# AmnonDrory/LidarRegistration

Measured on AMD Instinct MI355X. Metric: registration pairs/sec (30k-pt FCGF pairs, mutual-NN + 50k RANSAC iters + refit), higher is better.
Workload: dtype f32; 1 GPU; configs[1]: 30000-pt x32-d synthetic FCGF pair, --mode MNN --iters 50000, 3-pt sampling + ELC + LS refit; 192 distinct resident pairs per GPU, T copied to the host inside the timed region; pairs_per_batched_call=32, batched_calls_in_flight_per_gpu=2, parallelism=pair-sharded x1

## Files before the change

### include/lidarreg.h

```cpp
#ifndef LIDARREG_H
#define LIDARREG_H

#include <stddef.h>
#include <stdint.h>

#ifdef __cplusplus
extern "C" {
#endif

#define LR_API __attribute__((visibility("default")))

enum { LR_OK = 0, LR_EINVAL = -1, LR_ENOMEM = -2, LR_EHIP = -3, LR_ESIZE = -4 };

enum { LR_MODE_NO_FILTER = 0, LR_MODE_MNN = 1, LR_MODE_GPF = 2 };

typedef struct lr_workspace lr_workspace;

typedef struct lr_ransac_params {
    uint32_t struct_size;
    int32_t  sample_size;
    int32_t  use_elc;
    float    thr2;
    int32_t  iters;
    uint64_t seed;
    float    confidence;
    int32_t  batch;
    int32_t  sampler;
    int32_t  prosac_growth;
    int32_t  scoring;
    int32_t  local_opt;
    int32_t  lo_rounds;
    int32_t  lo_trials;
    int32_t  lo_max_calls;
    int32_t  min_iters;
} lr_ransac_params;

typedef struct lr_ransac_result {
    int64_t  best_h;
    uint32_t best_count;
    uint32_t pad0;
    uint64_t best_ssq;
    int64_t  n_valid;
    int64_t  n_ids;
} lr_ransac_result;

typedef struct lr_icp_result {
    double   fitness;
    double   inlier_rmse;
    int32_t  n_corr;
    int32_t  iterations;
} lr_icp_result;

typedef struct lr_pair_result {
    double   T[16];
    double   T_ransac[16];
    lr_ransac_result ransac;
    int32_t  n_corr;
    int32_t  n_refit;
    int32_t  n_nn_fixed;
    int32_t  status;
    int32_t  reserved[8];
    double   T_icp[16];
    lr_icp_result icp;
} lr_pair_result;

typedef struct lr_pair_params {
    uint32_t struct_size;
    int32_t  mode;
    int32_t  refit;
    lr_ransac_params ransac;
    int32_t  gpf_grid_wid;
    int32_t  icp;
    double   gpf_factor;
    double   refit_thr2;
} lr_pair_params;

LR_API int         lr_version(void);
LR_API const char *lr_last_error(void);

LR_API int    lr_workspace_create(lr_workspace **ws, int max_n0, int max_n1, int dim, int max_iters);
LR_API int    lr_workspace_create_batch(lr_workspace **ws, int max_pairs, int max_n0, int max_n1, int dim, int max_iters);
LR_API int    lr_workspace_destroy(lr_workspace *ws);
LR_API size_t lr_workspace_bytes(const lr_workspace *ws);
LR_API int    lr_workspace_poison(lr_workspace *ws, int byte, void *stream);
LR_API int    lr_debug_fake_current_device(int device);
enum {
    LR_OPT_NN_BLOCKS        = 1,
    LR_OPT_NN_BLOCKS_BATCH  = 2,
    LR_OPT_NN_SAMPLE_STRIDE = 3,
    LR_OPT_REV_STRIPS       = 4,
    LR_OPT_NN_SECOND_AUTO   = 5,
    LR_OPT_CLOCK_PROBE      = 6
};
LR_API int    lr_workspace_option(lr_workspace *ws, int option, int value);
LR_API int    lr_workspace_clock(lr_workspace *ws, double *mhz, unsigned long long *cycles, unsigned long long *ticks, int reset);

LR_API int lr_nn_top2(lr_workspace *ws, const float *F0, int n0, const float *F1, int n1, int dim,
                      int32_t *idx1, int32_t *idx2, float *s1, float *s2, void *stream);

LR_API int lr_nn_to_mutual(lr_workspace *ws, const float *F0, int n0, const float *F1, int n1, int dim,
                           const int32_t *idx1, const int32_t *idx2,
                           uint8_t *is_bb, int32_t *out_idx0, int32_t *out_idx1, int32_t *out_idx2,
                           int32_t *n_out, void *stream);

LR_API int lr_feat_ratio(const float *F0, const float *F1, int dim, int m,
                         const int32_t *i0, const int32_t *i1, const int32_t *i2, float *out, void *stream);

LR_API int lr_gpf(lr_workspace *ws, const float *F0, int n0, const float *F1, int n1, int dim,
                  const int32_t *idx1, const int32_t *idx2, const float *xyz0,
                  int grid_wid, double factor,
                  int32_t *out_idx0, int32_t *out_idx1, int32_t *out_idx2, float *out_score,
                  int32_t *n_out, void *stream);

LR_API int lr_gpf_bb_first(lr_workspace *ws, const float *F0, int n0, const float *F1, int n1, int dim,
                           const int32_t *idx1, const int32_t *idx2, const float *xyz0,
                           int grid_wid, double max_matches,
                           int32_t *out_idx0, int32_t *out_idx1, int32_t *out_idx2, float *out_score,
                           int32_t *n_out, int32_t *has_score, void *stream);

LR_API int lr_ransac(lr_workspace *ws, const float *src, const float *tgt, int m, const int32_t *m_dev,
                     const lr_ransac_params *p, double *T_out, lr_ransac_result *res, void *stream);

LR_API int lr_inlier_mask(lr_workspace *ws, const float *src, const float *tgt, int m, const double *T, float thr2,
                          uint8_t *mask, int32_t *n_inliers, void *stream);
LR_API int lr_workspace_mask_at(lr_workspace *ws, int pair, const float *xyz0, const float *xyz1, int n0, float thr2,
                                uint8_t *mask, int32_t *n_inliers, void *stream);

LR_API int lr_refit(lr_workspace *ws, const float *xyz0, int n0, const float *xyz1, const int32_t *idx1,
                    const double *T_in, double thr2, double *T_out, int32_t *n_inliers, void *stream);

LR_API int lr_icp(lr_workspace *ws, const float *xyz0, int n0, const float *xyz1, int n1, const double *T_init,
                  double max_dist, int max_iter, double rel_fitness, double rel_rmse,
                  double *T_out, lr_icp_result *res, void *stream);

LR_API int lr_icp_batch(lr_workspace *ws, double max_dist, int max_iter, double rel_fitness, double rel_rmse,
                        lr_pair_result *out, void *stream);

LR_API int lr_kabsch(const double *P, const double *Q, const double *w, int n, double *T_out, void *stream);

LR_API int lr_register_pair(lr_workspace *ws, const float *xyz0, const float *xyz1,
                            const float *F0, const float *F1, int n0, int n1, int dim,
                            const lr_pair_params *p, lr_pair_result *out, void *stream);

LR_API int lr_register_batch(lr_workspace *ws, int npairs, const float *const *xyz0, const float *const *xyz1,
                             const float *const *F0, const float *const *F1, const int32_t *n0, const int32_t *n1, int dim,
                             const lr_pair_params *p, lr_pair_result *out, void *stream);

LR_API int lr_workspace_lists(lr_workspace *ws, int n0, int32_t *nn_idx1, int32_t *nn_idx2,
                              int32_t *corr_idx0, int32_t *corr_idx1, void *stream);
LR_API int lr_workspace_lists_at(lr_workspace *ws, int pair, int n0, int32_t *nn_idx1, int32_t *nn_idx2,
                                 int32_t *corr_idx0, int32_t *corr_idx1, void *stream);
LR_API int lr_workspace_lists_batch(lr_workspace *ws, int npairs, int width, int32_t *nn_idx1, int32_t *nn_idx2,
                                    int32_t *corr_idx0, int32_t *corr_idx1, void *stream);

LR_API size_t lr_voxel_dedup_scratch_bytes(int n);
LR_API int    lr_voxel_dedup(const double *coords, int n, int32_t *sel, int32_t *n_sel, int32_t *cells, void *scratch,
                             size_t scratch_bytes, void *stream);

typedef struct lr_teaser_params {
    uint32_t struct_size;
    int32_t  max_iterations;
    double   noise_bound;
    double   cbar2;
    double   kcore_threshold;
    double   gnc_factor;
    double   cost_threshold;
    int64_t  node_budget;
    double   time_budget_ms;
    int32_t  rotation_tim_graph;
    int32_t  estimate_scaling;
} lr_teaser_params;

typedef struct lr_teaser_result {
    double   T[16];
    int32_t  status;
    int32_t  K;
    int32_t  exact;
    int32_t  max_core;
    int32_t  lb;
    int32_t  pad0;
    uint64_t nodes;
    int32_t  gnc_iters;
    int32_t  n_rot_inliers;
    int32_t  n_trans_inliers;
    int32_t  pad1;
} lr_teaser_result;

LR_API size_t lr_teaser_scratch_bytes(int max_m);
LR_API int lr_teaser(const float *src, const float *tgt, int m, const int32_t *m_dev, const lr_teaser_params *p,
                     lr_teaser_result *result, int32_t *clique_out, void *scratch, size_t scratch_bytes, void *stream);
LR_API int lr_teaser_batch(int npairs, const float *const *src, const float *const *tgt, const int32_t *m, const int32_t *const *m_dev,
                           const lr_teaser_params *p, lr_teaser_result *results, int32_t *const *clique_out, void *scratch,
                           size_t scratch_bytes, void *stream);
LR_API int lr_teaser_timing(int enable);
LR_API int lr_teaser_stage_times(float out[4]);

typedef struct lr_sm_params {
    uint32_t struct_size;
    int32_t  iterations;
    double   inlier_threshold;
    double   top_ratio;
} lr_sm_params;

typedef struct lr_sm_result {
    double   T[16];
    int32_t  status;
    int32_t  K;
    int32_t  m;
    int32_t  reserved;
    double   weight_sum;
} lr_sm_result;

LR_API size_t lr_sm_scratch_bytes(int max_m);
LR_API int lr_sm(const float *src, const float *tgt, int m, const int32_t *m_dev, const lr_sm_params *p, lr_sm_result *result,
                 float *eig_out, uint8_t *labels_out, void *scratch, size_t scratch_bytes, void *stream);
LR_API int lr_sm_batch(int npairs, const float *const *src, const float *const *tgt, const int32_t *m, const int32_t *const *m_dev,
                       const lr_sm_params *p, lr_sm_result *results, float *const *eig_out, uint8_t *const *labels_out, void *scratch,
                       size_t scratch_bytes, void *stream);

typedef struct lr_overlap_params {
    uint32_t struct_size;
    uint32_t reserved;
    double   voxel_size;
    double   radius;
} lr_overlap_params;

typedef struct lr_overlap_result {
    int32_t  status;
    int32_t  n0_ds, n1_ds;
    int32_t  n_overlap;
    int32_t  n0_dropped, n1_dropped;
    double   frac, frac_sym;
} lr_overlap_result;

LR_API size_t lr_voxel_mean_scratch_bytes(int n);
LR_API int lr_voxel_mean(const double *xyz, int n, const double *T, double voxel_size, double *cent, float *cent_f32,
                         int32_t *counts, int32_t *first, int32_t *info, void *scratch, size_t scratch_bytes, void *stream);
LR_API size_t lr_overlap_scratch_bytes(int max_n0, int max_n1);
LR_API int lr_overlap(const double *xyz0, int n0, const double *xyz1, int n1, const double *T, const lr_overlap_params *p,
                      lr_overlap_result *result, void *scratch, size_t scratch_bytes, void *stream);
LR_API int lr_overlap_batch(int npairs, const double *const *xyz0, const int32_t *n0, const double *const *xyz1, const int32_t *n1,
                            const double *const *T, const lr_overlap_params *p, lr_overlap_result *results, void *scratch,
                            size_t scratch_bytes, void *stream);

typedef struct lr_nn3_params {
    uint32_t struct_size;
    uint32_t reserved;
    double   cell;
} lr_nn3_params;

typedef struct lr_refine_z_params {
    uint32_t struct_size;
    int32_t  max_repeats;
    double   xy_gate;
    double   min_change;
    double   cell;
} lr_refine_z_params;

typedef struct lr_refine_z_result {
    int32_t  status;
    int32_t  repeats;
    int32_t  n_valid;
    int32_t  n0_dropped, n1_dropped;
    int32_t  reserved;
    double   dz;
    double   last_step;
} lr_refine_z_result;

LR_API size_t lr_nn3_scratch_bytes(int n0, int n1);
LR_API int lr_nn3(const double *xyz0, int n0, const double *xyz1, int n1, const lr_nn3_params *p, int32_t *idx, double *dist,
                  int32_t *info, void *scratch, size_t scratch_bytes, void *stream);
LR_API size_t lr_refine_z_scratch_bytes(int n0, int n1);
LR_API int lr_refine_z(const double *xyz0, int n0, const double *xyz1, int n1, const double *T, const lr_refine_z_params *p,
                       lr_refine_z_result *result, void *scratch, size_t scratch_bytes, void *stream);

typedef struct lr_bbrf_params {
    uint32_t struct_size;
    int32_t  n_iter;
    double   angles_lr, trans_lr;
    double   beta1, beta2, eps;
    double   cell;
} lr_bbrf_params;

typedef struct lr_bbrf_result {
    double   T[16];
    double   B_to_A[16];
    int32_t  status;
    int32_t  best_iter;
    double   best_loss;
    int32_t  n_pairs_best;
    int32_t  iters_run;
} lr_bbrf_result;

LR_API size_t lr_bbrf_scratch_bytes(int n0, int n1, int n_iter);
LR_API int lr_bbrf(const double *xyzA, const double *nrmA, int n0, const double *xyzB, const double *nrmB, int n1,
                   const lr_bbrf_params *params, lr_bbrf_result *result, double *log, void *scratch, size_t scratch_bytes, void *stream);
LR_API size_t lr_normals_scratch_bytes(int n);
LR_API int lr_normals(const double *xyz, int n, double radius, int max_nn, double *normals_out, int32_t *info, void *scratch,
                      size_t scratch_bytes, void *stream);

LR_API int lr_workspace_timing(lr_workspace *ws, int enable);
LR_API int lr_workspace_timing_read(lr_workspace *ws, float *nn_ms, float *ransac_ms, int *n_samples);
LR_API int lr_workspace_stage_times(lr_workspace *ws, float out[8], int *n_samples);

#ifdef __cplusplus
}
#endif
#endif
```

### lidarregistration_amd/_ext.py

```python
import ctypes
import os
import subprocess

_HERE = os.path.dirname(os.path.abspath(__file__))
CSRC = os.path.join(_HERE, "csrc")
LIB_PATH = os.environ.get("LIDARREG_LIB") or os.path.join(CSRC, "liblidarreg.so")

LR_MODE_NO_FILTER, LR_MODE_MNN, LR_MODE_GPF = 0, 1, 2

SYMBOLS = [
    "lr_version", "lr_last_error", "lr_workspace_create", "lr_workspace_destroy", "lr_workspace_bytes", "lr_workspace_poison",
    "lr_nn_top2", "lr_nn_to_mutual", "lr_feat_ratio", "lr_gpf", "lr_gpf_bb_first", "lr_ransac", "lr_refit", "lr_icp", "lr_kabsch",
    "lr_register_pair", "lr_workspace_lists", "lr_workspace_timing", "lr_workspace_timing_read",
    "lr_workspace_create_batch", "lr_register_batch", "lr_workspace_lists_at", "lr_inlier_mask", "lr_workspace_mask_at",
    "lr_voxel_dedup_scratch_bytes", "lr_voxel_dedup", "lr_workspace_option", "lr_workspace_stage_times", "lr_icp_batch", "lr_workspace_lists_batch",
    "lr_workspace_clock", "lr_debug_fake_current_device",
    "lr_teaser_scratch_bytes", "lr_teaser", "lr_teaser_batch", "lr_teaser_timing", "lr_teaser_stage_times",
    "lr_sm_scratch_bytes", "lr_sm", "lr_sm_batch",
    "lr_voxel_mean_scratch_bytes", "lr_voxel_mean", "lr_overlap_scratch_bytes", "lr_overlap", "lr_overlap_batch",
    "lr_nn3_scratch_bytes", "lr_nn3", "lr_refine_z_scratch_bytes", "lr_refine_z",
    "lr_bbrf_scratch_bytes", "lr_bbrf", "lr_normals_scratch_bytes", "lr_normals",
]

OPTIONS = {"nn_blocks": 1, "nn_blocks_batch": 2, "nn_sample_stride": 3, "rev_strips": 4, "nn_second_auto": 5, "clock_probe": 6}
DEFAULT_OPTIONS = {}


class LidarRegError(RuntimeError):
    pass


class RansacParams(ctypes.Structure):
    _fields_ = [("struct_size", ctypes.c_uint32), ("sample_size", ctypes.c_int32), ("use_elc", ctypes.c_int32), ("thr2", ctypes.c_float),
                ("iters", ctypes.c_int32), ("seed", ctypes.c_uint64), ("confidence", ctypes.c_float), ("batch", ctypes.c_int32),
                ("sampler", ctypes.c_int32), ("prosac_growth", ctypes.c_int32), ("scoring", ctypes.c_int32), ("local_opt", ctypes.c_int32),
                ("lo_rounds", ctypes.c_int32), ("lo_trials", ctypes.c_int32), ("lo_max_calls", ctypes.c_int32), ("min_iters", ctypes.c_int32)]

    def __init__(self, *args, **kw):
        kw.pop("struct_size", None)
        super().__init__(ctypes.sizeof(type(self)), *args, **kw)

    def effective_thr2(self):
        return float(self.thr2) * 2.25 if self.scoring == 2 else float(self.thr2)


class RansacResult(ctypes.Structure):
    _fields_ = [("best_h", ctypes.c_int64), ("best_count", ctypes.c_uint32), ("pad0", ctypes.c_uint32),
                ("best_ssq", ctypes.c_uint64), ("n_valid", ctypes.c_int64), ("n_ids", ctypes.c_int64)]


class IcpResult(ctypes.Structure):
    _fields_ = [("fitness", ctypes.c_double), ("inlier_rmse", ctypes.c_double), ("n_corr", ctypes.c_int32),
                ("iterations", ctypes.c_int32)]


class PairResult(ctypes.Structure):
    _fields_ = [("T", ctypes.c_double * 16), ("T_ransac", ctypes.c_double * 16), ("ransac", RansacResult),
                ("n_corr", ctypes.c_int32), ("n_refit", ctypes.c_int32), ("n_nn_fixed", ctypes.c_int32),
                ("status", ctypes.c_int32), ("reserved", ctypes.c_int32 * 8), ("T_icp", ctypes.c_double * 16), ("icp", IcpResult)]


class PairParams(ctypes.Structure):
    _fields_ = [("struct_size", ctypes.c_uint32), ("mode", ctypes.c_int32), ("refit", ctypes.c_int32), ("ransac", RansacParams),
                ("gpf_grid_wid", ctypes.c_int32), ("icp", ctypes.c_int32), ("gpf_factor", ctypes.c_double),
                ("refit_thr2", ctypes.c_double)]

    def __init__(self, *args, **kw):
        kw.pop("struct_size", None)
        super().__init__(ctypes.sizeof(type(self)), *args, **kw)
        if self.ransac.struct_size == 0:
            self.ransac.struct_size = ctypes.sizeof(RansacParams)


class TeaserParams(ctypes.Structure):
    _fields_ = [("struct_size", ctypes.c_uint32), ("max_iterations", ctypes.c_int32), ("noise_bound", ctypes.c_double),
                ("cbar2", ctypes.c_double), ("kcore_threshold", ctypes.c_double), ("gnc_factor", ctypes.c_double),
                ("cost_threshold", ctypes.c_double), ("node_budget", ctypes.c_int64), ("time_budget_ms", ctypes.c_double),
                ("rotation_tim_graph", ctypes.c_int32), ("estimate_scaling", ctypes.c_int32)]
    DEFAULTS = dict(max_iterations=10000, noise_bound=0.3, cbar2=1.0, kcore_threshold=0.5, gnc_factor=1.4, cost_threshold=1e-16,
                    node_budget=10 ** 7, time_budget_ms=10000.0)

    def __init__(self, **kw):
        kw.pop("struct_size", None)
        super().__init__(struct_size=ctypes.sizeof(type(self)), **{**self.DEFAULTS, **kw})


class TeaserResult(ctypes.Structure):
    _fields_ = [("T", ctypes.c_double * 16), ("status", ctypes.c_int32), ("K", ctypes.c_int32), ("exact", ctypes.c_int32),
                ("max_core", ctypes.c_int32), ("lb", ctypes.c_int32), ("pad0", ctypes.c_int32), ("nodes", ctypes.c_uint64),
                ("gnc_iters", ctypes.c_int32), ("n_rot_inliers", ctypes.c_int32), ("n_trans_inliers", ctypes.c_int32),
                ("pad1", ctypes.c_int32)]


class SmParams(ctypes.Structure):
    _fields_ = [("struct_size", ctypes.c_uint32), ("iterations", ctypes.c_int32), ("inlier_threshold", ctypes.c_double),
                ("top_ratio", ctypes.c_double)]
    DEFAULTS = dict(iterations=10, inlier_threshold=0.6, top_ratio=0.05)

    def __init__(self, **kw):
        kw.pop("struct_size", None)
        super().__init__(struct_size=ctypes.sizeof(type(self)), **{**self.DEFAULTS, **kw})


class SmResult(ctypes.Structure):
    _fields_ = [("T", ctypes.c_double * 16), ("status", ctypes.c_int32), ("K", ctypes.c_int32), ("m", ctypes.c_int32),
                ("reserved", ctypes.c_int32), ("weight_sum", ctypes.c_double)]


class OverlapParams(ctypes.Structure):
    _fields_ = [("struct_size", ctypes.c_uint32), ("reserved", ctypes.c_uint32), ("voxel_size", ctypes.c_double), ("radius", ctypes.c_double)]
    DEFAULTS = dict(voxel_size=1.0, radius=0.0)

    def __init__(self, **kw):
        kw.pop("struct_size", None)
        super().__init__(struct_size=ctypes.sizeof(type(self)), **{**self.DEFAULTS, **kw})


class OverlapResult(ctypes.Structure):
    _fields_ = [("status", ctypes.c_int32), ("n0_ds", ctypes.c_int32), ("n1_ds", ctypes.c_int32), ("n_overlap", ctypes.c_int32),
                ("n0_dropped", ctypes.c_int32), ("n1_dropped", ctypes.c_int32), ("frac", ctypes.c_double), ("frac_sym", ctypes.c_double)]


class Nn3Params(ctypes.Structure):
    _fields_ = [("struct_size", ctypes.c_uint32), ("reserved", ctypes.c_uint32), ("cell", ctypes.c_double)]

    def __init__(self, **kw):
        kw.pop("struct_size", None)
        super().__init__(struct_size=ctypes.sizeof(type(self)), **kw)


class RefineZParams(ctypes.Structure):
    _fields_ = [("struct_size", ctypes.c_uint32), ("max_repeats", ctypes.c_int32), ("xy_gate", ctypes.c_double), ("min_change", ctypes.c_double),
                ("cell", ctypes.c_double)]
    DEFAULTS = dict(max_repeats=10, xy_gate=0.3, min_change=1e-6, cell=0.0)

    def __init__(self, **kw):
        kw.pop("struct_size", None)
        super().__init__(struct_size=ctypes.sizeof(type(self)), **{**self.DEFAULTS, **kw})


class RefineZResult(ctypes.Structure):
    _fields_ = [("status", ctypes.c_int32), ("repeats", ctypes.c_int32), ("n_valid", ctypes.c_int32), ("n0_dropped", ctypes.c_int32),
                ("n1_dropped", ctypes.c_int32), ("reserved", ctypes.c_int32), ("dz", ctypes.c_double), ("last_step", ctypes.c_double)]


class BbrfParams(ctypes.Structure):
    _fields_ = [("struct_size", ctypes.c_uint32), ("n_iter", ctypes.c_int32), ("angles_lr", ctypes.c_double), ("trans_lr", ctypes.c_double),
                ("beta1", ctypes.c_double), ("beta2", ctypes.c_double), ("eps", ctypes.c_double), ("cell", ctypes.c_double)]
    DEFAULTS = dict(n_iter=100, angles_lr=2e-4, trans_lr=2e-4, beta1=0.9, beta2=0.999, eps=1e-8, cell=0.0)

    def __init__(self, **kw):
        kw.pop("struct_size", None)
        super().__init__(struct_size=ctypes.sizeof(type(self)), **{**self.DEFAULTS, **kw})


class BbrfResult(ctypes.Structure):
    _fields_ = [("T", ctypes.c_double * 16), ("B_to_A", ctypes.c_double * 16), ("status", ctypes.c_int32), ("best_iter", ctypes.c_int32),
                ("best_loss", ctypes.c_double), ("n_pairs_best", ctypes.c_int32), ("iters_run", ctypes.c_int32)]


assert ctypes.sizeof(BbrfParams) == 56 and ctypes.sizeof(BbrfResult) == 280
assert ctypes.sizeof(Nn3Params) == 16 and ctypes.sizeof(RefineZParams) == 32 and ctypes.sizeof(RefineZResult) == 40
assert ctypes.sizeof(OverlapParams) == 24 and ctypes.sizeof(OverlapResult) == 40
assert ctypes.sizeof(TeaserParams) == 72 and ctypes.sizeof(TeaserResult) == 176
assert ctypes.sizeof(SmParams) == 24 and ctypes.sizeof(SmResult) == 152
assert ctypes.sizeof(PairResult) == 496 and ctypes.sizeof(RansacParams) == 72 and ctypes.sizeof(PairParams) == 112

_lib = None


def build(force=False):
    srcs = [os.path.join(CSRC, f) for f in os.listdir(CSRC) if f.endswith((".hip", ".h"))]
    srcs.append(os.path.join(_HERE, "..", "include", "lidarreg.h"))
    stale = not os.path.exists(LIB_PATH) or any(os.path.getmtime(s) > os.path.getmtime(LIB_PATH) for s in srcs)
    if force or stale:
        subprocess.check_call(["make", "-C", CSRC, "-s", "-j4", "liblidarreg.so"])
    return LIB_PATH


def lib():
    global _lib
    if _lib is None:
        if not os.path.exists(LIB_PATH):
            raise LidarRegError(
                f"{LIB_PATH} is missing: build it with `python -c 'import __graft_entry__ as g; g.build()'` "
                "(hipcc --offload-arch=gfx950).  There is no CPU fallback.")
        import torch
        try:
            L = ctypes.CDLL(LIB_PATH)
        except OSError as e:
            raise LidarRegError(f"cannot load {LIB_PATH}: {e}") from e
        L.lr_last_error.restype = ctypes.c_char_p
        L.lr_workspace_bytes.restype = ctypes.c_size_t
        L.lr_workspace_bytes.argtypes = [ctypes.c_void_p]
        L.lr_workspace_poison.argtypes = [ctypes.c_void_p, ctypes.c_int, ctypes.c_void_p]
        L.lr_workspace_create.argtypes = [ctypes.POINTER(ctypes.c_void_p), ctypes.c_int, ctypes.c_int, ctypes.c_int, ctypes.c_int]
        L.lr_workspace_destroy.argtypes = [ctypes.c_void_p]
        vp, ci = ctypes.c_void_p, ctypes.c_int
        L.lr_nn_top2.argtypes = [vp, vp, ci, vp, ci, ci, vp, vp, vp, vp, vp]
        L.lr_nn_to_mutual.argtypes = [vp, vp, ci, vp, ci, ci, vp, vp, vp, vp, vp, vp, vp, vp]
        L.lr_feat_ratio.argtypes = [vp, vp, ci, ci, vp, vp, vp, vp, vp]
        L.lr_gpf.argtypes = [vp, vp, ci, vp, ci, ci, vp, vp, vp, ci, ctypes.c_double, vp, vp, vp, vp, vp, vp]
        L.lr_gpf_bb_first.argtypes = [vp, vp, ci, vp, ci, ci, vp, vp, vp, ci, ctypes.c_double, vp, vp, vp, vp, vp, vp, vp]
        L.lr_ransac.argtypes = [vp, vp, vp, ci, vp, ctypes.POINTER(RansacParams), vp, vp, vp]
        L.lr_refit.argtypes = [vp, vp, ci, vp, vp, vp, ctypes.c_double, vp, vp, vp]
        L.lr_icp.argtypes = [vp, vp, ci, vp, ci, vp, ctypes.c_double, ci, ctypes.c_double, ctypes.c_double, vp, vp, vp]
        L.lr_kabsch.argtypes = [vp, vp, vp, ci, vp, vp]
        L.lr_icp_batch.argtypes = [vp, ctypes.c_double, ci, ctypes.c_double, ctypes.c_double, vp, vp]
        L.lr_register_pair.argtypes = [vp, vp, vp, vp, vp, ci, ci, ci, ctypes.POINTER(PairParams), vp, vp]
        L.lr_workspace_lists.argtypes = [vp, ci, vp, vp, vp, vp, vp]
        L.lr_workspace_lists_at.argtypes = [vp, ci, ci, vp, vp, vp, vp, vp]
        L.lr_workspace_lists_batch.argtypes = [vp, ci, ci, vp, vp, vp, vp, vp]
        L.lr_inlier_mask.argtypes = [vp, vp, vp, ci, vp, ctypes.c_float, vp, vp, vp]
        L.lr_workspace_mask_at.argtypes = [vp, ci, vp, vp, ci, ctypes.c_float, vp, vp, vp]
        L.lr_voxel_dedup_scratch_bytes.restype = ctypes.c_size_t
        L.lr_voxel_dedup_scratch_bytes.argtypes = [ci]
        L.lr_voxel_dedup.argtypes = [vp, ci, vp, vp, vp, vp, ctypes.c_size_t, vp]
        L.lr_workspace_create_batch.argtypes = [ctypes.POINTER(ctypes.c_void_p), ci, ci, ci, ci, ci]
        pp, ip = ctypes.POINTER(ctypes.c_void_p), ctypes.POINTER(ctypes.c_int32)
        L.lr_register_batch.argtypes = [vp, ci, pp, pp, pp, pp, ip, ip, ci, ctypes.POINTER(PairParams), vp, vp]
        L.lr_workspace_option.argtypes = [vp, ci, ci]
        L.lr_workspace_stage_times.argtypes = [vp, ctypes.POINTER(ctypes.c_float * 8), ctypes.POINTER(ci)]
        L.lr_workspace_timing.argtypes = [vp, ci]
        if hasattr(L, "lr_workspace_clock"):
            L.lr_workspace_clock.argtypes = [vp, ctypes.POINTER(ctypes.c_double), ctypes.POINTER(ctypes.c_ulonglong), ctypes.POINTER(ctypes.c_ulonglong), ci]
        L.lr_teaser_scratch_bytes.restype = ctypes.c_size_t
        L.lr_teaser_scratch_bytes.argtypes = [ci]
        L.lr_teaser.argtypes = [vp, vp, ci, vp, ctypes.POINTER(TeaserParams), vp, vp, vp, ctypes.c_size_t, vp]
        L.lr_teaser_batch.argtypes = [ci, pp, pp, ip, pp, ctypes.POINTER(TeaserParams), vp, pp, vp, ctypes.c_size_t, vp]
        L.lr_teaser_timing.argtypes = [ci]
        L.lr_teaser_stage_times.argtypes = [ctypes.POINTER(ctypes.c_float * 4)]
        L.lr_sm_scratch_bytes.restype = ctypes.c_size_t
        L.lr_sm_scratch_bytes.argtypes = [ci]
        L.lr_sm.argtypes = [vp, vp, ci, vp, ctypes.POINTER(SmParams), vp, vp, vp, vp, ctypes.c_size_t, vp]
        L.lr_sm_batch.argtypes = [ci, pp, pp, ip, pp, ctypes.POINTER(SmParams), vp, pp, pp, vp, ctypes.c_size_t, vp]
        dp = ctypes.c_double
        L.lr_voxel_mean_scratch_bytes.restype = ctypes.c_size_t
        L.lr_voxel_mean_scratch_bytes.argtypes = [ci]
        L.lr_voxel_mean.argtypes = [vp, ci, vp, dp, vp, vp, vp, vp, vp, vp, ctypes.c_size_t, vp]
        L.lr_overlap_scratch_bytes.restype = ctypes.c_size_t
        L.lr_overlap_scratch_bytes.argtypes = [ci, ci]
        L.lr_overlap.argtypes = [vp, ci, vp, ci, vp, ctypes.POINTER(OverlapParams), vp, vp, ctypes.c_size_t, vp]
        L.lr_overlap_batch.argtypes = [ci, pp, ip, pp, ip, pp, ctypes.POINTER(OverlapParams), vp, vp, ctypes.c_size_t, vp]
        L.lr_nn3_scratch_bytes.restype = ctypes.c_size_t
        L.lr_nn3_scratch_bytes.argtypes = [ci, ci]
        L.lr_nn3.argtypes = [vp, ci, vp, ci, ctypes.POINTER(Nn3Params), vp, vp, vp, vp, ctypes.c_size_t, vp]
        L.lr_refine_z_scratch_bytes.restype = ctypes.c_size_t
        L.lr_refine_z_scratch_bytes.argtypes = [ci, ci]
        L.lr_refine_z.argtypes = [vp, ci, vp, ci, vp, ctypes.POINTER(RefineZParams), vp, vp, ctypes.c_size_t, vp]
        L.lr_bbrf_scratch_bytes.restype = ctypes.c_size_t
        L.lr_bbrf_scratch_bytes.argtypes = [ci, ci, ci]
        L.lr_bbrf.argtypes = [vp, vp, ci, vp, vp, ci, ctypes.POINTER(BbrfParams), vp, vp, vp, ctypes.c_size_t, vp]
        L.lr_normals_scratch_bytes.restype = ctypes.c_size_t
        L.lr_normals_scratch_bytes.argtypes = [ci]
        L.lr_normals.argtypes = [vp, ci, dp, ci, vp, vp, vp, ctypes.c_size_t, vp]
        L.lr_workspace_timing_read.argtypes = [vp, ctypes.POINTER(ctypes.c_float), ctypes.POINTER(ctypes.c_float), ctypes.POINTER(ci)]
        _lib = L
    return _lib


def check(rc):
    if rc != 0:
        raise LidarRegError(f"liblidarreg error {rc}: {lib().lr_last_error().decode()}")


class Workspace:

    def __init__(self, max_n0, max_n1, dim=32, max_iters=50000, max_pairs=1):
        self._h = ctypes.c_void_p()
        self.max_n0, self.max_n1, self.dim, self.max_iters = int(max_n0), int(max_n1), int(dim), int(max_iters)
        self.max_pairs = int(max_pairs)
        check(lib().lr_workspace_create_batch(ctypes.byref(self._h), self.max_pairs, self.max_n0, self.max_n1, self.dim, self.max_iters))
        for name, value in DEFAULT_OPTIONS.items():
            self.set_option(name, value)

    def set_option(self, name, value):
        check(lib().lr_workspace_option(self._h, OPTIONS[name], int(value)))

    def stage_times(self):
        out = (ctypes.c_float * 8)(); n = ctypes.c_int()
        check(lib().lr_workspace_stage_times(self._h, out, ctypes.byref(n)))
        return list(out[:6]), n.value

    def timing(self, enable):
        check(lib().lr_workspace_timing(self._h, int(bool(enable))))

    def clock(self, reset=False):
        mhz = ctypes.c_double(); cyc = ctypes.c_ulonglong(); tk = ctypes.c_ulonglong()
        check(lib().lr_workspace_clock(self._h, ctypes.byref(mhz), ctypes.byref(cyc), ctypes.byref(tk), int(bool(reset))))
        return mhz.value, cyc.value, tk.value

    @property
    def handle(self):
        return self._h

    def fits(self, n0, n1, dim, iters):
        return n0 <= self.max_n0 and n1 <= self.max_n1 and dim == self.dim and iters <= self.max_iters

    @property
    def nbytes(self):
        return lib().lr_workspace_bytes(self._h)

    def poison(self, byte, stream=None):
        check(lib().lr_workspace_poison(self._h, int(byte), stream))

    def close(self):
        if self._h:
            lib().lr_workspace_destroy(self._h)
            self._h = ctypes.c_void_p()

    def __del__(self):
        try:
            self.close()
        except Exception:
            pass
```

### lidarregistration_amd/csrc/lr_api.hip

```cpp
#include "lr_internal.h"
#include <stdarg.h>
#include <string.h>
#include <stdlib.h>
#include <new>

static thread_local char g_err[512] = "";

void lr_set_error(const char *fmt, ...)
{
    va_list ap;
    va_start(ap, fmt);
    vsnprintf(g_err, sizeof(g_err), fmt, ap);
    va_end(ap);
}

static_assert(sizeof(lr_ransac_params) == 72 && sizeof(lr_pair_params) == 112 && sizeof(lr_pair_result) == 496,
              "ABI structs changed: update include/lidarreg.h, _ext.py, INTEGRATION.md and tests/test_abi_cpu.py together");

extern "C" int lr_version(void) { return 103; }
extern "C" const char *lr_last_error(void) { return g_err; }

static inline void forget_last_batch(lr_workspace *ws) { if (ws) { ws->last_batch = 0; ws->last_T_final = nullptr; } }

static int g_fake_device = -1;
struct lr_device_info { int known, ok, cus; char arch[64]; };
static lr_device_info g_dev[64];

static int device_info(int dev, const lr_device_info **out)
{
    if (dev < 0 || dev >= 64) { lr_set_error("device index %d out of range", dev); return LR_EINVAL; }
    lr_device_info &d = g_dev[dev];
    if (!d.known) {
        hipDeviceProp_t prop;
        LR_HIP(hipGetDeviceProperties(&prop, dev));
        snprintf(d.arch, sizeof d.arch, "%s", prop.gcnArchName);
        d.ok = strncmp(prop.gcnArchName, "gfx950", 6) == 0;
        d.cus = prop.multiProcessorCount > 0 ? prop.multiProcessorCount : 256;
        d.known = 1;
    }
    *out = &d;
    return LR_OK;
}

static int check_device(const lr_workspace *ws, hipStream_t st, const char *who)
{
    if (!ws) { lr_set_error("%s: null workspace", who); return LR_EINVAL; }
    int cur = -1;
    LR_HIP(hipGetDevice(&cur));
    if (g_fake_device >= 0) cur = g_fake_device;
    if (cur != ws->device) {
        lr_set_error("%s: the workspace was created on device %d but device %d is current (hipSetDevice / torch.cuda.set_device before the call; one workspace per device)",
                     who, ws->device, cur);
        return LR_EINVAL;
    }
    if (st) {
        hipDevice_t sd = -1;
        if (hipStreamGetDevice(st, &sd) == hipSuccess) {
            if ((int)sd != ws->device) { lr_set_error("%s: the stream belongs to device %d, the workspace to device %d", who, (int)sd, ws->device); return LR_EINVAL; }
        } else (void)hipGetLastError();
    }
    return LR_OK;
}
#define LR_CHECK_DEVICE(ws, stream, who) do { int rc_d_ = check_device(ws, (hipStream_t)(stream), who); if (rc_d_ != LR_OK) return rc_d_; } while (0)

int lr_check_memory_device(const void *mem, hipStream_t st, const char *who, int *n_cus)
{
    hipPointerAttribute_t attr;
    if (hipPointerGetAttributes(&attr, mem) != hipSuccess || attr.type != hipMemoryTypeDevice) {
        (void)hipGetLastError();
        lr_set_error("%s: scratch is not device memory", who);
        return LR_EINVAL;
    }
    int cur = -1;
    LR_HIP(hipGetDevice(&cur));
    if (g_fake_device >= 0) cur = g_fake_device;
    if (cur != attr.device) {
        lr_set_error("%s: the scratch lives on device %d but device %d is current (hipSetDevice / torch.cuda.set_device before the call)", who, attr.device, cur);
        return LR_EINVAL;
    }
    if (st) {
        hipDevice_t sd = -1;
        if (hipStreamGetDevice(st, &sd) == hipSuccess) {
            if ((int)sd != attr.device) { lr_set_error("%s: the stream belongs to device %d, the scratch to device %d", who, (int)sd, attr.device); return LR_EINVAL; }
        } else (void)hipGetLastError();
    }
    const lr_device_info *info = nullptr;
    LR_TRY_HIP(device_info(attr.device, &info));
    if (!info->ok) { lr_set_error("%s: device %d is %s; this library holds gfx950 code objects only", who, attr.device, info->arch); return LR_EINVAL; }
    if (n_cus) *n_cus = info->cus;
    return LR_OK;
}

extern "C" int lr_debug_fake_current_device(int device) { g_fake_device = device; return LR_OK; }

namespace {
struct Carver {
    size_t off = 0;
    char *base = nullptr;
    template <class T> T *take(size_t count)
    {
        off = (off + 255) & ~size_t(255);
        T *p = base ? reinterpret_cast<T *>(base + off) : nullptr;
        off += sizeof(T) * count;
        return p;
    }
};

void carve(lr_workspace *ws, Carver &c)
{
    const size_t n0 = ws->max_n0, n1 = ws->max_n1, n = ws->max_n, it = ws->max_iters;
    ws->nrm0 = c.take<float>(n0); ws->nrm1 = c.take<float>(n1);
    ws->H0 = c.take<_Float16>(n0 * 32); ws->H1 = c.take<_Float16>(n1 * 32);
    if (ws->dim != LR_FEAT_DIM) { ws->P0 = c.take<float>(n0 * 32); ws->P1 = c.take<float>(n1 * 32); }
    ws->tau = c.take<float>(n);
    ws->yfin = c.take<float>(n * LR_NN_MAX_STRIPS);
    ws->yshare = c.take<uint32_t>(n);
    ws->cand_cnt = c.take<int32_t>(LR_NN16_CNT_INTS(n)); ws->cand = c.take<int32_t>(LR_NN16_SEG_INTS(n));
    ws->counters = c.take<int32_t>(LR_CNT_TOTAL);
    ws->bmax0 = c.take<float>(n0 / 32 + 2); ws->bmax1 = c.take<float>(n1 / 32 + 2);
    ws->bmin0 = c.take<float>(n0 / 32 + 2); ws->bmin1 = c.take<float>(n1 / 32 + 2);
    ws->nn_range = c.take<float>(8);
    ws->rev_seed = c.take<uint32_t>(n1); ws->rev_rows = c.take<int32_t>(n1);
    ws->rev_seed64 = c.take<unsigned long long>(n1);
    ws->rev_cols = c.take<int32_t>(n0); ws->rev_s1 = c.take<float>(n0); ws->rev_pos = c.take<int32_t>(n0);
    ws->rev_tmin = c.take<float>(n0 / 32 + 2); ws->rev_hist = c.take<int32_t>(2 * 4096);
    ws->Hs = c.take<_Float16>(n0 * 32); ws->nrms = c.take<float>(n0);
    ws->nn_idx1 = c.take<int32_t>(n0); ws->nn_idx2 = c.take<int32_t>(n0);
    ws->nn_s1 = c.take<float>(n0); ws->nn_s2 = c.take<float>(n0);
    ws->rev_idx1 = c.take<int32_t>(n1);
    ws->is_bb = c.take<uint8_t>(n0);
    ws->blk_cnt = c.take<int32_t>(n0 / 256 + 2);
    ws->corr_idx0 = c.take<int32_t>(n0); ws->corr_idx1 = c.take<int32_t>(n0); ws->corr_idx2 = c.take<int32_t>(n0);
    ws->corr_score = c.take<float>(n0);
    ws->ratio = c.take<float>(n0);
    ws->cell = c.take<int32_t>(n0); ws->cell_sorted = c.take<int32_t>(n0);
    ws->gpf_quota = c.take<double>(LR_GPF_MAX_CELLS);
    ws->gpf_cells = c.take<int32_t>(3 * (LR_GPF_MAX_CELLS + 8) > 2 * (LR_PR_BUCKETS + 8) + 8 ? 3 * (LR_GPF_MAX_CELLS + 8) : 2 * (LR_PR_BUCKETS + 8) + 8);
    ws->gpf_keep = c.take<uint8_t>(n0);
    ws->gpf_f = c.take<float>(8);
    ws->corr8 = c.take<float>((n0 + 2) * 8);
    ws->prosac_G = c.take<int32_t>(n0 + 2); ws->prosac_rank = c.take<int32_t>(n0);
    ws->models = c.take<float>(it * 12);
    ws->models64 = c.take<double>(it * 12);
    ws->model_h = c.take<int32_t>(it);
    ws->models2 = c.take<float>(it * 12); ws->models64_2 = c.take<double>(it * 12); ws->model_h2 = c.take<int32_t>(it);
    ws->score_cnt = c.take<uint32_t>(it);
    ws->score_ssq = c.take<unsigned long long>(it);
    ws->refit_part = c.take<double>((n0 / 256 + 2) * 16);
    ws->icp_ints = c.take<int32_t>(3 * (32768 + 8));
    ws->icp_bucket = c.take<int32_t>(n1); ws->icp_pts = c.take<float>(4 * n1);
    ws->icp_state = c.take<double>(32); ws->icp_part = c.take<double>((n0 / 256 + 2) * 18);
    ws->lo_list = c.take<int32_t>(n0);
    ws->lo_ctl = c.take<char>(LR_LO_CTL_BYTES);
    ws->sc_info = c.take<char>(LR_SC_INFO_BYTES);
    ws->corr8s = c.take<float>((n0 + 4) * 8);
    ws->sc_perm = c.take<int32_t>(it); ws->sc_glen = c.take<int32_t>(it / 64 + 2);
    ws->sc_mb = c.take<uint8_t>(it); ws->sc_cb = c.take<uint8_t>(n0);
    ws->models_s = c.take<float>(it * 12);
    ws->res_tmp = c.take<lr_ransac_result>(1);
    ws->T_tmp = c.take<double>(48);
}
}

extern "C" int lr_workspace_create(lr_workspace **out, int max_n0, int max_n1, int dim, int max_iters)
{
    return lr_workspace_create_batch(out, 1, max_n0, max_n1, dim, max_iters);
}

extern "C" int lr_workspace_create_batch(lr_workspace **out, int max_pairs, int max_n0, int max_n1, int dim, int max_iters)
{
    LR_REQUIRE(out, LR_EINVAL, "lr_workspace_create: null output");
    LR_REQUIRE(max_pairs >= 1 && max_pairs <= LR_MAX_BATCH, LR_EINVAL, "lr_workspace_create_batch: max_pairs must be in [1, 64]");
    LR_REQUIRE(max_n0 > 0 && max_n1 > 0 && max_iters >= 0, LR_EINVAL, "lr_workspace_create: sizes must be positive");
    LR_REQUIRE(dim >= 1 && dim <= LR_FEAT_DIM, LR_EINVAL, "lr_workspace_create: descriptors of 1 to 32 dimensions are supported");
    LR_REQUIRE(max_n0 < (1 << 22) && max_n1 < (1 << 22), LR_ESIZE, "lr_workspace_create: clouds are limited to 2^22 points");
    int dev = -1;
    LR_HIP(hipGetDevice(&dev));
    const lr_device_info *di = nullptr;
    LR_TRY_HIP(device_info(dev, &di));
    if (!di->ok) {
        lr_set_error("lr_workspace_create: device %d is %s; this library holds gfx950 (MI355X) code objects only", dev, di->arch);
        return LR_EINVAL;
    }
    lr_workspace *ws = new (std::nothrow) lr_workspace();
    LR_REQUIRE(ws, LR_ENOMEM, "lr_workspace_create: host allocation failed");
    memset(ws, 0, sizeof(*ws));
    ws->device = dev; ws->n_cus = di->cus;
    ws->max_n0 = max_n0; ws->max_n1 = max_n1; ws->max_n = max_n0 > max_n1 ? max_n0 : max_n1;
    ws->dim = dim; ws->max_iters = max_iters > 0 ? max_iters : 1;
    ws->max_pairs = max_pairs;
    ws->nn_blocks_target = 3 * ws->n_cus;
    ws->nn_blocks_batch = 12 * ws->n_cus;
    ws->nn_sample_stride = 0; ws->rev_strips = 0; ws->nn_second_auto = 0; ws->clock_probe = 0;
    Carver sizing;
    carve(ws, sizing);
    ws->stride = (sizing.off + 511) & ~size_t(255);
    const size_t desc_off = ws->stride * (size_t)max_pairs;
    const size_t clk_off = (desc_off + sizeof(lr_pair_desc) * LR_MAX_BATCH + 255) & ~size_t(255);
    ws->bytes = clk_off + 256;
    hipError_t e = hipMalloc(&ws->base, ws->bytes);
    if (e != hipSuccess) {
        lr_set_error("lr_workspace_create: hipMalloc(%zu) -> %s", ws->bytes, hipGetErrorString(e));
        delete ws;
        return e == hipErrorOutOfMemory ? LR_ENOMEM : LR_EHIP;
    }
    Carver real;
    real.base = ws->base;
    carve(ws, real);
    ws->descs = reinterpret_cast<lr_pair_desc *>(ws->base + desc_off);
    ws->clk_dev = reinterpret_cast<unsigned long long *>(ws->base + clk_off);
    if (hipHostMalloc(reinterpret_cast<void **>(&ws->form_host), 2 * sizeof(int32_t), hipHostMallocMapped) == hipSuccess) {
        ws->form_host[0] = ws->form_host[1] = 0;
        if (hipHostGetDevicePointer(reinterpret_cast<void **>(&ws->form_dev), ws->form_host, 0) != hipSuccess) { (void)hipHostFree(ws->form_host); ws->form_host = ws->form_dev = nullptr; }
    } else { (void)hipGetLastError(); ws->form_host = ws->form_dev = nullptr; }
    if (hipMemset(ws->base, 0, ws->bytes) != hipSuccess || hipStreamSynchronize(nullptr) != hipSuccess) {
        if (ws->form_host) (void)hipHostFree(ws->form_host);
        (void)hipFree(ws->base); delete ws; lr_set_error("lr_workspace_create: hipMemset failed"); return LR_EHIP;
    }
    for (int k = 0; k < LR_NEV; ++k)
        if (hipEventCreate(&ws->timer.ev[k]) != hipSuccess) {
            for (int q = 0; q < k; ++q) (void)hipEventDestroy(ws->timer.ev[q]);
            if (ws->form_host) (void)hipHostFree(ws->form_host);
            (void)hipFree(ws->base); delete ws; lr_set_error("lr_workspace_create: hipEventCreate failed"); return LR_EHIP;
        }
    *out = ws;
    return LR_OK;
}

extern "C" int lr_workspace_destroy(lr_workspace *ws)
{
    if (!ws) return LR_OK;
    if (ws->form_host) (void)hipHostFree(ws->form_host);
    for (int k = 0; k < LR_NEV; ++k) (void)hipEventDestroy(ws->timer.ev[k]);
    (void)hipFree(ws->base);
    delete ws;
    return LR_OK;
}

extern "C" size_t lr_workspace_bytes(const lr_workspace *ws) { return ws ? ws->bytes : 0; }

extern "C" int lr_workspace_option(lr_workspace *ws, int option, int value)
{
    LR_REQUIRE(ws, LR_EINVAL, "lr_workspace_option: null workspace");
    LR_REQUIRE(value >= 0, LR_EINVAL, "lr_workspace_option: value must be >= 0");
    switch (option) {
    case LR_OPT_NN_BLOCKS: ws->nn_blocks_target = value > 0 ? value : 3 * ws->n_cus; break;
    case LR_OPT_NN_BLOCKS_BATCH: ws->nn_blocks_batch = value > 0 ? value : 12 * ws->n_cus; break;
    case LR_OPT_NN_SAMPLE_STRIDE: ws->nn_sample_stride = value > 4096 ? 4096 : value; break;
    case LR_OPT_REV_STRIPS: ws->rev_strips = value > 64 ? 64 : value; break;
    case LR_OPT_NN_SECOND_AUTO: ws->nn_second_auto = value ? 1 : 0; break;
    case LR_OPT_CLOCK_PROBE: ws->clock_probe = value ? 1 : 0; break;
    default: lr_set_error("lr_workspace_option: unknown option %d", option); return LR_EINVAL;
    }
    return LR_OK;
}

extern "C" int lr_workspace_poison(lr_workspace *ws, int byte, void *stream)
{
    LR_CHECK_DEVICE(ws, stream, "lr_workspace_poison");
    forget_last_batch(ws);
    LR_HIP(hipMemsetAsync(ws->base, byte & 0xff, ws->bytes, (hipStream_t)stream));
    return LR_OK;
}

extern "C" int lr_workspace_lists(lr_workspace *ws, int n0, int32_t *nn_idx1, int32_t *nn_idx2,
                                  int32_t *corr_idx0, int32_t *corr_idx1, void *stream)
{
    return lr_workspace_lists_at(ws, 0, n0, nn_idx1, nn_idx2, corr_idx0, corr_idx1, stream);
}

extern "C" int lr_workspace_lists_at(lr_workspace *ws, int pair, int n0, int32_t *nn_idx1, int32_t *nn_idx2,
                                     int32_t *corr_idx0, int32_t *corr_idx1, void *stream)
{
    LR_CHECK_DEVICE(ws, stream, "lr_workspace_lists");
    LR_REQUIRE(pair >= 0 && pair < ws->max_pairs, LR_EINVAL, "lr_workspace_lists: pair outside the workspace");
    LR_REQUIRE(pair < ws->last_npairs, LR_EINVAL, "lr_workspace_lists: the last registration call on this workspace had fewer pairs");
    LR_REQUIRE(n0 > 0 && n0 <= ws->max_n0, LR_ESIZE, "lr_workspace_lists: n0 exceeds the workspace");
    hipStream_t st = (hipStream_t)stream;
    const size_t nb = sizeof(int32_t) * (size_t)n0, off = (size_t)pair * ws->stride;
    auto at = [&](const int32_t *p) { return reinterpret_cast<const char *>(p) + off; };
    if (nn_idx1) LR_HIP(hipMemcpyAsync(nn_idx1, at(ws->nn_idx1), nb, hipMemcpyDeviceToDevice, st));
    if (nn_idx2) LR_HIP(hipMemcpyAsync(nn_idx2, at(ws->nn_idx2), nb, hipMemcpyDeviceToDevice, st));
    if (corr_idx0) LR_HIP(hipMemcpyAsync(corr_idx0, at(ws->corr_idx0), nb, hipMemcpyDeviceToDevice, st));
    if (corr_idx1) LR_HIP(hipMemcpyAsync(corr_idx1, at(ws->corr_idx1), nb, hipMemcpyDeviceToDevice, st));
    return LR_OK;
}

extern "C" int lr_workspace_lists_batch(lr_workspace *ws, int npairs, int width, int32_t *nn_idx1, int32_t *nn_idx2,
                                        int32_t *corr_idx0, int32_t *corr_idx1, void *stream)
{
    LR_CHECK_DEVICE(ws, stream, "lr_workspace_lists_batch");
    LR_REQUIRE(npairs >= 1 && npairs <= ws->last_npairs, LR_EINVAL, "lr_workspace_lists_batch: the last registration call on this workspace had fewer pairs");
    LR_REQUIRE(width > 0 && width <= ws->max_n0, LR_ESIZE, "lr_workspace_lists_batch: width exceeds the workspace");
    hipStream_t st = (hipStream_t)stream;
    const size_t wb = sizeof(int32_t) * (size_t)width;
    auto copy = [&](int32_t *dst, const int32_t *src) -> int {
        if (!dst) return LR_OK;
        LR_HIP(hipMemcpy2DAsync(dst, wb, src, ws->stride, wb, (size_t)npairs, hipMemcpyDeviceToDevice, st));
        return LR_OK;
    };
    LR_TRY_HIP(copy(nn_idx1, ws->nn_idx1)); LR_TRY_HIP(copy(nn_idx2, ws->nn_idx2));
    LR_TRY_HIP(copy(corr_idx0, ws->corr_idx0)); LR_TRY_HIP(copy(corr_idx1, ws->corr_idx1));
    return LR_OK;
}

__global__ void __launch_bounds__(256) zero_scratch_kernel(uint32_t *__restrict__ p, size_t words, lr_zargs z)
{
    lr_z(p, z, blockIdx.z);
    for (size_t k = (size_t)blockIdx.x * 256 + threadIdx.x; k < words; k += (size_t)gridDim.x * 256) p[k] = 0u;
}
int lr_zero_scratch(const lr_call &c, void *p, size_t bytes)
{
    const size_t words = (bytes + 3) / 4;
    int blocks = (int)((words + 255) / 256);
    if (blocks > 1024) blocks = 1024;
    hipLaunchKernelGGL(zero_scratch_kernel, dim3(blocks < 1 ? 1 : blocks, 1, c.pairs), dim3(256), 0, c.st, reinterpret_cast<uint32_t *>(p), words, c.z);
    LR_LAUNCH_CHECK();
    return LR_OK;
}

extern "C" int lr_workspace_clock(lr_workspace *ws, double *mhz, unsigned long long *cycles, unsigned long long *ticks, int reset)
{
    LR_CHECK_DEVICE(ws, nullptr, "lr_workspace_clock");
    unsigned long long h[2] = { 0ull, 0ull };
    LR_HIP(hipMemcpy(h, ws->clk_dev, sizeof h, hipMemcpyDeviceToHost));
    if (cycles) *cycles = h[0];
    if (ticks) *ticks = h[1];
    if (mhz) *mhz = h[1] ? 100.0 * (double)h[0] / (double)h[1] : 0.0;
    if (reset) LR_HIP(hipMemset(ws->clk_dev, 0, sizeof h));
    return LR_OK;
}

int lr_timer_mark(const lr_call &c, lr_event e)
{
    lr_stage_timer &t = c.ws->timer;
    bool due = false;
    switch (e) {
    case LR_EV_FWD_FILTER_BEGIN: case LR_EV_FWD_FILTER_END: due = c.armed && !t.begun(); break;
    case LR_EV_REV_FILTER_BEGIN: case LR_EV_REV_FILTER_END: due = t.begun() && !t.has(LR_EV_REV_FILTER_END) && !t.has(LR_EV_RANSAC_END); break;
    case LR_EV_RANSAC_BEGIN: case LR_EV_RANSAC_END: due = t.begun() && !t.has(LR_EV_RANSAC_END); break;
    case LR_EV_CALL_BEGIN: case LR_EV_FWD_NN_DONE: case LR_EV_REV_NN_DONE: due = c.armed; break;
    case LR_EV_CALL_END: due = c.armed && t.has(LR_EV_RANSAC_END); break;
    case LR_NEV: break;
    }
    if (!t.on || !due) return LR_OK;
    LR_HIP(hipEventRecord(t.ev[e], c.st));
    t.recorded |= 1u << e;
    return LR_OK;
}

static int lr_timer_collect(lr_stage_timer &t)
{
    if (!t.begun()) return LR_OK;
    float ms = 0;
    auto span = [&](lr_event a, lr_event b) -> int { LR_HIP(hipEventElapsedTime(&ms, t.ev[a], t.ev[b])); return LR_OK; };
    LR_TRY_HIP(span(LR_EV_FWD_FILTER_BEGIN, LR_EV_FWD_FILTER_END)); t.ms.nn += ms; t.ms.fwd_filter += ms;
    if (t.has(LR_EV_REV_FILTER_END)) { LR_TRY_HIP(span(LR_EV_REV_FILTER_BEGIN, LR_EV_REV_FILTER_END)); t.ms.nn += ms; t.ms.rev_filter += ms; }
    if (t.has(LR_EV_RANSAC_END)) { LR_TRY_HIP(span(LR_EV_RANSAC_BEGIN, LR_EV_RANSAC_END)); t.ms.ransac += ms; }
    if (t.has(LR_EV_CALL_END)) {
        LR_TRY_HIP(span(LR_EV_CALL_BEGIN, LR_EV_CALL_END)); t.ms.call += ms;
        LR_TRY_HIP(span(LR_EV_CALL_BEGIN, LR_EV_FWD_NN_DONE)); t.ms.fwd += ms;
        if (t.has(LR_EV_REV_NN_DONE)) { LR_TRY_HIP(span(LR_EV_FWD_NN_DONE, LR_EV_REV_NN_DONE)); t.ms.rev += ms; }
    }
    t.n_samples += 1;
    t.recorded = 0;
    return LR_OK;
}

extern "C" int lr_workspace_timing(lr_workspace *ws, int enable)
{
    LR_CHECK_DEVICE(ws, nullptr, "lr_workspace_timing");
    ws->timer.on = enable; ws->timer.recorded = 0; ws->timer.n_samples = 0; ws->timer.ms = {};
    return LR_OK;
}

extern "C" int lr_workspace_timing_read(lr_workspace *ws, float *nn_ms, float *ransac_ms, int *n_samples)
{
    LR_CHECK_DEVICE(ws, nullptr, "lr_workspace_timing_read");
    LR_TRY_HIP(lr_timer_collect(ws->timer));
    if (nn_ms) *nn_ms = ws->timer.ms.nn;
    if (ransac_ms) *ransac_ms = ws->timer.ms.ransac;
    if (n_samples) *n_samples = ws->timer.n_samples;
    return LR_OK;
}

extern "C" int lr_workspace_stage_times(lr_workspace *ws, float out[8], int *n_samples)
{
    LR_REQUIRE(ws && out, LR_EINVAL, "lr_workspace_stage_times: null pointer");
    LR_CHECK_DEVICE(ws, nullptr, "lr_workspace_stage_times");
    const lr_stage_timer &t = ws->timer;
    LR_TRY_HIP(lr_timer_collect(ws->timer));
    out[0] = t.ms.call; out[1] = t.ms.fwd; out[2] = t.ms.fwd_filter; out[3] = t.ms.rev_filter; out[4] = t.ms.ransac; out[5] = t.ms.rev;
    out[6] = out[7] = 0.0f;
    if (n_samples) *n_samples = t.n_samples;
    return LR_OK;
}

static int check_nn_args(const lr_workspace *ws, const void *F0, int n0, const void *F1, int n1, int dim, const char *who)
{
    if (!ws || !F0 || !F1) { lr_set_error("%s: null pointer", who); return LR_EINVAL; }
    if (dim != ws->dim) { lr_set_error("%s: dim %d != workspace dim %d", who, dim, ws->dim); return LR_EINVAL; }
    if (n0 <= 0 || n1 <= 0) { lr_set_error("%s: empty cloud (n0=%d, n1=%d)", who, n0, n1); return LR_EINVAL; }
    if (n0 > ws->max_n0 || n1 > ws->max_n1) { lr_set_error("%s: (%d,%d) exceeds workspace (%d,%d)", who, n0, n1, ws->max_n0, ws->max_n1); return LR_ESIZE; }
    return LR_OK;
}

#define LR_TRY(x) do { int rc_ = (x); if (rc_ != LR_OK) return rc_; } while (0)


static int check_ransac_params(const lr_ransac_params *p, const char *who) { LR_CHECK_STRUCT_SIZE(lr_ransac_params, p, who); return LR_OK; }
static int check_pair_params(const lr_pair_params *p, const char *who) { LR_CHECK_STRUCT_SIZE(lr_pair_params, p, who); return check_ransac_params(&p->ransac, who); }

__global__ void __launch_bounds__(256)
pad_feats_kernel(const float *__restrict__ Fa, int na, float *__restrict__ Pa, const float *__restrict__ Fb, int nb, float *__restrict__ Pb,
                 int dim, int nblk_a, lr_zargs z)
{
    if (z.descs) { const lr_pair_desc d = z.descs[blockIdx.z]; Fa = d.F0; na = d.n0; Fb = d.F1; nb = d.n1; }
    lr_z(Pa, z, blockIdx.z); lr_z(Pb, z, blockIdx.z);
    const bool second = (int)blockIdx.x >= nblk_a;
    const float *__restrict__ F = second ? Fb : Fa;
    float *__restrict__ P = second ? Pb : Pa;
    const int n = second ? nb : na;
    const int row = (second ? blockIdx.x - nblk_a : blockIdx.x) * 8 + (threadIdx.x >> 5), k = threadIdx.x & 31;
    if (row < n) P[(size_t)row * 32 + k] = k < dim ? F[(size_t)row * dim + k] : 0.0f;
}
__global__ void pad_patch_descs_kernel(lr_pair_desc *__restrict__ descs, int npairs, float *P0, float *P1, size_t stride)
{
    const int k = threadIdx.x;
    if (k < npairs) {
        descs[k].F0 = reinterpret_cast<const float *>(reinterpret_cast<const char *>(P0) + (size_t)k * stride);
        descs[k].F1 = reinterpret_cast<const float *>(reinterpret_cast<const char *>(P1) + (size_t)k * stride);
    }
}
static void pad_if_narrow(const lr_call &c, const float *&F0, int n0, const float *&F1, int n1, int &dim)
{
    if (dim == LR_FEAT_DIM) return;
    lr_workspace *ws = c.ws;
    const int nblk_a = lr_cdiv(n0, 8);
    hipLaunchKernelGGL(pad_feats_kernel, dim3(nblk_a + lr_cdiv(n1, 8), 1, c.pairs), dim3(256), 0, c.st, F0, n0, ws->P0, F1, n1, ws->P1, dim, nblk_a, c.z);
    if (c.z.descs) hipLaunchKernelGGL(pad_patch_descs_kernel, dim3(1), dim3(64), 0, c.st, ws->descs, c.pairs, ws->P0, ws->P1, ws->stride);
    F0 = ws->P0; F1 = ws->P1; dim = LR_FEAT_DIM;
}

static int operator_prep(lr_workspace *ws, const float *&F0, int n0, const float *&F1, int n1, int &dim, void *stream, const char *who,
                         bool required, const char *required_msg, lr_call *call)
{
    LR_TRY(check_nn_args(ws, F0, n0, F1, n1, dim, who));
    LR_CHECK_DEVICE(ws, stream, who);
    forget_last_batch(ws);
    LR_REQUIRE(required, LR_EINVAL, required_msg);
    *call = lr_call_single(ws, stream);
    pad_if_narrow(*call, F0, n0, F1, n1, dim);
    return lr_nn16_prep(*call, F0, n0, F1, n1);
}

extern "C" int lr_nn_top2(lr_workspace *ws, const float *F0, int n0, const float *F1, int n1, int dim,
                          int32_t *idx1, int32_t *idx2, float *s1, float *s2, void *stream)
{
    lr_call c;
    LR_TRY(operator_prep(ws, F0, n0, F1, n1, dim, stream, "lr_nn_top2", idx1, "lr_nn_top2: idx1 is required", &c));
    return lr_nn16_run(c, F0, n0, F1, n1, idx1, idx2, s1, s2);
}

extern "C" int lr_nn_to_mutual(lr_workspace *ws, const float *F0, int n0, const float *F1, int n1, int dim,
                               const int32_t *idx1, const int32_t *idx2, uint8_t *is_bb,
                               int32_t *o0, int32_t *o1, int32_t *o2, int32_t *n_out, void *stream)
{
    lr_call c;
    LR_TRY(operator_prep(ws, F0, n0, F1, n1, dim, stream, "lr_nn_to_mutual", idx1, "lr_nn_to_mutual: idx1 is required", &c));
    LR_TRY(lr_nn16_reverse(c, F0, n0, F1, n1, idx1, ws->rev_idx1));
    return lr_mutual_run(c, n0, idx1, idx2, ws->rev_idx1, is_bb, o0, o1, o2, n_out);
}

extern "C" int lr_gpf(lr_workspace *ws, const float *F0, int n0, const float *F1, int n1, int dim,
                      const int32_t *idx1, const int32_t *idx2, const float *xyz0, int grid_wid, double factor,
                      int32_t *o0, int32_t *o1, int32_t *o2, float *oscore, int32_t *n_out, void *stream)
{
    lr_call c;
    LR_TRY(operator_prep(ws, F0, n0, F1, n1, dim, stream, "lr_gpf", idx1 && idx2 && xyz0 && o0 && o1, "lr_gpf: null pointer", &c));
    LR_TRY(lr_nn16_reverse(c, F0, n0, F1, n1, idx1, ws->rev_idx1));
    LR_TRY(lr_mutual_run(c, n0, idx1, nullptr, ws->rev_idx1, ws->is_bb, nullptr, nullptr, nullptr, nullptr));
    return lr_gpf_run(c, F0, n0, F1, dim, idx1, idx2, ws->is_bb, xyz0, grid_wid, factor, o0, o1, o2, oscore, n_out);
}

extern "C" int lr_gpf_bb_first(lr_workspace *ws, const float *F0, int n0, const float *F1, int n1, int dim,
                               const int32_t *idx1, const int32_t *idx2, const float *xyz0, int grid_wid, double max_matches,
                               int32_t *o0, int32_t *o1, int32_t *o2, float *oscore, int32_t *n_out, int32_t *has_score,
                               void *stream)
{
    lr_call c;
    LR_TRY(operator_prep(ws, F0, n0, F1, n1, dim, stream, "lr_gpf_bb_first", idx1 && idx2 && xyz0 && o0 && o1 && o2 && n_out && has_score,
                         "lr_gpf_bb_first: null pointer", &c));
    int32_t *mb_dev = ws->counters + LR_CNT_NCORR;
    LR_TRY(lr_nn16_reverse(c, F0, n0, F1, n1, idx1, ws->rev_idx1));
    LR_TRY(lr_mutual_run(c, n0, idx1, idx2, ws->rev_idx1, ws->is_bb, ws->corr_idx0, ws->corr_idx1, ws->corr_idx2, mb_dev));
    const lr_gpf_subset sub = { mb_dev, ws->corr_idx0, has_score, max_matches };
    return lr_gpf_run(c, F0, n0, F1, dim, ws->corr_idx1, ws->corr_idx2, nullptr, xyz0, grid_wid, 0.0, o0, o1, o2, oscore, n_out, nullptr, nullptr, &sub);
}

extern "C" int lr_ransac(lr_workspace *ws, const float *src, const float *tgt, int m, const int32_t *m_dev,
                         const lr_ransac_params *p, double *T_out, lr_ransac_result *res, void *stream)
{
    LR_REQUIRE(ws && src && tgt && p && T_out && res, LR_EINVAL, "lr_ransac: null pointer");
    LR_TRY(check_ransac_params(p, "lr_ransac"));
    LR_CHECK_DEVICE(ws, stream, "lr_ransac");
    forget_last_batch(ws);
    LR_REQUIRE(m >= 0 && m <= ws->max_n0, LR_ESIZE, "lr_ransac: m exceeds the workspace");
    const lr_call c = lr_call_single(ws, stream);
    LR_TRY(lr_pack_corr(c, src, tgt, nullptr, nullptr, m, m_dev, ws->corr8));
    return lr_ransac_run(c, ws->corr8, m, m_dev, p, T_out, res);
}

extern "C" int lr_inlier_mask(lr_workspace *ws, const float *src, const float *tgt, int m, const double *T, float thr2,
                              uint8_t *mask, int32_t *n_inliers, void *stream)
{
    LR_REQUIRE(src && tgt && mask && m >= 0, LR_EINVAL, "lr_inlier_mask: bad argument");
    LR_REQUIRE(T || ws, LR_EINVAL, "lr_inlier_mask: neither a model nor a workspace");
    LR_REQUIRE(thr2 > 0.0f, LR_EINVAL, "lr_inlier_mask: thr2 must be positive");
    if (!T) LR_CHECK_DEVICE(ws, stream, "lr_inlier_mask");
    return lr_inlier_mask_run(src, tgt, nullptr, nullptr, m, nullptr, T ? T : ws->T_tmp, thr2, mask, n_inliers, (hipStream_t)stream);
}

extern "C" int lr_workspace_mask_at(lr_workspace *ws, int pair, const float *xyz0, const float *xyz1, int n0, float thr2,
                                    uint8_t *mask, int32_t *n_inliers, void *stream)
{
    LR_REQUIRE(ws && xyz0 && xyz1 && mask, LR_EINVAL, "lr_workspace_mask_at: null pointer");
    LR_REQUIRE(pair >= 0 && pair < ws->max_pairs, LR_EINVAL, "lr_workspace_mask_at: pair outside the workspace");
    LR_REQUIRE(pair < ws->last_npairs, LR_EINVAL, "lr_workspace_mask_at: the last registration call on this workspace had fewer pairs");
    LR_REQUIRE(n0 > 0 && n0 <= ws->max_n0, LR_ESIZE, "lr_workspace_mask_at: n0 exceeds the workspace");
    LR_REQUIRE(thr2 > 0.0f, LR_EINVAL, "lr_workspace_mask_at: thr2 must be positive");
    LR_CHECK_DEVICE(ws, stream, "lr_workspace_mask_at");
    const size_t off = (size_t)pair * ws->stride;
    auto at = [&](auto *p) { return reinterpret_cast<decltype(p)>(reinterpret_cast<char *>(p) + off); };
    return lr_inlier_mask_run(xyz0, xyz1, at(ws->corr_idx0), at(ws->corr_idx1), n0, at(ws->counters) + LR_CNT_NCORR, at(ws->T_tmp), thr2,
                              mask, n_inliers, (hipStream_t)stream);
}

extern "C" int lr_refit(lr_workspace *ws, const float *xyz0, int n0, const float *xyz1, const int32_t *idx1,
                        const double *T_in, double thr2, double *T_out, int32_t *n_inl, void *stream)
{
    LR_REQUIRE(ws && xyz0 && xyz1 && idx1 && T_in && T_out, LR_EINVAL, "lr_refit: null pointer");
    LR_REQUIRE(n0 > 0 && n0 <= ws->max_n0, LR_ESIZE, "lr_refit: n0 exceeds the workspace");
    LR_CHECK_DEVICE(ws, stream, "lr_refit");
    forget_last_batch(ws);
    return lr_refit_run(lr_call_single(ws, stream), xyz0, n0, xyz1, idx1, T_in, thr2, T_out, n_inl, nullptr);
}

extern "C" int lr_icp(lr_workspace *ws, const float *xyz0, int n0, const float *xyz1, int n1, const double *T_init,
                      double max_dist, int max_iter, double rel_fitness, double rel_rmse, double *T_out, lr_icp_result *res, void *stream)
{
    LR_REQUIRE(ws && xyz0 && xyz1 && T_init && T_out, LR_EINVAL, "lr_icp: null pointer");
    LR_REQUIRE(n0 > 0 && n0 <= ws->max_n0 && n1 > 0 && n1 <= ws->max_n1, LR_ESIZE, "lr_icp: cloud exceeds the workspace");
    LR_CHECK_DEVICE(ws, stream, "lr_icp");
    forget_last_batch(ws);
    return lr_icp_run(lr_call_single(ws, stream), xyz0, n0, xyz1, n1, T_init, nullptr, max_dist, max_iter, rel_fitness, rel_rmse, T_out, res);
}

__global__ void pair_icp_kernel(const double *__restrict__ T_icp, const lr_icp_result *__restrict__ r, lr_pair_result *__restrict__ out, int have, lr_zargs z);

extern "C" int lr_icp_batch(lr_workspace *ws, double max_dist, int max_iter, double rel_fitness, double rel_rmse, lr_pair_result *out, void *stream)
{
    LR_REQUIRE(ws && out, LR_EINVAL, "lr_icp_batch: null pointer");
    LR_CHECK_DEVICE(ws, stream, "lr_icp_batch");
    LR_REQUIRE(ws->last_batch && ws->last_npairs >= 1 && ws->last_T_final, LR_EINVAL,
               "lr_icp_batch: no successful lr_register_batch on this workspace since the last call that touched its scratch");
    hipStream_t st = (hipStream_t)stream;
    LR_REQUIRE(st == ws->last_stream, LR_EINVAL, "lr_icp_batch: must be enqueued on the stream of the lr_register_batch call it continues");
    const lr_call c = lr_call_batch(ws, stream, ws->last_npairs);
    lr_icp_result *icp_res = reinterpret_cast<lr_icp_result *>(ws->icp_state + 24);
    LR_TRY(lr_icp_run(c, nullptr, ws->last_mx0, nullptr, ws->last_mx1, ws->last_T_final, ws->res_tmp, max_dist, max_iter, rel_fitness, rel_rmse,
                      ws->T_tmp + 32, icp_res));
    hipLaunchKernelGGL(pair_icp_kernel, dim3(1, 1, c.pairs), dim3(64), 0, st, ws->T_tmp + 32, icp_res, out, 1, c.z);
    if (hipGetLastError() != hipSuccess) { lr_set_error("lr_icp_batch: launch failed"); return LR_EHIP; }
    return LR_OK;
}

__global__ void pair_icp_kernel(const double *__restrict__ T_icp, const lr_icp_result *__restrict__ r, lr_pair_result *__restrict__ out, int have,
                                lr_zargs z)
{
    lr_z(T_icp, z, blockIdx.z); lr_z(r, z, blockIdx.z);
    out += blockIdx.z;
    const int k = threadIdx.x;
    if (k < 16) out->T_icp[k] = have ? T_icp[k] : out->T[k];
    if (k == 0) {
        if (have) out->icp = *r;
        else { out->icp.fitness = 0.0; out->icp.inlier_rmse = 0.0; out->icp.n_corr = 0; out->icp.iterations = 0; }
    }
}

__global__ void pair_result_kernel(const double *__restrict__ T_ransac, const double *__restrict__ T_final,
                                   const lr_ransac_result *__restrict__ rr, const int32_t *__restrict__ counters,
                                   const int32_t *__restrict__ n_refit, lr_pair_result *__restrict__ out, lr_zargs z)
{
    lr_z(T_ransac, z, blockIdx.z); lr_z(T_final, z, blockIdx.z); lr_z(rr, z, blockIdx.z); lr_z(counters, z, blockIdx.z); lr_z(n_refit, z, blockIdx.z);
    out += blockIdx.z;
    const int k = threadIdx.x;
    if (k < 16) { out->T[k] = T_final[k]; out->T_ransac[k] = T_ransac[k]; }
    if (k == 0) {
        out->ransac = *rr;
        out->n_corr = counters[LR_CNT_NCORR];
        out->n_refit = n_refit ? *n_refit : 0;
        out->n_nn_fixed = counters[LR_CNT_FIX_TOTAL];
        out->status = rr->best_h < 0 ? 1 : 0;
        for (int q = 0; q < 8; ++q) out->reserved[q] = 0;
        out->reserved[1] = reinterpret_cast<const lr_ransac_state *>(counters + LR_CNT_COUNT)->lo_timeouts;
        out->reserved[2] = (counters[LR_CNT_FORM_MISS_F] ? 1 : 0) | (counters[LR_CNT_FORM_MISS_R] ? 2 : 0);
        out->icp.fitness = 0.0; out->icp.inlier_rmse = 0.0; out->icp.n_corr = 0; out->icp.iterations = 0;
    }
    if (k < 16) out->T_icp[k] = T_final[k];
}

static int register_stages(const lr_call &c, const float *xyz0, const float *xyz1, const float *F0, const float *F1,
                           int n0, int n1, int dim, const lr_pair_params *p, lr_pair_result *out)
{
    lr_workspace *ws = c.ws;
    int32_t *m_dev = ws->counters + LR_CNT_NCORR;
    int32_t *n_refit = ws->counters + LR_CNT_COUNT - 2;
    pad_if_narrow(c, F0, n0, F1, n1, dim);
    LR_TRY(lr_nn16_prep(c, F0, n0, F1, n1, true));
    const bool fuse_seed = p->mode != LR_MODE_NO_FILTER;
    LR_TRY_HIP(lr_timer_mark(c, LR_EV_CALL_BEGIN));
    const bool want2 = !(ws->nn_second_auto && p->mode != LR_MODE_GPF && p->ransac.sampler == 0);
    int32_t *idx2 = want2 ? ws->nn_idx2 : nullptr;
    LR_TRY(lr_nn16_run(c, F0, n0, F1, n1, ws->nn_idx1, idx2, ws->nn_s1, ws->nn_s2, fuse_seed));
    LR_TRY_HIP(lr_timer_mark(c, LR_EV_FWD_NN_DONE));
    if (p->mode == LR_MODE_NO_FILTER) {
        LR_TRY(lr_identity_corr(c, n0, ws->nn_idx1, idx2, ws->corr_idx0, ws->corr_idx1, idx2 ? ws->corr_idx2 : nullptr, m_dev));
    } else {
        LR_TRY(lr_nn16_reverse(c, F0, n0, F1, n1, ws->nn_idx1, ws->rev_idx1, fuse_seed));
        LR_TRY_HIP(lr_timer_mark(c, LR_EV_REV_NN_DONE));
        if (p->mode == LR_MODE_MNN) {
            LR_TRY(lr_mutual_run(c, n0, ws->nn_idx1, idx2, ws->rev_idx1, ws->is_bb, ws->corr_idx0, ws->corr_idx1,
                                 idx2 ? ws->corr_idx2 : nullptr, m_dev, xyz0, xyz1, ws->corr8));
        } else {
            LR_TRY(lr_mutual_run(c, n0, ws->nn_idx1, nullptr, ws->rev_idx1, ws->is_bb, nullptr, nullptr, nullptr, nullptr));
            LR_TRY(lr_gpf_run(c, F0, n0, F1, dim, ws->nn_idx1, ws->nn_idx2, ws->is_bb, xyz0, p->gpf_grid_wid, p->gpf_factor,
                              ws->corr_idx0, ws->corr_idx1, ws->corr_idx2, ws->corr_score, m_dev, xyz1, ws->corr8));
        }
    }
    if (p->ransac.sampler == 1) {
        LR_TRY(lr_prosac_order(c, F0, F1, dim, p->mode == LR_MODE_GPF ? ws->corr_score : nullptr, n0, m_dev));
        LR_TRY(lr_pack_corr(c, xyz0, xyz1, ws->corr_idx0, ws->corr_idx1, n0, m_dev, ws->corr8, ws->prosac_rank));
    } else if (p->mode == LR_MODE_NO_FILTER) LR_TRY(lr_pack_corr(c, xyz0, xyz1, ws->corr_idx0, ws->corr_idx1, n0, m_dev, ws->corr8));
    LR_TRY(lr_ransac_run(c, ws->corr8, n0, m_dev, &p->ransac, ws->T_tmp, ws->res_tmp));
    const double *T_final = ws->T_tmp;
    if (p->refit) {
        const bool filtered = p->refit == 2, weighted = p->refit == 3;
        LR_TRY(lr_refit_run(c, xyz0, n0, xyz1, filtered ? ws->corr_idx1 : ws->nn_idx1, ws->T_tmp, p->refit_thr2, ws->T_tmp + 16, n_refit, ws->res_tmp, out,
                            filtered ? ws->corr_idx0 : nullptr, filtered ? m_dev : nullptr, weighted ? F0 : nullptr, weighted ? F1 : nullptr));
        T_final = ws->T_tmp + 16;
    }
    if (!p->refit)
        hipLaunchKernelGGL(pair_result_kernel, dim3(1, 1, c.pairs), dim3(64), 0, c.st, ws->T_tmp, T_final, ws->res_tmp, ws->counters,
                           (const int32_t *)nullptr, out, c.z);
    ws->last_T_final = T_final; ws->last_mx0 = n0; ws->last_mx1 = n1;
    if (p->icp) {
        lr_icp_result *icp_res = reinterpret_cast<lr_icp_result *>(ws->icp_state + 24);
        LR_TRY(lr_icp_run(c, xyz0, n0, xyz1, n1, T_final, ws->res_tmp, 0.6, 30, 1e-6, 1e-6, ws->T_tmp + 32, icp_res));
        hipLaunchKernelGGL(pair_icp_kernel, dim3(1, 1, c.pairs), dim3(64), 0, c.st, ws->T_tmp + 32, icp_res, out, 1, c.z);
    }
    LR_TRY_HIP(lr_timer_mark(c, LR_EV_CALL_END));
    LR_LAUNCH_CHECK();
    return LR_OK;
}

extern "C" int lr_register_pair(lr_workspace *ws, const float *xyz0, const float *xyz1, const float *F0, const float *F1,
                                int n0, int n1, int dim, const lr_pair_params *p, lr_pair_result *out, void *stream)
{
    LR_REQUIRE(ws && xyz0 && xyz1 && p && out, LR_EINVAL, "lr_register_pair: null pointer");
    LR_TRY(check_pair_params(p, "lr_register_pair"));
    LR_TRY(check_nn_args(ws, F0, n0, F1, n1, dim, "lr_register_pair"));
    LR_CHECK_DEVICE(ws, stream, "lr_register_pair");
    LR_REQUIRE(p->mode == LR_MODE_NO_FILTER || p->mode == LR_MODE_MNN || p->mode == LR_MODE_GPF, LR_EINVAL,
               "lr_register_pair: unknown mode");
    ws->last_npairs = 1; ws->last_batch = 0;
    return register_stages(lr_call_single(ws, stream), xyz0, xyz1, F0, F1, n0, n1, dim, p, out);
}

__global__ void batch_setup_kernel(lr_desc_table t, lr_pair_desc *__restrict__ descs, int npairs)
{
    const int k = threadIdx.x;
    if (k < npairs) descs[k] = t.d[k];
}

extern "C" int lr_register_batch(lr_workspace *ws, int npairs, const float *const *xyz0, const float *const *xyz1,
                                 const float *const *F0, const float *const *F1, const int32_t *n0, const int32_t *n1, int dim,
                                 const lr_pair_params *p, lr_pair_result *out, void *stream)
{
    LR_REQUIRE(ws && xyz0 && xyz1 && F0 && F1 && n0 && n1 && p && out, LR_EINVAL, "lr_register_batch: null pointer");
    LR_TRY(check_pair_params(p, "lr_register_batch"));
    LR_REQUIRE(npairs >= 1 && npairs <= ws->max_pairs, LR_ESIZE, "lr_register_batch: npairs exceeds the workspace (lr_workspace_create_batch)");
    LR_CHECK_DEVICE(ws, stream, "lr_register_batch");
    LR_REQUIRE(p->mode == LR_MODE_NO_FILTER || p->mode == LR_MODE_MNN || p->mode == LR_MODE_GPF, LR_EINVAL,
               "lr_register_batch: unknown mode");
    lr_desc_table t;
    int mx0 = 0, mx1 = 0;
    for (int k = 0; k < npairs; ++k) {
        LR_REQUIRE(xyz0[k] && xyz1[k], LR_EINVAL, "lr_register_batch: null pointer");
        LR_TRY(check_nn_args(ws, F0[k], n0[k], F1[k], n1[k], dim, "lr_register_batch"));
        t.d[k] = lr_pair_desc{ xyz0[k], xyz1[k], F0[k], F1[k], n0[k], n1[k] };
        mx0 = n0[k] > mx0 ? n0[k] : mx0; mx1 = n1[k] > mx1 ? n1[k] : mx1;
    }
    for (int k = npairs; k < LR_MAX_BATCH; ++k) t.d[k] = lr_pair_desc{ nullptr, nullptr, nullptr, nullptr, 0, 0 };
    hipStream_t st = (hipStream_t)stream;
    hipLaunchKernelGGL(batch_setup_kernel, dim3(1), dim3(64), 0, st, t, ws->descs, npairs);
    ws->last_npairs = npairs; forget_last_batch(ws);
    const int rc = register_stages(lr_call_batch(ws, stream, npairs), xyz0[0], xyz1[0], F0[0], F1[0], mx0, mx1, dim, p, out);
    if (rc == LR_OK) { ws->last_batch = 1; ws->last_stream = st; } else ws->last_T_final = nullptr;
    return rc;
}
```

### lidarregistration_amd/csrc/lr_internal.h

```cpp
#pragma once
#include <hip/hip_runtime.h>
#include <stdint.h>
#include <stdio.h>
#include "../../include/lidarreg.h"

void lr_set_error(const char *fmt, ...);

#define LR_HIP(call)                                                                      \
    do {                                                                                  \
        hipError_t e_ = (call);                                                           \
        if (e_ != hipSuccess) {                                                           \
            lr_set_error("%s:%d: %s -> %s", __FILE__, __LINE__, #call, hipGetErrorString(e_)); \
            return LR_EHIP;                                                               \
        }                                                                                 \
    } while (0)

#define LR_LAUNCH_CHECK() LR_HIP(hipGetLastError())

#define LR_REQUIRE(cond, code, msg)                 \
    do {                                            \
        if (!(cond)) { lr_set_error("%s", msg); return code; } \
    } while (0)

#define LR_NN16_SEG 4096
#define LR_NN16_SEG_INTS(n) ((size_t)((n) / 256 + 1) * 4 * LR_NN16_SEG * 2)
#define LR_NN16_CNT_INTS(n) ((size_t)((n) / 256 + 1) * 4 * 65)
static inline int lr_cdiv(int a, int b) { return (a + b - 1) / b; }
__host__ __device__ static inline int lr_seg_cap(int strips) { const int c = (LR_NN16_SEG / strips) & ~63; return c < 64 ? 64 : c; }

#define LR_TRY_HIP(x) do { int rc__ = (x); if (rc__ != LR_OK) return rc__; } while (0)

#define LR_CHECK_STRUCT_SIZE(T, p, who) do {                                                                                            \
        if (!(p)) { lr_set_error("%s: null params", who); return LR_EINVAL; }                                                            \
        if ((p)->struct_size != sizeof(T)) {                                                                                             \
            lr_set_error("%s: " #T ".struct_size is %u, this library (lr_version %d) expects %zu -- set it to sizeof(" #T ") / rebuild against include/lidarreg.h", \
                         who, (p)->struct_size, lr_version(), sizeof(T));                                                                \
            return LR_EINVAL;                                                                                                            \
        } } while (0)

#define LR_NN_MAX_STRIPS 8
#define LR_FEAT_DIM 32

#ifndef LR_SCORE_BLOCKS
#define LR_SCORE_BLOCKS 2048
#endif
#define LR_GPF_MAX_CELLS 4096
#define LR_PR_BUCKETS 8192
#define LR_SC_INFO_BYTES 2048
#define LR_LO_CTL_BYTES 20480

struct lr_pair_desc {
    const float *xyz0, *xyz1, *F0, *F1;
    int32_t n0, n1;
};
struct lr_zargs {
    size_t stride;
    const lr_pair_desc *descs;
};
#define LR_MAX_BATCH 64
struct lr_desc_table { lr_pair_desc d[LR_MAX_BATCH]; };

#ifdef __HIPCC__
#define lr_z(p, z, pair) \
    do { const size_t lr_zo_ = (size_t)(pair) * (z).stride; p = (decltype(p))((const char *)(p) + (lr_zo_ & ((size_t)0 - (size_t)((p) != nullptr)))); } while (0)
__device__ __forceinline__ bool lr_xcd_block(int total, int &logical)
{
    const int chunk = (int)gridDim.x >> 3;
    logical = ((int)blockIdx.x & 7) * chunk + ((int)blockIdx.x >> 3);
    return logical < total;
}
#endif

enum lr_event {
    LR_EV_FWD_FILTER_BEGIN, LR_EV_FWD_FILTER_END,
    LR_EV_RANSAC_BEGIN, LR_EV_RANSAC_END,
    LR_EV_REV_FILTER_BEGIN, LR_EV_REV_FILTER_END,
    LR_EV_CALL_BEGIN,
    LR_EV_FWD_NN_DONE, LR_EV_CALL_END, LR_EV_REV_NN_DONE,
    LR_NEV
};
struct lr_stage_timer {
    int on;
    unsigned recorded;
    int n_samples;
    hipEvent_t ev[LR_NEV];
    struct { float call, fwd, fwd_filter, rev_filter, ransac, rev, nn; } ms;
    bool has(lr_event e) const { return (recorded >> e & 1u) != 0; }
    bool begun() const { return has(LR_EV_FWD_FILTER_END); }
    bool armed() const { return on && !begun(); }
};

struct lr_workspace {
    int max_n0, max_n1, max_n, dim, max_iters;
    int max_pairs;
    int device, n_cus;
    int last_npairs;
    int last_batch;
    int last_mx0, last_mx1;
    const double *last_T_final;
    hipStream_t last_stream;
    size_t stride;
    size_t bytes;
    char *base;
    lr_pair_desc *descs;
    float *nrm0, *nrm1;
    _Float16 *H0, *H1;
    float *P0, *P1;
    float *tau;
    uint32_t *yshare;
    float *yfin;
    int32_t *cand_cnt, *cand;
    float *bmax0, *bmax1;
    float *bmin0, *bmin1;
    float *nn_range;
    int form_prev[2];
    int32_t *form_host, *form_dev;
    uint32_t *rev_seed;
    unsigned long long *rev_seed64;
    int32_t *rev_rows;
    int32_t *rev_cols;
    int32_t *rev_pos;
    float *rev_s1;
    float *rev_tmin;
    int32_t *rev_hist;
    _Float16 *Hs; float *nrms;
    int nn_blocks_target;
    int nn_blocks_batch;
    int nn_sample_stride;
    int rev_strips;
    int nn_second_auto;
    int clock_probe;
    unsigned long long *clk_dev;
    int32_t *counters;
    int32_t *nn_idx1, *nn_idx2;
    float *nn_s1, *nn_s2;
    int32_t *rev_idx1;
    uint8_t *is_bb;
    int32_t *blk_cnt;
    int32_t *corr_idx0, *corr_idx1, *corr_idx2;
    float *corr_score;
    float *ratio;
    int32_t *cell;
    int32_t *cell_sorted;
    double *gpf_quota;
    int32_t *gpf_cells;
    uint8_t *gpf_keep;
    float *gpf_f;
    int32_t *prosac_G;
    int32_t *prosac_rank;
    float *corr8;
    float *models;
    double *models64;
    int32_t *model_h;
    float *models2; double *models64_2; int32_t *model_h2;
    uint32_t *score_cnt;
    unsigned long long *score_ssq;
    double *refit_part;
    int32_t *lo_list;
    void *lo_ctl;
    void *sc_info;
    float *corr8s;
    int32_t *sc_perm;
    float *models_s;
    int32_t *sc_glen;
    uint8_t *sc_mb, *sc_cb;
    lr_ransac_result *res_tmp;
    double *T_tmp;
    int32_t *icp_ints;
    int32_t *icp_bucket;
    float *icp_pts;
    double *icp_state, *icp_part;
    lr_stage_timer timer;
};

struct lr_call {
    lr_workspace *ws;
    hipStream_t st;
    int pairs;
    lr_zargs z;
    bool armed;
};
static inline lr_call lr_call_single(lr_workspace *ws, void *stream) { return lr_call{ ws, (hipStream_t)stream, 1, lr_zargs{ 0, nullptr }, ws->timer.armed() }; }
static inline lr_call lr_call_batch(lr_workspace *ws, void *stream, int pairs) { return lr_call{ ws, (hipStream_t)stream, pairs, lr_zargs{ ws->stride, ws->descs }, ws->timer.armed() }; }

enum {
    LR_CNT_FIX = 0,
    LR_CNT_FIX_TOTAL,
    LR_CNT_NCORR,
    LR_CNT_NVALID,
    LR_CNT_NBB,
    LR_CNT_NREV,
    LR_CNT_RLO,
    LR_CNT_RHI,
    LR_CNT_REFIT_TICKET,
    LR_CNT_NVALID2,
    LR_CNT_FORM_MISS_F,
    LR_CNT_FORM_MISS_R,
    LR_CNT_COUNT = 16,
    LR_CNT_TOTAL = 64
};

__host__ __device__ inline size_t lr_corr_at(int c, int k) { return (size_t)(c >> 1) * 16 + 2 * k + (c & 1); }

struct lr_ransac_state {
    double T[12];
    unsigned long long ssq;
    long long n_valid, n_ids;
    uint32_t cnt;
    int32_t h;
    int32_t done;
    int32_t lo_pending;
    int32_t lo_calls;
    int32_t lo_timeouts;
    double sprt_eps, sprt_delta;
    unsigned long long rej_inl, rej_pts;
    unsigned long long evals, evals_full;
};
static_assert(sizeof(lr_ransac_state) <= (LR_CNT_TOTAL - LR_CNT_COUNT) * sizeof(int32_t), "lr_ransac_state does not fit");

int lr_zero_scratch(const lr_call &c, void *p, size_t bytes);
int lr_check_memory_device(const void *mem, hipStream_t st, const char *who, int *n_cus);
int lr_timer_mark(const lr_call &c, lr_event e);

int lr_nn16_prep(const lr_call &c, const float *F0, int n0, const float *F1, int n1, bool zero_counters = false);
int lr_nn16_run(const lr_call &c, const float *F0, int n0, const float *F1, int n1,
                int32_t *idx1, int32_t *idx2, float *s1, float *s2, bool seed_reverse = false);
int lr_nn16_reverse(const lr_call &c, const float *F0, int n0, const float *F1, int n1, const int32_t *fwd_idx1, int32_t *rev, bool seeded = false);

int lr_mutual_run(const lr_call &c, int n0, const int32_t *idx1, const int32_t *idx2, const int32_t *rev,
                  uint8_t *is_bb, int32_t *o0, int32_t *o1, int32_t *o2, int32_t *n_out,
                  const float *xyz0 = nullptr, const float *xyz1 = nullptr, float *corr8 = nullptr);
int lr_identity_corr(const lr_call &c, int n0, const int32_t *idx1, const int32_t *idx2,
                     int32_t *o0, int32_t *o1, int32_t *o2, int32_t *n_out);
int lr_pack_corr(const lr_call &c, const float *xyz0, const float *xyz1, const int32_t *i0, const int32_t *i1, int m_max,
                 const int32_t *m_dev, float *corr8, const int32_t *rank = nullptr);
int lr_prosac_order(const lr_call &c, const float *F0, const float *F1, int dim, const float *quality, int m_max, const int32_t *m_dev);
struct lr_gpf_subset { const int32_t *mb_dev, *b0; int32_t *has_score; double max_matches; };
int lr_gpf_run(const lr_call &c, const float *F0, int n0, const float *F1, int dim,
               const int32_t *idx1, const int32_t *idx2, const uint8_t *is_bb, const float *xyz0,
               int grid_wid, double factor, int32_t *o0, int32_t *o1, int32_t *o2, float *oscore,
               int32_t *n_out, const float *xyz1 = nullptr, float *corr8 = nullptr, const lr_gpf_subset *sub = nullptr);

int lr_icp_run(const lr_call &c, const float *xyz0, int n0, const float *xyz1, int n1, const double *T_init,
               const lr_ransac_result *gate, double max_dist, int max_iter, double rel_fit, double rel_rmse,
               double *T_out, lr_icp_result *res);

int lr_ransac_run(const lr_call &c, const float *corr8, int m_max, const int32_t *m_dev, const lr_ransac_params *p,
                  double *T_out, lr_ransac_result *res);
int lr_inlier_mask_run(const float *src, const float *tgt, const int32_t *i0, const int32_t *i1, int m_max, const int32_t *m_dev,
                       const double *T, float thr2, uint8_t *mask, int32_t *n_inliers, hipStream_t st);
int lr_refit_run(const lr_call &c, const float *xyz0, int n0, const float *xyz1, const int32_t *idx1,
                 const double *T_in, double thr2, double *T_out, int32_t *n_inl, const lr_ransac_result *gate,
                 lr_pair_result *pair_out = nullptr, const int32_t *idx0 = nullptr, const int32_t *m_dev = nullptr,
                 const float *F0 = nullptr, const float *F1 = nullptr);
```

### lidarregistration_amd/csrc/lr_nn16.hip

```cpp
#include "lr_internal.h"
#include <math.h>
#include <stdlib.h>
#include <type_traits>

typedef float f32x4 __attribute__((ext_vector_type(4)));
typedef float f32x2 __attribute__((ext_vector_type(2)));
typedef _Float16 f16x8 __attribute__((ext_vector_type(8)));

#define LR_INF __builtin_huge_valf()
#define LR_IMAX 0x7fffffff

__device__ __forceinline__ uint32_t lr_ord_enc(float v) { const uint32_t b = __float_as_uint(v); return (b & 0x80000000u) ? ~b : (b | 0x80000000u); }
__device__ __forceinline__ float lr_ord_dec(uint32_t u) { return __uint_as_float((u & 0x80000000u) ? (u & 0x7fffffffu) : ~u); }
#define LR_ORD_INF 0xff800000u

__global__ void __launch_bounds__(256)
nn16_prep_kernel(const float *__restrict__ Fa, int na, _Float16 *__restrict__ Ha, float *__restrict__ nrma, float *__restrict__ bmaxa, float *__restrict__ bmina,
                 const float *__restrict__ Fb, int nb, _Float16 *__restrict__ Hb, float *__restrict__ nrmb, float *__restrict__ bmaxb, float *__restrict__ bminb,
                 uint32_t *__restrict__ seed_b, unsigned long long *__restrict__ seed64_b, int32_t *__restrict__ counters, int zero_counters, int nblk_a,
                 uint32_t *__restrict__ yshare_a, lr_zargs z)
{
    __shared__ float s_m[4], s_n[4];
    if (z.descs) { const lr_pair_desc d = z.descs[blockIdx.z]; Fa = d.F0; na = d.n0; Fb = d.F1; nb = d.n1; }
    lr_z(bmina, z, blockIdx.z); lr_z(bminb, z, blockIdx.z);
    lr_z(Ha, z, blockIdx.z); lr_z(nrma, z, blockIdx.z); lr_z(bmaxa, z, blockIdx.z); lr_z(Hb, z, blockIdx.z); lr_z(nrmb, z, blockIdx.z);
    lr_z(bmaxb, z, blockIdx.z); lr_z(seed_b, z, blockIdx.z); lr_z(seed64_b, z, blockIdx.z); lr_z(counters, z, blockIdx.z); lr_z(yshare_a, z, blockIdx.z);
    if (counters && blockIdx.x == 0 && (int)threadIdx.x < LR_CNT_TOTAL) {
        const int k = threadIdx.x;
        if (k == LR_CNT_RLO) counters[k] = 0x7f7f7f7f;
        else if (k == LR_CNT_RHI || k == LR_CNT_FORM_MISS_F || k == LR_CNT_FORM_MISS_R || zero_counters) counters[k] = 0;
    }
    const bool second = (int)blockIdx.x >= nblk_a;
    const float *__restrict__ F = second ? Fb : Fa;
    _Float16 *__restrict__ H = second ? Hb : Ha;
    float *__restrict__ nrm = second ? nrmb : nrma;
    float *__restrict__ block_max = second ? bmaxb : bmaxa;
    float *__restrict__ block_min = second ? bminb : bmina;
    const int n = second ? nb : na;
    const int blk = second ? blockIdx.x - nblk_a : blockIdx.x;
    const int gid = blk * 256 + threadIdx.x;
    const int row = gid >> 3, t = gid & 7, lane = threadIdx.x & 63;
    const bool live = row < n;
    f32x4 v = { 0.0f, 0.0f, 0.0f, 0.0f };
    if (live) v = reinterpret_cast<const f32x4 *>(F + (size_t)row * 32)[t];
    float run = 0.0f;
#pragma unroll
    for (int s = 0; s < 8; ++s) {
        float in = __shfl(run, (lane & ~7) | (s > 0 ? s - 1 : 0));
        if (s == 0) in = 0.0f;
        float out = __builtin_fmaf(v.x, v.x, in);
        out = __builtin_fmaf(v.y, v.y, out);
        out = __builtin_fmaf(v.z, v.z, out);
        out = __builtin_fmaf(v.w, v.w, out);
        if (t == s) run = out;
    }
    const float norm = __shfl(run, (lane & ~7) | 7);
    if (live) {
        if (t == 0) {
            nrm[row] = norm;
            if (!second && yshare_a) yshare_a[row] = LR_ORD_INF;
            if (second && seed_b) { seed_b[row] = 0x7f7f7f7fu; seed64_b[row] = ~0ull; }
        }
        const int pos = 4 * t;
        typedef _Float16 f16x4 __attribute__((ext_vector_type(4)));
        f16x4 hv = { (_Float16)v.x, (_Float16)v.y, (_Float16)v.z, (_Float16)v.w };
        *reinterpret_cast<f16x4 *>(H + (size_t)row * 32 + pos) = hv;
    }
    float m = live ? norm : 0.0f, mn = live ? ((norm - norm == 0.0f) ? norm : -1.0f) : LR_INF;
#pragma unroll
    for (int k = 32; k >= 1; k >>= 1) { m = fmaxf(m, __shfl_xor(m, k)); mn = fminf(mn, __shfl_xor(mn, k)); }
    if (lane == 0) { s_m[threadIdx.x >> 6] = m; s_n[threadIdx.x >> 6] = mn; }
    __syncthreads();
    if (threadIdx.x == 0) {
        block_max[blk] = fmaxf(fmaxf(s_m[0], s_m[1]), fmaxf(s_m[2], s_m[3]));
        if (block_min) block_min[blk] = fminf(fminf(s_n[0], s_n[1]), fminf(s_n[2], s_n[3]));
    }
}

__global__ void __launch_bounds__(256)
nn16_range_kernel(int na, const float *__restrict__ bmaxa, const float *__restrict__ bmina, int nb, const float *__restrict__ bmaxb,
                  const float *__restrict__ bminb, float *__restrict__ range, int32_t *__restrict__ form_out, lr_zargs z)
{
    __shared__ float s_m[4], s_n[4];
    if (z.descs) { na = z.descs[blockIdx.z].n0; nb = z.descs[blockIdx.z].n1; }
    lr_z(bmaxa, z, blockIdx.z); lr_z(bmina, z, blockIdx.z); lr_z(bmaxb, z, blockIdx.z); lr_z(bminb, z, blockIdx.z); lr_z(range, z, blockIdx.z);
    const bool second = blockIdx.x == 1;
    const float *__restrict__ bmax = second ? bmaxb : bmaxa, *__restrict__ bmin = second ? bminb : bmina;
    const int nblk = ((second ? nb : na) + 31) >> 5;
    float mx = 0.0f, mn = LR_INF;
    for (int b = threadIdx.x; b < nblk; b += 256) { mx = fmaxf(mx, bmax[b]); mn = fminf(mn, bmin[b]); }
#pragma unroll
    for (int k = 32; k >= 1; k >>= 1) { mx = fmaxf(mx, __shfl_xor(mx, k)); mn = fminf(mn, __shfl_xor(mn, k)); }
    if ((threadIdx.x & 63) == 0) { s_m[threadIdx.x >> 6] = mx; s_n[threadIdx.x >> 6] = mn; }
    __syncthreads();
    if (threadIdx.x == 0) {
        const float hi = fmaxf(fmaxf(s_m[0], s_m[1]), fmaxf(s_m[2], s_m[3])), lo = fminf(fminf(s_n[0], s_n[1]), fminf(s_n[2], s_n[3]));
        range[2 * second] = hi;
        range[2 * second + 1] = lo;
        if (form_out) form_out[second] = (lo > 0.0f && hi < LR_INF && hi - lo <= 1e-4f * hi) ? 1 : 2;
    }
}

#define LR_LDS_ROW 64
__device__ __forceinline__ int lr_lds_off(int j, int p) { return j * LR_LDS_ROW + ((p ^ ((j >> 1) & 3)) << 4); }
#define LR_BLOCK_ROWS 256
#define LR_PB_CH 4
#define LR_PB_WLIST 512
#define LR_PB_COLMASK 0x3fffffu
#define LR_PB_HASG 0x1000000u
#define LR_PB_DGROUPS 3
#define LR_PB_TIGHTEN 48

__device__ __forceinline__ int lr_pb_row(int kb, int b) { return 16 * (b >> 2) + 4 * kb + (b & 3); }
__device__ __forceinline__ int lr_pb_kb(unsigned x) { return (int)(x >> 22) & 3; }

#define LR_RS_BUCKETS 4096

__device__ __forceinline__ int rs_bucket(float v, float lo, float scale)
{
    const int b = (int)((v - lo) * scale);
    return min(max(b, 0), LR_RS_BUCKETS - 1);
}
__device__ __forceinline__ float rs_scale(float lo, float hi) { return hi > lo ? (float)LR_RS_BUCKETS / (hi - lo) : 0.0f; }

struct lr_thr_in {
    const float *nQ;
    const float *range_c;
    int need, sstride;
};
struct lr_pb_grid { int gx, gy, total, dir, only; };
struct lr_ex_out {
    int32_t *idx1, *idx2;
    float *s1o, *s2o;
    uint32_t *seed_out;
    float *seed_s1;
    uint32_t *seed_range;
    unsigned long long *seed64;
};
struct lr_pb_tail {
    unsigned long long *clk;
};
__device__ __forceinline__ lr_pb_tail lr_pb_tail_args()
{
    auto ka = __builtin_amdgcn_kernarg_segment_ptr();
    asm volatile("" : "+s"(ka) :: "memory");
    typedef const unsigned long long __attribute__((opencl_constant)) *cw_t;
    static_assert(sizeof(lr_pb_tail) == 8, "read as one 64-bit word");
    lr_pb_tail t;
    const unsigned long long w = *(cw_t)ka;
    __builtin_memcpy(&t, &w, sizeof t);
    return t;
}

#define LR_EX_EMPTY 0xffffffffffffffffull
__device__ __forceinline__ void ex_offer(unsigned long long *best, unsigned long long *second, float sv, int j)
{
    const unsigned long long key = ((unsigned long long)__float_as_uint(sv) << 32) | (unsigned)j;
    const unsigned long long old = atomicMin(best, key);
    atomicMin(second, old > key ? old : key);
}
__device__ __forceinline__ void ex_write_row(const lr_ex_out &o, int rowd, unsigned long long kb, unsigned long long ks, int nb, int need, float &sv, float &key)
{
    const int i1 = kb == LR_EX_EMPTY ? -1 : (int)(unsigned)kb;
    const float b1 = kb == LR_EX_EMPTY ? LR_INF : __uint_as_float((unsigned)(kb >> 32));
    o.idx1[rowd] = i1;
    if (o.idx2) o.idx2[rowd] = ks == LR_EX_EMPTY ? (nb > 1 ? LR_IMAX : -1) : (int)(unsigned)ks;
    if (o.s1o) o.s1o[rowd] = b1;
    if (o.s2o) o.s2o[rowd] = ks == LR_EX_EMPTY ? LR_INF : __uint_as_float((unsigned)(ks >> 32));
    if (o.seed_out) {
        sv = b1;
        if (!(sv < 3.0e38f)) sv = 3.0e38f;
        if (i1 >= 0 && i1 < nb) {
            atomicMin(&o.seed_out[i1], __float_as_uint(sv));
            atomicMin(&o.seed64[i1], ((unsigned long long)__float_as_uint(sv) << 32) | (unsigned)rowd);
        }
        key = sv;
        if (need >= 2) { key = ks == LR_EX_EMPTY ? 3.0e38f : __uint_as_float((unsigned)(ks >> 32)); if (!(key < 3.0e38f)) key = 3.0e38f; }
        o.seed_s1[rowd] = key;
    }
}
__device__ __forceinline__ void ex_range(const lr_ex_out &o, bool writer, float sv, float key, int lane)
{
    float lo = writer ? sv : 3.0e38f, hi = writer ? fmaxf(sv, key) : 0.0f;
#pragma unroll
    for (int k = 32; k >= 1; k >>= 1) { lo = fminf(lo, __shfl_xor(lo, k)); hi = fmaxf(hi, __shfl_xor(hi, k)); }
    if (lane == 0) {
        atomicMin(&o.seed_range[0], __float_as_uint(lo));
        atomicMax(&o.seed_range[1], __float_as_uint(hi));
    }
}
__device__ __forceinline__ bool ex_bad8(const f32x4 &u, const f32x4 &v)
{
    const float big = fmaxf(fmaxf(fmaxf(fabsf(u.x), fabsf(u.y)), fmaxf(fabsf(u.z), fabsf(u.w))), fmaxf(fmaxf(fabsf(v.x), fabsf(v.y)), fmaxf(fabsf(v.z), fabsf(v.w))));
    return !(big <= 65504.0f) || u.x != u.x || u.y != u.y || u.z != u.z || u.w != u.w || v.x != v.x || v.y != v.y || v.z != v.z || v.w != v.w;
}

#ifdef LR_PB_PROBE
__device__ unsigned long long lr_pb_stat[16];
#define LR_PROBE(...) __VA_ARGS__
#else
#define LR_PROBE(...)
#endif
#define LR_PB_WAVES 3
template <bool SIGN>
__global__ void __launch_bounds__(256) __attribute__((amdgpu_waves_per_eu(LR_PB_WAVES, LR_PB_WAVES)))
nn16_passb_kernel(lr_pb_tail tail_first , unsigned long long *clk_on,
                  const _Float16 *__restrict__ Hq, int na_host, const int32_t *__restrict__ rowmap, const int32_t *__restrict__ na_dev,
                  const _Float16 *__restrict__ Hc, const float *__restrict__ nC, int nb,
                  int tiles_per_strip, const float *__restrict__ tau, int32_t *__restrict__ cand_cnt, int32_t *__restrict__ cand,
                  const int32_t *__restrict__ colmap, const float *__restrict__ tile_min, const uint32_t *__restrict__ row_bound,
                  const int32_t *__restrict__ rev_offs, const uint32_t *__restrict__ rev_range, float *__restrict__ yfin, int yfin_stride,
                  uint32_t *__restrict__ yshare, int32_t *__restrict__ form_miss, lr_thr_in thr, lr_pb_grid pg, lr_zargs z)
{
    int logical;
    if (!lr_xcd_block(pg.total, logical)) return;
    const int bx = logical % pg.gx, by = (logical / pg.gx) % pg.gy, pair = logical / (pg.gx * pg.gy);
    if (z.descs) {
        const lr_pair_desc d = z.descs[pair];
        na_host = pg.dir ? d.n1 : d.n0; nb = pg.dir ? d.n0 : d.n1;
    }
    lr_z(Hq, z, pair); lr_z(rowmap, z, pair); lr_z(na_dev, z, pair); lr_z(Hc, z, pair); lr_z(nC, z, pair); lr_z(tau, z, pair);
    lr_z(cand_cnt, z, pair); lr_z(cand, z, pair); lr_z(colmap, z, pair); lr_z(tile_min, z, pair); lr_z(row_bound, z, pair); lr_z(rev_offs, z, pair); lr_z(rev_range, z, pair);
    lr_z(thr.nQ, z, pair); lr_z(thr.range_c, z, pair); lr_z(yfin, z, pair); lr_z(yshare, z, pair);
    const int na = na_dev ? *na_dev : na_host;
    if (bx * LR_BLOCK_ROWS >= na) return;
    float max_nc = 0.0f, min_nc = 0.0f;
    if (thr.range_c) { max_nc = thr.range_c[0]; min_nc = thr.range_c[1]; }
    const bool sign_ok = thr.range_c != nullptr && min_nc > 0.0f && max_nc < LR_INF && max_nc - min_nc <= 1e-4f * max_nc && true;
    if (sign_ok != SIGN) {
        if (pg.only && form_miss && bx == 0 && by == 0 && threadIdx.x == 0) { lr_z(form_miss, z, pair); *form_miss = 1; }
        return;
    }
    const float xhat = SIGN ? 0.5f * min_nc : 0.0f;
    __shared__ int s_limit[4];
    __shared__ unsigned long long s_clk[2];
    if (clk_on && threadIdx.x == 0) { s_clk[0] = __builtin_amdgcn_s_memtime(); s_clk[1] = __builtin_amdgcn_s_memrealtime(); }
    constexpr int CH = LR_PB_CH;
    constexpr int XOFF = CH * 32 * LR_LDS_ROW;
    constexpr int BUF = XOFF + (SIGN ? 0 : CH * 32 * 4);
    __shared__ __attribute__((aligned(16))) unsigned char lds_a[BUF];
    __shared__ __attribute__((aligned(16))) unsigned char lds_b[BUF];
    constexpr int WL = (LR_PB_CH >= 8 && !SIGN) ? (LR_PB_WLIST * 7) / 8 : LR_PB_WLIST;
    __shared__ uint2 wlist[4][WL];
    __shared__ __attribute__((aligned(16))) float s_Y[LR_BLOCK_ROWS];
    __shared__ float s_D[LR_BLOCK_ROWS], s_N1[LR_BLOCK_ROWS], s_N2[LR_BLOCK_ROWS];
    __shared__ unsigned s_att[2];
    const int tid = threadIdx.x, wave = __builtin_amdgcn_readfirstlane(tid >> 6), lane = tid & 63;
    const int c16 = lane & 15, kb = lane >> 4;
    const int row0 = bx * LR_BLOCK_ROWS + wave * 64;
    LR_PROBE(int n_visits = 0, n_hits = 0, n_rounds = 0, n_groups = 0, n_tk_derive = 0, n_tk_flush = 0, n_tk_a = 0, n_tk_b = 0;
             const unsigned long long tk_start = __builtin_amdgcn_s_memrealtime(); unsigned long long tk_walk = 0;)
    int ntiles = (nb + 31) >> 5;
    int my_strips = pg.gy;
    if (tile_min) {
        if (tid == 0) {
            const float lo = __uint_as_float(rev_range[0]), scale = rs_scale(lo, __uint_as_float(rev_range[1]));
            const float sv = __uint_as_float(row_bound[rowmap[bx * LR_BLOCK_ROWS]]);
            const int b = rs_bucket(sv, lo, scale);
            s_limit[0] = ((b + 1 < LR_RS_BUCKETS ? rev_offs[b + 1] : nb) + 31) >> 5;
        }
        __syncthreads();
        ntiles = min(ntiles, s_limit[0]);
        my_strips = min(pg.gy, (ntiles + tiles_per_strip - 1) / tiles_per_strip);
        if (by >= my_strips) return;
        tiles_per_strip = (ntiles + my_strips - 1) / my_strips;
    }
    const int t_begin = by * tiles_per_strip;
    const int t_end = min(ntiles, t_begin + tiles_per_strip);
    const int nchunks = t_end > t_begin ? (t_end - t_begin + CH - 1) / CH : 0;

    f16x8 a16[4];
#pragma unroll
    for (int rbk = 0; rbk < 4; ++rbk) {
        int row = min(row0 + 16 * rbk + c16, na - 1);
        if (rowmap) row = rowmap[row];
        a16[rbk] = *reinterpret_cast<const f16x8 *>(Hq + (size_t)row * 32 + 8 * kb);
    }

    f32x4 stage[CH / 2];
    float stage_n = 0.0f;

    {
        const int rw = bx * LR_BLOCK_ROWS + tid;
        float Dv = LR_INF;
        if (thr.nQ && rw < na) {
            const float scale = thr.nQ[rowmap ? rowmap[rw] : rw] + max_nc;
            Dv = (1.05e-3f * scale + 4e-7f) + 8e-6f * scale;
        }
        s_D[tid] = Dv; s_N1[tid] = -LR_INF; s_N2[tid] = -LR_INF;
        if (tau) s_Y[tid] = rw < na ? 0.5f * tau[rw] : -LR_INF;
        else {
            const int sstride = thr.sstride;
            const int nsamp = t_end > t_begin ? (t_end - t_begin + sstride - 1) / sstride : 0;
            const int nsch = (nsamp + CH - 1) / CH;
            constexpr bool P1E = SIGN;
            auto tile_s = [&](int c, int k) { return t_begin + (c * CH + k) * sstride; };
            auto load_s = [&](int c) {
#pragma unroll
                for (int q = 0; q < CH / 2; ++q) {
                    const int p = tid + 256 * q;
                    const int col = tile_s(c, p >> 7) * 32 + ((p >> 2) & 31);
                    stage[q] = *reinterpret_cast<const f32x4 *>(reinterpret_cast<const unsigned char *>(Hc) + (size_t)min(col, nb - 1) * 64 + (p & 3) * 16);
                }
                const int lc = tid & (CH * 32 - 1);
                const int col = tile_s(c, lc >> 5) * 32 + (lc & 31);
                if constexpr (!P1E) stage_n = nC[min(col, nb - 1)];
            };
            auto store_s = [&](int buf) {
#pragma unroll
                for (int q = 0; q < CH / 2; ++q) {
                    const int p = tid + 256 * q;
                    *reinterpret_cast<f32x4 *>(&(buf ? lds_b : lds_a)[lr_lds_off(p >> 2, p & 3)]) = stage[q];
                }
                if constexpr (P1E) return;
                float xm = 0.5f * stage_n;
#pragma unroll
                for (int k = 16; k >= 1; k >>= 1) xm = fmaxf(xm, __shfl_xor(xm, k));
                if (tid < CH * 32 && (tid & 31) == 0) *reinterpret_cast<float *>(&(buf ? lds_b : lds_a)[XOFF + (tid >> 5) * 4]) = xm;
            };
            float m1[4], m2[4];
#pragma unroll
            for (int rbk = 0; rbk < 4; ++rbk) { m1[rbk] = -LR_INF; m2[rbk] = -LR_INF; }
            f32x4 runm[4];
#pragma unroll
            for (int rbk = 0; rbk < 4; ++rbk) runm[rbk] = f32x4{ -LR_INF, -LR_INF, -LR_INF, -LR_INF };
            auto fold = [&](const f32x4 &lo4, const f32x4 &hi4, int rbk, float xmax) {
                if constexpr (P1E) {
                    asm("v_max3_f32 %0, %0, %4, %8\n\tv_max3_f32 %1, %1, %5, %9\n\tv_max3_f32 %2, %2, %6, %10\n\tv_max3_f32 %3, %3, %7, %11"
                        : "+v"(runm[rbk][0]), "+v"(runm[rbk][1]), "+v"(runm[rbk][2]), "+v"(runm[rbk][3])
                        : "v"(lo4[0]), "v"(lo4[1]), "v"(lo4[2]), "v"(lo4[3]), "v"(hi4[0]), "v"(hi4[1]), "v"(hi4[2]), "v"(hi4[3]));
                    return;
                }
                float t, lo;
                asm("v_max3_f32 %0, %2, %3, %4\n\tv_max3_f32 %0, %0, %5, %6\n\tv_max3_f32 %0, %0, %7, %8\n\tv_max_f32 %0, %0, %9\n\t"
                    "v_sub_f32 %0, %0, %10\n\tv_min_f32 %1, %11, %0"
                    : "=&v"(t), "=&v"(lo)
                    : "v"(lo4[0]), "v"(lo4[1]), "v"(lo4[2]), "v"(lo4[3]), "v"(hi4[0]), "v"(hi4[1]), "v"(hi4[2]), "v"(hi4[3]), "v"(xmax), "v"(m1[rbk]));
                asm("v_max_f32 %0, %0, %1" : "+v"(m1[rbk]) : "v"(t));
                asm("v_max_f32 %0, %0, %1" : "+v"(m2[rbk]) : "v"(lo));
            };
            const f32x4 zero4 = { 0, 0, 0, 0 };
            const int frag16s = lr_lds_off(c16, kb);
            f32x4 sA[8], sB[8];
            bool pend = false;
            float pend_x = 0.0f;
            if (nsch > 0) {
                load_s(0); store_s(0);
                __syncthreads();
                for (int c = 0; c < nsch; ++c) {
                    const int buf = c & 1;
                    if (c + 1 < nsch) load_s(c + 1);
                    const unsigned char *lbuf = buf ? lds_b : lds_a;
                    const unsigned char *bp = &lbuf[frag16s];
                    f16x8 b0 = *reinterpret_cast<const f16x8 *>(bp), b1 = *reinterpret_cast<const f16x8 *>(bp + 16 * LR_LDS_ROW);
                    float xmax = *reinterpret_cast<const float *>(&lbuf[XOFF]);
#pragma unroll
                    for (int k = 0; k < CH; ++k) {
                        f16x8 n0 = b0, n1 = b1; float nx = xmax;
                        if (k + 1 < CH) {
                            n0 = *reinterpret_cast<const f16x8 *>(bp + (k + 1) * 32 * LR_LDS_ROW);
                            n1 = *reinterpret_cast<const f16x8 *>(bp + (k + 1) * 32 * LR_LDS_ROW + 16 * LR_LDS_ROW);
                            nx = *reinterpret_cast<const float *>(&lbuf[XOFF + (k + 1) * 4]);
                        }
                        f32x4 (&cur)[8] = (k & 1) ? sB : sA;
                        const f32x4 (&prev)[8] = (k & 1) ? sA : sB;
                        __builtin_amdgcn_sched_barrier(0);
#pragma unroll
                        for (int rbk = 0; rbk < 4; ++rbk) {
                            cur[rbk] = __builtin_amdgcn_mfma_f32_16x16x32_f16(b0, a16[rbk], zero4, 0, 0, 0);
                            cur[4 + rbk] = __builtin_amdgcn_mfma_f32_16x16x32_f16(b1, a16[rbk], zero4, 0, 0, 0);
                        }
                        __builtin_amdgcn_sched_barrier(0);
                        if (pend) {
#pragma unroll
                            for (int rbk = 0; rbk < 4; ++rbk) fold(prev[rbk], prev[4 + rbk], rbk, pend_x);
                        }
                        __builtin_amdgcn_sched_barrier(0);
                        pend = tile_s(c, k) < t_end && (tile_s(c, k) + 1) * 32 <= nb;
                        pend_x = xmax;
                        b0 = n0; b1 = n1; xmax = nx;
                    }
                    if (c + 1 < nsch) store_s(buf ^ 1);
                    __syncthreads();
                }
                if (pend) {
                    asm volatile("s_nop 15\n\ts_nop 15" ::: "memory");
#pragma unroll
                    for (int rbk = 0; rbk < 4; ++rbk) fold(sB[rbk], sB[4 + rbk], rbk, pend_x);
                }
            }
            if constexpr (P1E) {
                const float xg = 0.5f * max_nc;
#pragma unroll
                for (int rbk = 0; rbk < 4; ++rbk) {
                    const float a = fmaxf(runm[rbk][0], runm[rbk][1]), b = fminf(runm[rbk][0], runm[rbk][1]);
                    const float c = fmaxf(runm[rbk][2], runm[rbk][3]), d = fminf(runm[rbk][2], runm[rbk][3]);
                    m1[rbk] = fmaxf(a, c) - xg;
                    m2[rbk] = fmaxf(fminf(a, c), fmaxf(b, d)) - xg;
                }
            }
#pragma unroll
            for (int rbk = 0; rbk < 4; ++rbk) {
#pragma unroll
                for (int o = 16; o <= 32; o <<= 1) {
                    const float c1 = __shfl_xor(m1[rbk], o), c2 = __shfl_xor(m2[rbk], o);
                    const float hi = fmaxf(m1[rbk], c1), lo = fminf(m1[rbk], c1);
                    m2[rbk] = fmaxf(lo, fmaxf(m2[rbk], c2));
                    m1[rbk] = hi;
                }
                const int rl = wave * 64 + 16 * rbk + c16, row = bx * LR_BLOCK_ROWS + rl;
                if (kb == 0) {
                    float yv = -LR_INF;
                    if (row < na) {
                        const float U = -2.0f * (thr.need >= 2 ? m2[rbk] : m1[rbk]);
                        const float scale = thr.nQ[rowmap ? rowmap[row] : row] + max_nc;
                        const float E = 1.05e-3f * scale + 4e-7f;
                        yv = 0.5f * (U + 2.0f * E + 6e-6f * scale + 2e-6f * fabsf(U));
                    }
                    s_Y[rl] = yv;
                }
            }
        }
        __syncthreads();
    }
    const bool pooled = yshare != nullptr && thr.nQ != nullptr && my_strips > 1;
    if (pooled) {
        const int rw = bx * LR_BLOCK_ROWS + tid;
        if (rw < na) {
            const float yv = s_Y[tid];
            if (yv == yv) { const float other = lr_ord_dec(atomicMin(&yshare[rw], lr_ord_enc(yv))); if (other < yv) s_Y[tid] = other; }
        }
        __syncthreads();
    }

    f32x4 y4[4];
    auto load_y = [&]() {
#pragma unroll
        for (int rbk = 0; rbk < 4; ++rbk) y4[rbk] = *reinterpret_cast<const f32x4 *>(&s_Y[wave * 64 + 16 * rbk + 4 * kb]);
#pragma unroll
        for (int rbk = 0; rbk < 4; ++rbk) y4[rbk] -= xhat;
    };
    load_y();
    LR_PROBE(tk_walk = __builtin_amdgcn_s_memrealtime();)
    static_assert(CH % 4 == 0, "the staging maps 4 waves onto groups of 16 columns");
    constexpr int NQ = CH * 2 / 4;
    const __amdgpu_buffer_rsrc_t rsrcH = __builtin_amdgcn_make_buffer_rsrc(const_cast<_Float16 *>(Hc), 0, nb * 64, 0x27000);
    const __amdgpu_buffer_rsrc_t rsrcN = __builtin_amdgcn_make_buffer_rsrc(const_cast<float *>(nC), 0, nb * 4, 0x27000);
    const int ld_voff = wave * NQ * 1024 + (lane >> 2) * 64 + (((lane & 3) ^ ((lane >> 3) & 3)) << 4);
    const int st_noff = (tid & (CH * 32 - 1)) * 4;
    auto load_chunk = [&](auto bufc, int c) {
        constexpr int buf = decltype(bufc)::value;
        const int col0 = (t_begin + c * CH) * 32;
        __attribute__((address_space(3))) void *dst = (__attribute__((address_space(3))) void *)((buf ? lds_b : lds_a) + wave * NQ * 1024);
        static_assert(NQ == 2 || NQ == 4, "chunks of 4 or 8 tiles");
        __builtin_amdgcn_raw_ptr_buffer_load_lds(rsrcH, dst, 16, ld_voff, col0 * 64, 0, 0);
        __builtin_amdgcn_raw_ptr_buffer_load_lds(rsrcH, dst, 16, ld_voff, col0 * 64, 1024, 0);
        if constexpr (NQ == 4) {
            __builtin_amdgcn_raw_ptr_buffer_load_lds(rsrcH, dst, 16, ld_voff, col0 * 64, 2048, 0);
            __builtin_amdgcn_raw_ptr_buffer_load_lds(rsrcH, dst, 16, ld_voff, col0 * 64, 3072, 0);
        }
        if constexpr (!SIGN) stage_n = __builtin_bit_cast(float, __builtin_amdgcn_raw_buffer_load_b32(rsrcN, st_noff, col0 * 4, 0));
    };
    auto finish_chunk = [&](auto bufc, int c) {
        constexpr int buf = decltype(bufc)::value;
        if constexpr (!SIGN) {
            const int col = (t_begin + c * CH) * 32 + (tid & (CH * 32 - 1));
            const bool ok = col < nb && (col >> 5) < t_end;
            if (tid < CH * 32) *reinterpret_cast<float *>(&(buf ? lds_b : lds_a)[XOFF + tid * 4]) = ok ? 0.5f * stage_n : LR_INF;
        }
    };
    typedef std::integral_constant<int, 0> c0_t;
    typedef std::integral_constant<int, 1> c1_t;
    const int frag16 = lr_lds_off(c16, kb), x_lane = XOFF + c16 * 4;
    auto read_b = [&](auto bufc, int k, f16x8 &b0, f16x8 &b1, f32x2 &xj) {
        constexpr int buf = decltype(bufc)::value;
        const unsigned char *lbuf = buf ? lds_b : lds_a;
        b0 = *reinterpret_cast<const f16x8 *>(&lbuf[frag16 + k * 32 * LR_LDS_ROW]);
        b1 = *reinterpret_cast<const f16x8 *>(&lbuf[frag16 + k * 32 * LR_LDS_ROW + 16 * LR_LDS_ROW]);
        if constexpr (!SIGN) {
            xj.x = *reinterpret_cast<const float *>(&lbuf[x_lane + k * 32 * 4]);
            xj.y = *reinterpret_cast<const float *>(&lbuf[x_lane + k * 32 * 4 + 64]);
        }
    };
    int wcnt = 0;
    const unsigned lanecode = (unsigned)c16 | ((unsigned)kb << 22);
    auto cold_lane = [&]() { int l; asm volatile("v_mbcnt_lo_u32_b32 %0, -1, 0\n\tv_mbcnt_hi_u32_b32 %0, -1, %0" : "=v"(l)); return l; };
    int wdone = 0;
    int trig = LR_PB_TIGHTEN;
    int wposted = 0, wnext = 0;
    const int seg_cap = lr_seg_cap(my_strips);
    uint2 *__restrict__ seg = reinterpret_cast<uint2 *>(cand) + (size_t)(bx * 4 + wave) * LR_NN16_SEG + (size_t)by * seg_cap;
    int seg_fill = 0;
    const bool tightening = thr.nQ != nullptr;
    auto my_wish = [&]() { return (wcnt >= WL / 2 ? 2 : 0) | ((tightening && wcnt - wdone >= trig) ? 1 : 0); };
    auto set_next = [&]() { wnext = tightening ? min(wdone + trig, WL / 2) : WL / 2; };
    set_next();
    auto derive = [&](bool update) {
        const int lane = cold_lane(), c16 = lane & 15, kb = lane >> 4;
        const int nlist = min(wcnt, WL);
        __builtin_amdgcn_s_setprio(3);
        LR_PROBE(++n_rounds; n_groups += (nlist - wdone + 15) >> 4; const unsigned long long tk0 = __builtin_amdgcn_s_memrealtime();)
        constexpr int DG = SIGN ? LR_PB_DGROUPS : (LR_PB_DGROUPS > 2 ? 2 : LR_PB_DGROUPS);
        for (int e0 = wdone; e0 < nlist; e0 += 16 * DG) {
            uint2 v[DG]; f16x8 bf[DG]; float xn[DG];
#pragma unroll
            for (int g = 0; g < DG; ++g) {
                v[g] = wlist[wave][min(e0 + 16 * g + c16, WL - 1)];
                const int col = (int)(v[g].x & LR_PB_COLMASK);
                bf[g] = __builtin_bit_cast(f16x8, __builtin_amdgcn_raw_buffer_load_b128(rsrcH, col * 64 + kb * 16, 0, 0));
                xn[g] = __builtin_bit_cast(float, __builtin_amdgcn_raw_buffer_load_b32(rsrcN, col * 4, 0, 0));
            }
            LR_PROBE({ const unsigned long long ta = __builtin_amdgcn_s_memrealtime(); asm volatile("s_waitcnt vmcnt(0)" ::: "memory"); n_tk_a += (int)(__builtin_amdgcn_s_memrealtime() - ta); })
#pragma unroll
            for (int g = 0; g < DG; ++g) {
                if (e0 + 16 * g >= nlist) break;
                const int e = e0 + 16 * g + c16;
                const bool valid = e < nlist;
                const int col = (int)(v[g].x & LR_PB_COLMASK);
                const float x = (valid && col < nb && (col >> 5) < t_end) ? 0.5f * xn[g] - xhat : LR_INF;
                f32x4 d[4];
#pragma unroll
                for (int rbk = 0; rbk < 4; ++rbk) d[rbk] = __builtin_amdgcn_mfma_f32_16x16x32_f16(a16[rbk], bf[g], y4[rbk], 0, 0, 0);
                if (valid && lr_pb_kb(v[g].x) == kb) {
                    unsigned mask = 0u;
#pragma unroll
                    for (int rbk = 0; rbk < 4; ++rbk)
#pragma unroll
                        for (int k = 0; k < 4; ++k) mask |= (d[rbk][k] < x) ? 0u : (1u << (4 * rbk + k));
                    uint2 w = make_uint2(v[g].x, mask);
                    if (update && mask != 0u && (mask & (mask - 1u)) == 0u) {
                        const int b = __builtin_ctz(mask);
                        const int rl = wave * 64 + lr_pb_row(kb, b);
                        float m = fmaxf(fmaxf(fmaxf(d[0][0], d[0][1]), fmaxf(d[0][2], d[0][3])), fmaxf(fmaxf(d[1][0], d[1][1]), fmaxf(d[1][2], d[1][3])));
                        m = fmaxf(m, fmaxf(fmaxf(fmaxf(d[2][0], d[2][1]), fmaxf(d[2][2], d[2][3])), fmaxf(fmaxf(d[3][0], d[3][1]), fmaxf(d[3][2], d[3][3]))));
                        const float gv = (m - x) - s_Y[rl];
                        const float old = atomicMax(&s_N1[rl], gv);
                        atomicMax(&s_N2[rl], fminf(old, gv));
                        const unsigned gb = __float_as_uint(gv);
                        const unsigned up16 = (gb & 0x80000000u) ? (gb >> 16) : ((gb + 0xffffu) >> 16);
                        w.y |= up16 << 16;
                        w.x |= LR_PB_HASG;
                    }
                    wlist[wave][e] = w;
                }
            }
        }
        LR_PROBE(const unsigned long long tb = __builtin_amdgcn_s_memrealtime();)
        wdone = nlist;
        if (false && update) trig = min(2 * trig, 192);
        set_next();
        if (update) {
            const int rl = wave * 64 + lane;
            const float gn = thr.need >= 2 ? s_N2[rl] : s_N1[rl];
            const float yn = (s_D[rl] - gn) + 2e-6f * fabsf(gn);
            float yv = s_Y[rl];
            if (yn < yv) yv = yn;
            if (pooled && row0 + lane < na && yv == yv) {
                const float other = lr_ord_dec(atomicMin(&yshare[row0 + lane], lr_ord_enc(yv)));
                if (other < yv) yv = other;
            }
            s_Y[rl] = yv;
            load_y();
        }
        LR_PROBE(asm volatile("s_waitcnt vmcnt(0) lgkmcnt(0)" ::: "memory"); n_tk_b += (int)(__builtin_amdgcn_s_memrealtime() - tb); n_tk_derive += (int)(__builtin_amdgcn_s_memrealtime() - tk0);)
        __builtin_amdgcn_s_setprio(0);
    };
    auto flush = [&]() {
        if (wdone < wcnt) derive(tightening);
        const int lane = cold_lane();
        LR_PROBE(const unsigned long long tkf = __builtin_amdgcn_s_memrealtime();)
        if (wcnt > WL) seg_fill = -1;
        else if (seg_fill >= 0) {
            for (int e0 = 0; e0 < wcnt; e0 += 64) {
                const int e = e0 + lane;
                uint2 v = make_uint2(0u, 0u);
                if (e < wcnt) v = wlist[wave][e];
                const int col = (int)(v.x & LR_PB_COLMASK);
                bool keep = e < wcnt && (v.y & 0xffffu) != 0u && col < nb && (col >> 5) < t_end;
                if (v.x & LR_PB_HASG) {
                    const float gv = __uint_as_float(v.y & 0xffff0000u);
                    const int rl = wave * 64 + lr_pb_row(lr_pb_kb(v.x), __builtin_ctz((v.y & 0xffffu) | 0x8000u));
                    const float yr = s_Y[rl];
                    if (gv + 1e-5f * (fabsf(gv) + fabsf(yr)) < -yr) keep = false;
                }
                const unsigned long long kb = __builtin_amdgcn_ballot_w64(keep);
                const int pos = seg_fill + (int)__builtin_amdgcn_mbcnt_hi((unsigned)(kb >> 32), __builtin_amdgcn_mbcnt_lo((unsigned)kb, 0u));
                const int nk = __builtin_popcountll(kb);
                if (seg_fill + nk > seg_cap) { seg_fill = -1; break; }
                if (keep) { if (colmap) v.x = (unsigned)colmap[col] | (v.x & ~LR_PB_COLMASK); seg[pos] = v; }
                seg_fill += nk;
            }
        }
        wcnt = 0; wdone = 0; set_next();
        LR_PROBE(n_tk_flush += (int)(__builtin_amdgcn_s_memrealtime() - tkf);)
    };
    auto check = [&](const f32x4 &r0, const f32x4 &r1, const f32x4 &r2, const f32x4 &r3, float x, int tile, int cb) {
        bool mine_hit;
        if constexpr (SIGN) {
            int sa, sb;
            asm("v_bitop3_b32 %0, %2, %3, %4 bitop3:0x80\n\tv_bitop3_b32 %1, %10, %11, %12 bitop3:0x80\n\t"
                "v_bitop3_b32 %0, %0, %5, %6 bitop3:0x80\n\tv_bitop3_b32 %1, %1, %13, %14 bitop3:0x80\n\t"
                "v_bitop3_b32 %0, %0, %7, %8 bitop3:0x80\n\tv_bitop3_b32 %1, %1, %15, %16 bitop3:0x80\n\t"
                "v_bitop3_b32 %0, %0, %1, %9 bitop3:0x80\n\tv_and_b32 %0, %0, %17"
                : "=&v"(sa), "=&v"(sb)
                : "v"(r0[0]), "v"(r0[1]), "v"(r0[2]), "v"(r0[3]), "v"(r1[0]), "v"(r1[1]), "v"(r1[2]), "v"(r1[3]),
                  "v"(r2[0]), "v"(r2[1]), "v"(r2[2]), "v"(r2[3]), "v"(r3[0]), "v"(r3[1]), "v"(r3[2]), "v"(r3[3]));
            mine_hit = sa >= 0;
        } else {
            float ma, mb;
            asm("v_max3_f32 %0, %2, %3, %4\n\tv_max3_f32 %1, %10, %11, %12\n\t"
                "v_max3_f32 %0, %0, %5, %6\n\tv_max3_f32 %1, %1, %13, %14\n\t"
                "v_max3_f32 %0, %0, %7, %8\n\tv_max3_f32 %1, %1, %15, %16\n\t"
                "v_max3_f32 %0, %0, %1, %9\n\tv_max_f32 %0, %0, %17"
                : "=&v"(ma), "=&v"(mb)
                : "v"(r0[0]), "v"(r0[1]), "v"(r0[2]), "v"(r0[3]), "v"(r1[0]), "v"(r1[1]), "v"(r1[2]), "v"(r1[3]),
                  "v"(r2[0]), "v"(r2[1]), "v"(r2[2]), "v"(r2[3]), "v"(r3[0]), "v"(r3[1]), "v"(r3[2]), "v"(r3[3]));
            mine_hit = ma >= x;
        }
        const unsigned long long hit = __builtin_amdgcn_ballot_w64(mine_hit);
        if (__builtin_expect(hit != 0ull, 0)) {
            if (mine_hit) {
                const int pos = wcnt + (int)__builtin_amdgcn_mbcnt_hi((unsigned)(hit >> 32), __builtin_amdgcn_mbcnt_lo((unsigned)hit, 0u));
                unsigned lc = lanecode;
                if constexpr (!SIGN) { const int ln = cold_lane(); lc = (unsigned)(ln & 15) | ((unsigned)(ln >> 4) << 22); }
                if (pos < WL) wlist[wave][pos] = make_uint2((unsigned)(tile * 32 + cb * 16) | lc, 0u);
            }
            wcnt += __builtin_popcountll(hit);
            LR_PROBE(++n_visits; n_hits += __builtin_popcountll(hit);)
        }
    };

    f16x8 b0, b1;
    f32x2 xN = { LR_INF, LR_INF }, xC = { LR_INF, LR_INF };
    f32x4 acc[4][2];
#pragma unroll
    for (int q = 0; q < 4; ++q)
#pragma unroll
        for (int cb = 0; cb < 2; ++cb)
#pragma unroll
            for (int g = 0; g < 4; ++g) acc[q][cb][g] = -LR_INF;

    auto step = [&](int c, int k, auto parc) {
        constexpr int par = decltype(parc)::value;
        f16x8 n0, n1; f32x2 nx;
        if (k + 1 < CH) read_b(std::integral_constant<int, par>{}, k + 1, n0, n1, nx);
        else read_b(std::integral_constant<int, par ^ 1>{}, 0, n0, n1, nx);
        const int tileC = t_begin + c * CH + k - 1;
#define MF(rbk, cb, b) acc[rbk][cb] = __builtin_amdgcn_mfma_f32_16x16x32_f16(a16[rbk], b, y4[rbk], 0, 0, 0)
        check(acc[0][0], acc[1][0], acc[2][0], acc[3][0], xC.x, tileC, 0);
        __builtin_amdgcn_sched_barrier(0);
        MF(0, 0, b0); MF(1, 0, b0); MF(2, 0, b0); MF(3, 0, b0);
        __builtin_amdgcn_sched_barrier(0);
        check(acc[0][1], acc[1][1], acc[2][1], acc[3][1], xC.y, tileC, 1);
        __builtin_amdgcn_sched_barrier(0);
        MF(0, 1, b1); MF(1, 1, b1); MF(2, 1, b1); MF(3, 1, b1);
        __builtin_amdgcn_sched_barrier(0);
#undef MF
        b0 = n0; b1 = n1; xC = xN; xN = nx;
    };
    auto drain = [&]() {
        const int tileC = t_begin + nchunks * CH - 1;
        check(acc[0][0], acc[1][0], acc[2][0], acc[3][0], xC.x, tileC, 0);
        check(acc[0][1], acc[1][1], acc[2][1], acc[3][1], xC.y, tileC, 1);
    };
    if (nchunks > 0) {
        load_chunk(c0_t{}, 0);
        __builtin_amdgcn_s_waitcnt(0x0F70);
        finish_chunk(c0_t{}, 0);
        if (nchunks > 1) load_chunk(c1_t{}, 1);
        if (tid == 0) s_att[0] = 0u;
        __syncthreads();
        read_b(c0_t{}, 0, b0, b1, xN);
        int c = 0;
        int wish = 0;
        auto chunk = [&](auto parc, auto tailc) {
            constexpr int par = decltype(parc)::value;
            constexpr bool tail = decltype(tailc)::value != 0;
            unsigned wishes = 0u;
#pragma unroll
            for (int k = 0; k < CH; ++k) {
                if (k == CH - 1) {
                    if (!tail || c + 1 < nchunks) { __builtin_amdgcn_s_waitcnt(0x0F70); finish_chunk(std::integral_constant<int, par ^ 1>{}, c + 1); }
                    if (__builtin_expect(wcnt >= wnext, 0)) {
                        const int wm = my_wish();
                        if (lane == 0) reinterpret_cast<unsigned char *>(&s_att[0])[wave] = (unsigned char)wm;
                        wposted = wm; wnext = 0x7fffffff;
                    }
                    __syncthreads();
                    wishes = s_att[0];
                    if (!tail || c + 2 < nchunks) load_chunk(std::integral_constant<int, par>{}, c + 2);
                }
                step(c, k, parc);
            }
            wish = (int)__builtin_amdgcn_readfirstlane(wishes);
            ++c;
        };
        typedef std::integral_constant<int, 0> body_t;
        typedef std::integral_constant<int, 1> tail_t;
        while (c < nchunks) {
            wish = 0;
            if (c & 1) chunk(c1_t{}, tail_t{});
            else if (c + 3 < nchunks) {
                do { chunk(c0_t{}, body_t{}); if (wish) break; chunk(c1_t{}, body_t{}); } while (!wish && c + 3 < nchunks);
            } else chunk(c0_t{}, tail_t{});
            wish = (wish & 0x02020202) ? 2 : (wish ? 1 : 0);
            if (wish && wposted) { if (lane == 0) reinterpret_cast<unsigned char *>(&s_att[0])[wave] = 0; wposted = 0; }
            if (wish & 2) flush();
            else if (wish) { if (wdone < wcnt) derive(true); }
        }
        asm volatile("s_nop 15\n\ts_nop 15" ::: "memory");
        drain();
        flush();
    }
    if (lane == 0) {
        int32_t *cw = cand_cnt + (bx * 4 + wave) * (pg.gy + 1);
        cw[by] = seg_fill;
        if (by == 0) cw[pg.gy] = my_strips;
    }
    LR_PROBE(if (lane == 0) {
        atomicAdd(&lr_pb_stat[0], 1ull); atomicAdd(&lr_pb_stat[1], (unsigned long long)nchunks * CH * 4); atomicAdd(&lr_pb_stat[2], (unsigned long long)n_visits);
        atomicAdd(&lr_pb_stat[3], (unsigned long long)n_hits); atomicAdd(&lr_pb_stat[4], (unsigned long long)n_rounds); atomicAdd(&lr_pb_stat[5], (unsigned long long)n_groups);
        const unsigned long long tk_end = __builtin_amdgcn_s_memrealtime();
        atomicAdd(&lr_pb_stat[6], (unsigned long long)n_tk_derive); atomicAdd(&lr_pb_stat[7], (unsigned long long)n_tk_flush);
        atomicAdd(&lr_pb_stat[8], tk_walk - tk_start); atomicAdd(&lr_pb_stat[9], tk_end - tk_start);
        atomicAdd(&lr_pb_stat[10], (unsigned long long)n_tk_a); atomicAdd(&lr_pb_stat[11], (unsigned long long)n_tk_b);
    })
    if (yfin) {
        const int rw = row0 + lane;
        if (rw < na) yfin[(size_t)by * yfin_stride + rw] = tightening ? s_Y[wave * 64 + lane] : LR_INF;
    }
    if (threadIdx.x == 0) {
        const lr_pb_tail tl = lr_pb_tail_args();
        if (tl.clk) {
            atomicAdd(&tl.clk[0], __builtin_amdgcn_s_memtime() - s_clk[0]);
            atomicAdd(&tl.clk[1], __builtin_amdgcn_s_memrealtime() - s_clk[1]);
        }
    }
}

#define LR_EX_ROWS 64
#define LR_EX_STRIDE 33

__global__ void __launch_bounds__(256)
nn16_exact_kernel(const float *__restrict__ Fq, const float *__restrict__ nQ, int na,
                  const float *__restrict__ Fc, const float *__restrict__ nC, int nb,
                  const int32_t *__restrict__ cand_cnt, const int32_t *__restrict__ cand, int nstrips, int need,
                  const float *__restrict__ yfin, int yfin_stride,
                  const int32_t *__restrict__ rowmap, const int32_t *__restrict__ na_dev, lr_ex_out out,
                  int32_t *__restrict__ counters, const float *__restrict__ range_c, int dir, int gx, int total, lr_zargs z)
{
    int logical;
    if (!lr_xcd_block(total, logical)) return;
    const int bxi = logical % gx, pair = logical / gx;
    __shared__ float s_a[LR_EX_ROWS * LR_EX_STRIDE];
    __shared__ float s_nq[LR_EX_ROWS];
    __shared__ unsigned long long s_best[LR_EX_ROWS], s_second[LR_EX_ROWS];
    __shared__ int s_cnt[LR_EX_ROWS], s_rowd[LR_EX_ROWS], s_badrow[LR_EX_ROWS];
    __shared__ int s_bad, s_skip, s_nredo, s_redo[LR_EX_ROWS];
    if (z.descs) {
        const lr_pair_desc d = z.descs[pair];
        Fq = dir ? d.F1 : d.F0; na = dir ? d.n1 : d.n0; Fc = dir ? d.F0 : d.F1; nb = dir ? d.n0 : d.n1;
    }
    lr_z(nQ, z, pair); lr_z(nC, z, pair); lr_z(cand_cnt, z, pair); lr_z(cand, z, pair); lr_z(rowmap, z, pair); lr_z(yfin, z, pair);
    lr_z(na_dev, z, pair); lr_z(out.idx1, z, pair); lr_z(out.idx2, z, pair); lr_z(out.s1o, z, pair); lr_z(out.s2o, z, pair);
    lr_z(counters, z, pair); lr_z(out.seed_out, z, pair); lr_z(out.seed_s1, z, pair); lr_z(out.seed_range, z, pair); lr_z(out.seed64, z, pair); lr_z(range_c, z, pair);
    unsigned long long *__restrict__ const seed64 = out.seed64;
    if (na_dev) na = *na_dev;
    const int row0 = bxi * LR_EX_ROWS;
    if (row0 >= na) return;
    const int tid = threadIdx.x;
    const int miss = counters[LR_CNT_FORM_MISS_F + (dir ? 1 : 0)] != 0 ? 1 : 0;
    {
        const int rl = tid >> 2, part = tid & 3;
        const int rowc = min(row0 + rl, na - 1);
        const int rowd = rowmap ? rowmap[rowc] : rowc;
        const f32x4 *pa = reinterpret_cast<const f32x4 *>(Fq + (size_t)rowd * 32 + 8 * part);
        const f32x4 u = pa[0], v = pa[1];
        float *dst = &s_a[rl * LR_EX_STRIDE + 8 * part];
        dst[0] = u.x; dst[1] = u.y; dst[2] = u.z; dst[3] = u.w; dst[4] = v.x; dst[5] = v.y; dst[6] = v.z; dst[7] = v.w;
        const bool bad = ex_bad8(u, v);
        if (tid < LR_EX_ROWS) { s_best[tid] = LR_EX_EMPTY; s_second[tid] = LR_EX_EMPTY; s_cnt[tid] = 0; s_badrow[tid] = 0; }
        if (tid == 0) {
            s_bad = ((range_c != nullptr && range_c[1] < 0.0f) || miss) ? 1 : 0; s_skip = miss; s_nredo = 0;
        }
        if (part == 0) { s_nq[rl] = nQ[rowd]; s_rowd[rl] = rowd; }
        __syncthreads();
        if (bad) s_badrow[rl] = 1;
        if (dir == 1 && seed64 && tid < LR_EX_ROWS && row0 + tid < na) { s_best[tid] = seed64[s_rowd[tid]]; s_cnt[tid] = 1; }
    }
    __syncthreads();
    auto dist = [&](int rl, const f32x4 (&t)[8], float ncj) {
        const float *a = &s_a[rl * LR_EX_STRIDE];
        float acc = 0.0f;
#pragma unroll
        for (int k = 0; k < 8; ++k) {
            acc = __builtin_fmaf(a[4 * k], t[k].x, acc);
            acc = __builtin_fmaf(a[4 * k + 1], t[k].y, acc);
            acc = __builtin_fmaf(a[4 * k + 2], t[k].z, acc);
            acc = __builtin_fmaf(a[4 * k + 3], t[k].w, acc);
        }
        const float d2 = __builtin_fmaf(-2.0f, acc, s_nq[rl] + ncj);
        return __builtin_sqrtf(fmaxf(d2, 1e-30f));
    };
    if (!s_skip) {
        const int32_t *cw = cand_cnt + bxi * (nstrips + 1);
        const int used = min(max(cw[nstrips], 1), nstrips);
        const int seg_cap = lr_seg_cap(used);
        __shared__ float s_yf[LR_EX_ROWS];
        if (tid < LR_EX_ROWS) {
            float yv = LR_INF;
            if (yfin && row0 + tid < na) for (int sidx = 0; sidx < used; ++sidx) yv = fminf(yv, yfin[(size_t)sidx * yfin_stride + row0 + tid]);
            s_yf[tid] = yv;
        }
        __syncthreads();
        const uint2 *__restrict__ segs = reinterpret_cast<const uint2 *>(cand) + (size_t)bxi * LR_NN16_SEG;
        for (int sidx = 0; sidx < used; ++sidx) {
            const int c = cw[sidx];
            if (c < 0) { if (tid == 0) s_bad = 1; continue; }
            for (int e = tid; e < c; e += 256) {
                const uint2 v = segs[(size_t)sidx * seg_cap + e];
                const int j = (int)(v.x & LR_PB_COLMASK), ekb = lr_pb_kb(v.x);
                if (v.x & LR_PB_HASG) {
                    const int rl = lr_pb_row(ekb, __builtin_ctz((v.y & 0xffffu) | 0x8000u));
                    const float gv = __uint_as_float(v.y & 0xffff0000u), yr = s_yf[rl];
                    if (gv + 1e-5f * (fabsf(gv) + fabsf(yr)) < -yr) continue;
                }
                f32x4 t[8];
                const f32x4 *pb = reinterpret_cast<const f32x4 *>(Fc + (size_t)j * 32);
#pragma unroll
                for (int k = 0; k < 8; ++k) t[k] = pb[k];
                const float ncj = nC[j];
                unsigned m = v.y & 0xffffu;
                while (m) {
                    const int bit = __builtin_ctz(m);
                    m &= m - 1;
                    const int rl = lr_pb_row(ekb, bit);
                    ex_offer(&s_best[rl], &s_second[rl], dist(rl, t, ncj), j);
                    atomicAdd(&s_cnt[rl], 1);
                }
            }
        }
    }
    __syncthreads();
    if (tid < LR_EX_ROWS && row0 + tid < na && (s_bad || s_badrow[tid] || s_cnt[tid] < min(need, nb))) s_redo[atomicAdd(&s_nredo, 1)] = tid;
    __syncthreads();
    const int nredo = s_nredo;
    for (int r = 0; r < nredo; ++r) {
        const int rl = s_redo[r];
        if (tid == 0) { s_best[rl] = LR_EX_EMPTY; s_second[rl] = LR_EX_EMPTY; atomicAdd(&counters[LR_CNT_FIX_TOTAL], 1); }
        __syncthreads();
        for (int j = tid; j < nb; j += 256) {
            f32x4 t[8];
            const f32x4 *pb = reinterpret_cast<const f32x4 *>(Fc + (size_t)j * 32);
#pragma unroll
            for (int k = 0; k < 8; ++k) t[k] = pb[k];
            ex_offer(&s_best[rl], &s_second[rl], dist(rl, t, nC[j]), j);
        }
    }
    __syncthreads();
    float sv = 3.0e38f, key = 0.0f;
    const bool writer = tid < LR_EX_ROWS && row0 + tid < na;
    if (writer) ex_write_row(out, s_rowd[tid], s_best[tid], s_second[tid], nb, need, sv, key);
    if (out.seed_out && tid < 64) ex_range(out, writer, sv, key, tid);
}

int lr_nn16_prep(const lr_call &c, const float *F0, int n0, const float *F1, int n1, bool zero_counters)
{
    lr_workspace *ws = c.ws;
    hipLaunchKernelGGL(nn16_prep_kernel, dim3(lr_cdiv(n0, 32) + lr_cdiv(n1, 32), 1, c.pairs), dim3(256), 0, c.st, F0, n0, ws->H0, ws->nrm0, ws->bmax0, ws->bmin0,
                       F1, n1, ws->H1, ws->nrm1, ws->bmax1, ws->bmin1, ws->rev_seed, ws->rev_seed64, ws->counters, zero_counters ? 1 : 0, lr_cdiv(n0, 32), ws->yshare, c.z);
    hipLaunchKernelGGL(nn16_range_kernel, dim3(2, 1, c.pairs), dim3(256), 0, c.st, n0, (const float *)ws->bmax0, (const float *)ws->bmin0, n1, (const float *)ws->bmax1,
                       (const float *)ws->bmin1, ws->nn_range, c.pairs == 1 ? ws->form_dev : (int32_t *)nullptr, c.z);
    LR_LAUNCH_CHECK();
    return LR_OK;
}

static int lr_nn16_form_hint(const lr_call &c, int col_cloud)
{
    lr_workspace *ws = c.ws;
    if (c.pairs != 1 || !ws->form_host) return 0;
    const int h = *reinterpret_cast<const volatile int32_t *>(&ws->form_host[col_cloud]);
    const int prev = ws->form_prev[col_cloud];
    ws->form_prev[col_cloud] = h;
    return ((h == 1 || h == 2) && h == prev) ? h : 0;
}

struct lr_pb_args {
    const _Float16 *Hq; int na; const int32_t *rowmap, *na_dev;
    const _Float16 *Hc; const float *nC; int nb, tps;
    const float *tau;
    const int32_t *colmap; const float *tile_min; const uint32_t *row_bound; const int32_t *rev_offs; const uint32_t *rev_range;
    float *yfin; int yfin_stride; uint32_t *yshare;
    lr_thr_in thr;
    int row_blocks, strips, dir;
};
static int lr_nn16_passb(const lr_call &c, const lr_pb_args &a)
{
    lr_workspace *ws = c.ws;
    const int total = a.row_blocks * a.strips * c.pairs;
    const dim3 grid(8 * lr_cdiv(total, 8));
    LR_TRY_HIP(lr_timer_mark(c, a.dir ? LR_EV_REV_FILTER_BEGIN : LR_EV_FWD_FILTER_BEGIN));
    const int only = lr_nn16_form_hint(c, a.dir ? 0 : 1);
    int32_t *miss = ws->counters + (a.dir ? LR_CNT_FORM_MISS_R : LR_CNT_FORM_MISS_F);
    unsigned long long *clk = ws->clock_probe ? ws->clk_dev : (unsigned long long *)nullptr;
    const lr_pb_tail tl = { clk };
    const lr_pb_grid pg = { a.row_blocks, a.strips, total, a.dir, only };
    auto launch = [&](auto kernel) {
        hipLaunchKernelGGL(kernel, grid, dim3(256), 0, c.st, tl, clk, a.Hq, a.na, a.rowmap, a.na_dev, a.Hc, a.nC, a.nb, a.tps, a.tau, ws->cand_cnt, ws->cand,
                           a.colmap, a.tile_min, a.row_bound, a.rev_offs, a.rev_range, a.yfin, a.yfin_stride, a.yshare, miss, a.thr, pg, c.z);
    };
    if (only != 2) launch(nn16_passb_kernel<true>);
    if (only != 1) launch(nn16_passb_kernel<false>);
    return lr_timer_mark(c, a.dir ? LR_EV_REV_FILTER_END : LR_EV_FWD_FILTER_END);
}

int lr_nn16_run(const lr_call &c, const float *Fq, int na, const float *Fc, int nb,
                int32_t *idx1, int32_t *idx2, float *s1, float *s2, bool seed_reverse)
{
    lr_workspace *ws = c.ws;
    const float *nQ = ws->nrm0, *nC = ws->nrm1, *range_c = ws->nn_range + 2;
    const int need = idx2 ? 2 : 1;
    const int ntiles = lr_cdiv(nb, 32);
    const int row_blocks = lr_cdiv(na, LR_BLOCK_ROWS);
    int strips = c.pairs > 1 ? lr_cdiv(ws->nn_blocks_batch, row_blocks * c.pairs) : ws->nn_blocks_target / row_blocks;
    int smax = ntiles / 64;
    if (strips > smax) strips = smax;
    if (strips > LR_NN_MAX_STRIPS) strips = LR_NN_MAX_STRIPS;
    if (strips < 1) strips = 1;
    const int tps = lr_cdiv(ntiles, strips);
    int sstride = ws->nn_sample_stride > 0 ? ws->nn_sample_stride : (strips > 1 ? ntiles / 64 : tps / 32);
    if (ws->nn_sample_stride <= 0) { const int cap = strips > 1 ? 16 : 32; if (sstride > cap) sstride = cap; }
    if (sstride < 1) sstride = 1;
    if (sstride > tps) sstride = tps;
    lr_pb_args a = {};
    a.Hq = ws->H0; a.na = na; a.Hc = ws->H1; a.nC = nC; a.nb = nb; a.tps = tps;
    a.yfin = ws->yfin; a.yfin_stride = ws->max_n; a.yshare = ws->yshare;
    a.thr = lr_thr_in{ nQ, range_c, need, sstride };
    a.row_blocks = row_blocks; a.strips = strips; a.dir = 0;
    LR_TRY_HIP(lr_nn16_passb(c, a));
    const lr_ex_out eo = { idx1, idx2, s1, idx2 ? s2 : (float *)nullptr, seed_reverse ? ws->rev_seed : (uint32_t *)nullptr, ws->rev_s1,
                           reinterpret_cast<uint32_t *>(ws->counters + LR_CNT_RLO), ws->rev_seed64 };
    const int ex_gx = lr_cdiv(na, LR_EX_ROWS), ex_total = ex_gx * c.pairs;
    hipLaunchKernelGGL(nn16_exact_kernel, dim3(8 * lr_cdiv(ex_total, 8)), dim3(256), 0, c.st, Fq, nQ, na, Fc, nC, nb, ws->cand_cnt, ws->cand,
                       strips, need, (const float *)ws->yfin, ws->max_n, (const int32_t *)nullptr, (const int32_t *)nullptr, eo, ws->counters,
                       range_c, 0, ex_gx, ex_total, c.z);
    LR_LAUNCH_CHECK();
    return LR_OK;
}

__global__ void __launch_bounds__(256)
nn16_rev_seed_kernel(const float *__restrict__ F0, const float *__restrict__ n0v, int n0, const float *__restrict__ F1,
                     const float *__restrict__ n1v, const int32_t *__restrict__ idx1, uint32_t *__restrict__ seed_bits,
                     float *__restrict__ s1, uint32_t *__restrict__ range)
{
    __shared__ float s_lo[4], s_hi[4];
    const int i = blockIdx.x * 256 + threadIdx.x;
    float sv = 0.0f;
    if (i < n0) {
    const int j = idx1[i];
    const f32x4 *pa = reinterpret_cast<const f32x4 *>(F0 + (size_t)i * 32);
    const f32x4 *pb = reinterpret_cast<const f32x4 *>(F1 + (size_t)j * 32);
    float acc = 0.0f;
#pragma unroll
    for (int k = 0; k < 8; ++k) {
        const f32x4 a = pa[k], b = pb[k];
        acc = __builtin_fmaf(a.x, b.x, acc);
        acc = __builtin_fmaf(a.y, b.y, acc);
        acc = __builtin_fmaf(a.z, b.z, acc);
        acc = __builtin_fmaf(a.w, b.w, acc);
    }
    const float d2 = __builtin_fmaf(-2.0f, acc, n0v[i] + n1v[j]);
    sv = __builtin_sqrtf(fmaxf(d2, 1e-30f));
    if (!(sv < 3.0e38f)) sv = 3.0e38f;
    atomicMin(&seed_bits[j], __float_as_uint(sv));
    s1[i] = sv;
    }
    float lo = i < n0 ? sv : 3.0e38f, hi = i < n0 ? sv : 0.0f;
#pragma unroll
    for (int k = 32; k >= 1; k >>= 1) { lo = fminf(lo, __shfl_xor(lo, k)); hi = fmaxf(hi, __shfl_xor(hi, k)); }
    if ((threadIdx.x & 63) == 0) { s_lo[threadIdx.x >> 6] = lo; s_hi[threadIdx.x >> 6] = hi; }
    __syncthreads();
    if (threadIdx.x == 0) {
        atomicMin(&range[0], __float_as_uint(fminf(fminf(s_lo[0], s_lo[1]), fminf(s_lo[2], s_lo[3]))));
        atomicMax(&range[1], __float_as_uint(fmaxf(fmaxf(s_hi[0], s_hi[1]), fmaxf(s_hi[2], s_hi[3]))));
    }
}

#define LR_RO_ROUND 8192
#define LR_RO_QUEUE 3072
__global__ void __launch_bounds__(1024)
nn16_rev_order_kernel(int n0, int n1, const float *__restrict__ s1, const uint32_t *__restrict__ seed_bits, const uint32_t *__restrict__ range,
                      int32_t *__restrict__ offs, int32_t *__restrict__ n_rows, const float *__restrict__ block_max_c, int nblk_c,
                      const float *__restrict__ nrm1, const _Float16 *__restrict__ H0, const float *__restrict__ nrm0, int32_t *__restrict__ colmap,
                      _Float16 *__restrict__ H0s, float *__restrict__ nrm0s, int32_t *__restrict__ rowmap, float *__restrict__ tau,
                      int32_t *__restrict__ cand_cnt, int32_t *__restrict__ rev_out, int seg_counters, lr_zargs z)
{
    __shared__ int s_pos[2 * LR_RS_BUCKETS];
    __shared__ int2 s_q[LR_RO_QUEUE];
    __shared__ float s_m[16];
    __shared__ int s_w[16], s_own[4], s_nq, s_nrows;
    if (z.descs) { n0 = z.descs[blockIdx.z].n0; n1 = z.descs[blockIdx.z].n1; nblk_c = (n0 + 31) >> 5; }
    lr_z(s1, z, blockIdx.z); lr_z(seed_bits, z, blockIdx.z); lr_z(range, z, blockIdx.z); lr_z(offs, z, blockIdx.z); lr_z(n_rows, z, blockIdx.z);
    lr_z(block_max_c, z, blockIdx.z); lr_z(nrm1, z, blockIdx.z); lr_z(H0, z, blockIdx.z); lr_z(nrm0, z, blockIdx.z); lr_z(colmap, z, blockIdx.z);
    lr_z(H0s, z, blockIdx.z); lr_z(nrm0s, z, blockIdx.z); lr_z(rowmap, z, blockIdx.z); lr_z(tau, z, blockIdx.z); lr_z(cand_cnt, z, blockIdx.z); lr_z(rev_out, z, blockIdx.z);
    const int tid = threadIdx.x, lane = tid & 63, part = blockIdx.x, parts = gridDim.x;
    for (int k = part * 1024 + tid; k < seg_counters; k += parts * 1024) cand_cnt[k] = 0;
    const float lo = __uint_as_float(range[0]), scale = rs_scale(lo, __uint_as_float(range[1]));
    for (int k = tid; k < 2 * LR_RS_BUCKETS; k += 1024) s_pos[k] = 0;
    if (tid < 4) s_own[tid] = (tid & 1) ? 0 : 0x7fffffff;
    if (tid == 0) s_nq = 0;
    float mx = 0.0f;
    for (int b = tid; b < nblk_c; b += 1024) mx = fmaxf(mx, block_max_c[b]);
#pragma unroll
    for (int k = 32; k >= 1; k >>= 1) mx = fmaxf(mx, __shfl_xor(mx, k));
    if (lane == 0) s_m[tid >> 6] = mx;
    __syncthreads();
    float max_nc = 0.0f;
#pragma unroll
    for (int w = 0; w < 16; ++w) max_nc = fmaxf(max_nc, s_m[w]);
    for (int i0 = tid; i0 < max(n0, n1); i0 += 8 * 1024) {
        float v[8]; uint32_t u[8];
#pragma unroll
        for (int k = 0; k < 8; ++k) { v[k] = s1[min(i0 + 1024 * k, n0 - 1)]; u[k] = seed_bits[min(i0 + 1024 * k, n1 - 1)]; }
#pragma unroll
        for (int k = 0; k < 8; ++k) {
            if (i0 + 1024 * k < n0) atomicAdd(&s_pos[rs_bucket(v[k], lo, scale)], 1);
            const float sv = __uint_as_float(u[k]);
            if (i0 + 1024 * k < n1 && sv <= 3.0e38f) atomicAdd(&s_pos[LR_RS_BUCKETS + (LR_RS_BUCKETS - 1 - rs_bucket(sv, lo, scale))], 1);
        }
    }
    __syncthreads();
    for (int side = 0; side < 2; ++side) {
        int *hp = s_pos + side * LR_RS_BUCKETS;
        int v[LR_RS_BUCKETS / 1024], sum = 0;
#pragma unroll
        for (int k = 0; k < LR_RS_BUCKETS / 1024; ++k) { v[k] = hp[tid * (LR_RS_BUCKETS / 1024) + k]; sum += v[k]; }
        int inc = sum;
#pragma unroll
        for (int d = 1; d < 64; d <<= 1) { const int o = __shfl_up(inc, d); if (lane >= d) inc += o; }
        if (lane == 63) s_w[tid >> 6] = inc;
        __syncthreads();
        int base = 0;
        for (int w = 0; w < (tid >> 6); ++w) base += s_w[w];
        int run = base + inc - sum;
#pragma unroll
        for (int k = 0; k < LR_RS_BUCKETS / 1024; ++k) {
            hp[tid * (LR_RS_BUCKETS / 1024) + k] = run;
            if (part == 0) offs[side * LR_RS_BUCKETS + tid * (LR_RS_BUCKETS / 1024) + k] = run;
            run += v[k];
        }
        if (side == 1 && tid == 1023) { s_nrows = run; if (part == 0) *n_rows = run; }
        __syncthreads();
    }
    {
        const long long nrows = s_nrows;
        for (int k = tid; k < 2 * LR_RS_BUCKETS; k += 1024) {
            const int side = k >= LR_RS_BUCKETS, kb = k & (LR_RS_BUCKETS - 1);
            const long long n = side ? nrows : (long long)n0, lo_p = (long long)part * n, hi_p = (long long)(part + 1) * n;
            auto own = [&](int idx) { const long long sp = (long long)s_pos[idx] * parts; return sp >= lo_p && sp < hi_p; };
            if (own(k)) {
                if (kb == 0 || !own(k - 1)) s_own[2 * side] = k;
                if (kb == LR_RS_BUCKETS - 1 || !own(k + 1)) s_own[2 * side + 1] = k + 1;
            }
        }
    }
    __syncthreads();
    const int c_lo = s_own[0], c_len = max(s_own[1] - s_own[0], 0), r_lo = s_own[2], r_len = max(s_own[3] - s_own[2], 0);
    constexpr int U = LR_RO_ROUND / 1024;
    auto move_row = [&](int i, int p, int piece) {
        reinterpret_cast<f32x4 *>(H0s + (size_t)p * 32)[piece] = reinterpret_cast<const f32x4 *>(H0 + (size_t)i * 32)[piece];
        if (piece == 0) { colmap[p] = i; nrm0s[p] = nrm0[i]; }
    };
    for (int i0 = 0; i0 < n0; i0 += LR_RO_ROUND) {
        float v[U];
#pragma unroll
        for (int k = 0; k < U; ++k) v[k] = s1[min(i0 + tid + 1024 * k, n0 - 1)];
#pragma unroll
        for (int k = 0; k < U; ++k) {
            const int i = i0 + tid + 1024 * k, b = rs_bucket(v[k], lo, scale);
            if (i < n0 && (unsigned)(b - c_lo) < (unsigned)c_len) {
                const int p = atomicAdd(&s_pos[b], 1), slot = atomicAdd(&s_nq, 1);
                if (slot < LR_RO_QUEUE) s_q[slot] = make_int2(i, p);
                else { for (int piece = 0; piece < 4; ++piece) move_row(i, p, piece); }
            }
        }
        __syncthreads();
        const int nq = min(s_nq, LR_RO_QUEUE);
        __syncthreads();
        if (tid == 0) s_nq = 0;
        for (int e = tid >> 2; e < nq; e += 256) { const int2 ip = s_q[e]; move_row(ip.x, ip.y, tid & 3); }
        __syncthreads();
    }
    constexpr int U1 = 16;
    for (int j0 = tid; j0 < n1; j0 += U1 * 1024) {
        uint32_t v[U1];
#pragma unroll
        for (int k = 0; k < U1; ++k) v[k] = seed_bits[min(j0 + 1024 * k, n1 - 1)];
#pragma unroll
        for (int k = 0; k < U1; ++k) {
            const int row = j0 + 1024 * k;
            if (row >= n1) continue;
            const float sv = __uint_as_float(v[k]);
            if (!(sv <= 3.0e38f)) {
                if ((row & (parts - 1)) == part) rev_out[row] = -1;
                continue;
            }
            const int b = LR_RS_BUCKETS + (LR_RS_BUCKETS - 1 - rs_bucket(sv, lo, scale));
            if ((unsigned)(b - r_lo) >= (unsigned)r_len) continue;
            const int p = atomicAdd(&s_pos[b], 1);
            const float nj = nrm1[row], scl = nj + max_nc;
            const float E = 1.05e-3f * scl + 4e-7f;
            const float d2hi = sv * sv * (1.0f + 6e-7f);
            rowmap[p] = row;
            tau[p] = (d2hi - nj) + E + 6e-6f * scl + 2e-6f * d2hi;
        }
    }
}

int lr_nn16_reverse(const lr_call &c, const float *F0, int n0, const float *F1, int n1, const int32_t *fwd_idx1, int32_t *rev, bool seeded)
{
    lr_workspace *ws = c.ws; hipStream_t st = c.st;
    const float *nrm0 = ws->nrm0, *nrm1 = ws->nrm1;
    const int na = n1, nb = n0;
    const int ntiles = lr_cdiv(nb, 32);
    const int row_blocks = lr_cdiv(na, LR_BLOCK_ROWS);
    int strips = ws->rev_strips > 0 ? ws->rev_strips : 48 / c.pairs;
    if (ws->rev_strips <= 0) { if (strips > 8) strips = 8; if (strips < 2) strips = 2; }
    int smax = ntiles / 8;
    if (strips > smax) strips = smax;
    if (strips < 1) strips = 1;
    const int tps = lr_cdiv(ntiles, strips);
    uint32_t *seed = ws->rev_seed;
    uint32_t *range = reinterpret_cast<uint32_t *>(ws->counters + LR_CNT_RLO);
    int32_t *n_rows = ws->counters + LR_CNT_NREV;
    if (!seeded)
        hipLaunchKernelGGL(nn16_rev_seed_kernel, dim3(lr_cdiv(n0, 256)), dim3(256), 0, st, F0, nrm0, n0, F1, nrm1, fwd_idx1, seed, ws->rev_s1, range);
    const int order_parts = c.pairs >= 16 ? 8 : c.pairs >= 4 ? 16 : 32;
    hipLaunchKernelGGL(nn16_rev_order_kernel, dim3(order_parts, 1, c.pairs), dim3(1024), 0, st, n0, n1, (const float *)ws->rev_s1, (const uint32_t *)seed,
                       (const uint32_t *)range, ws->rev_hist, n_rows, (const float *)ws->bmax0, lr_cdiv(nb, 32), nrm1, (const _Float16 *)ws->H0, nrm0, ws->rev_cols, ws->Hs, ws->nrms,
                       ws->rev_rows, ws->tau, ws->cand_cnt, rev, row_blocks * 4 * (strips + 1), c.z);
    lr_pb_args a = {};
    a.Hq = ws->H1; a.na = na; a.rowmap = ws->rev_rows; a.na_dev = n_rows; a.Hc = ws->Hs; a.nC = ws->nrms; a.nb = nb; a.tps = tps;
    a.tau = ws->tau;
    a.colmap = ws->rev_cols; a.tile_min = seeded ? ws->rev_tmin : nullptr; a.row_bound = seed; a.rev_offs = ws->rev_hist; a.rev_range = range;
    a.thr = lr_thr_in{ nullptr, ws->nn_range, 1, 0 };
    a.row_blocks = row_blocks; a.strips = strips; a.dir = 1;
    LR_TRY_HIP(lr_nn16_passb(c, a));
    const lr_ex_out reo = { rev, nullptr, nullptr, nullptr, nullptr, nullptr, nullptr, seeded ? ws->rev_seed64 : (unsigned long long *)nullptr };
    const int ex_gx = lr_cdiv(na, LR_EX_ROWS), ex_total = ex_gx * c.pairs;
    hipLaunchKernelGGL(nn16_exact_kernel, dim3(8 * lr_cdiv(ex_total, 8)), dim3(256), 0, st, F1, nrm1, na, F0, nrm0, nb, ws->cand_cnt, ws->cand,
                       strips, 1, (const float *)nullptr, 0, (const int32_t *)ws->rev_rows, (const int32_t *)n_rows, reo, ws->counters,
                       (const float *)ws->nn_range, 1, ex_gx, ex_total, c.z);
    LR_LAUNCH_CHECK();
    return LR_OK;
}
```

Before: 12620 pairs/s.

## Enable form-specialised pass-B hint for batched calls and bound top1 exact search

```diff
diff --git a/include/lidarreg.h b/include/lidarreg.h
--- a/include/lidarreg.h
+++ b/include/lidarreg.h
@@ -152,6 +152,8 @@
                                  int32_t *corr_idx0, int32_t *corr_idx1, void *stream);
 LR_API int lr_workspace_lists_batch(lr_workspace *ws, int npairs, int width, int32_t *nn_idx1, int32_t *nn_idx2,
                                     int32_t *corr_idx0, int32_t *corr_idx1, void *stream);
+LR_API int lr_workspace_rev_key_at(lr_workspace *ws, int pair, int n0, float *key, void *stream);
+LR_API int lr_workspace_form_launches(lr_workspace *ws, long long out[4]);
 
 LR_API size_t lr_voxel_dedup_scratch_bytes(int n);
 LR_API int    lr_voxel_dedup(const double *coords, int n, int32_t *sel, int32_t *n_sel, int32_t *cells, void *scratch,
diff --git a/lidarregistration_amd/_ext.py b/lidarregistration_amd/_ext.py
--- a/lidarregistration_amd/_ext.py
+++ b/lidarregistration_amd/_ext.py
@@ -14,7 +14,7 @@
     "lr_register_pair", "lr_workspace_lists", "lr_workspace_timing", "lr_workspace_timing_read",
     "lr_workspace_create_batch", "lr_register_batch", "lr_workspace_lists_at", "lr_inlier_mask", "lr_workspace_mask_at",
     "lr_voxel_dedup_scratch_bytes", "lr_voxel_dedup", "lr_workspace_option", "lr_workspace_stage_times", "lr_icp_batch", "lr_workspace_lists_batch",
-    "lr_workspace_clock", "lr_debug_fake_current_device",
+    "lr_workspace_clock", "lr_debug_fake_current_device", "lr_workspace_rev_key_at", "lr_workspace_form_launches",
     "lr_teaser_scratch_bytes", "lr_teaser", "lr_teaser_batch", "lr_teaser_timing", "lr_teaser_stage_times",
     "lr_sm_scratch_bytes", "lr_sm", "lr_sm_batch",
     "lr_voxel_mean_scratch_bytes", "lr_voxel_mean", "lr_overlap_scratch_bytes", "lr_overlap", "lr_overlap_batch",
@@ -224,6 +224,9 @@
         L.lr_workspace_timing.argtypes = [vp, ci]
         if hasattr(L, "lr_workspace_clock"):
             L.lr_workspace_clock.argtypes = [vp, ctypes.POINTER(ctypes.c_double), ctypes.POINTER(ctypes.c_ulonglong), ctypes.POINTER(ctypes.c_ulonglong), ci]
+        if hasattr(L, "lr_workspace_rev_key_at"):
+            L.lr_workspace_rev_key_at.argtypes = [vp, ci, ci, vp, vp]
+            L.lr_workspace_form_launches.argtypes = [vp, ctypes.POINTER(ctypes.c_longlong * 4)]
         L.lr_teaser_scratch_bytes.restype = ctypes.c_size_t
         L.lr_teaser_scratch_bytes.argtypes = [ci]
         L.lr_teaser.argtypes = [vp, vp, ci, vp, ctypes.POINTER(TeaserParams), vp, vp, vp, ctypes.c_size_t, vp]
@@ -290,6 +293,11 @@
         check(lib().lr_workspace_clock(self._h, ctypes.byref(mhz), ctypes.byref(cyc), ctypes.byref(tk), int(bool(reset))))
         return mhz.value, cyc.value, tk.value
 
+    def form_launches(self):
+        out = (ctypes.c_longlong * 4)()
+        check(lib().lr_workspace_form_launches(self._h, ctypes.byref(out)))
+        return list(out)
+
     @property
     def handle(self):
         return self._h
diff --git a/lidarregistration_amd/csrc/lr_api.hip b/lidarregistration_amd/csrc/lr_api.hip
--- a/lidarregistration_amd/csrc/lr_api.hip
+++ b/lidarregistration_amd/csrc/lr_api.hip
@@ -209,8 +209,9 @@
     carve(ws, real);
     ws->descs = reinterpret_cast<lr_pair_desc *>(ws->base + desc_off);
     ws->clk_dev = reinterpret_cast<unsigned long long *>(ws->base + clk_off);
-    if (hipHostMalloc(reinterpret_cast<void **>(&ws->form_host), 2 * sizeof(int32_t), hipHostMallocMapped) == hipSuccess) {
-        ws->form_host[0] = ws->form_host[1] = 0;
+    ws->form_acc = reinterpret_cast<unsigned *>(ws->base + clk_off + 64);
+    if (hipHostMalloc(reinterpret_cast<void **>(&ws->form_host), 4 * sizeof(int32_t), hipHostMallocMapped) == hipSuccess) {
+        for (int k = 0; k < 4; ++k) ws->form_host[k] = 0;
         if (hipHostGetDevicePointer(reinterpret_cast<void **>(&ws->form_dev), ws->form_host, 0) != hipSuccess) { (void)hipHostFree(ws->form_host); ws->form_host = ws->form_dev = nullptr; }
     } else { (void)hipGetLastError(); ws->form_host = ws->form_dev = nullptr; }
     if (hipMemset(ws->base, 0, ws->bytes) != hipSuccess || hipStreamSynchronize(nullptr) != hipSuccess) {
@@ -260,6 +261,7 @@
     LR_CHECK_DEVICE(ws, stream, "lr_workspace_poison");
     forget_last_batch(ws);
     LR_HIP(hipMemsetAsync(ws->base, byte & 0xff, ws->bytes, (hipStream_t)stream));
+    LR_HIP(hipMemsetAsync(ws->form_acc, 0, 4 * sizeof(unsigned), (hipStream_t)stream));
     return LR_OK;
 }
 
@@ -283,6 +285,24 @@
     if (nn_idx2) LR_HIP(hipMemcpyAsync(nn_idx2, at(ws->nn_idx2), nb, hipMemcpyDeviceToDevice, st));
     if (corr_idx0) LR_HIP(hipMemcpyAsync(corr_idx0, at(ws->corr_idx0), nb, hipMemcpyDeviceToDevice, st));
     if (corr_idx1) LR_HIP(hipMemcpyAsync(corr_idx1, at(ws->corr_idx1), nb, hipMemcpyDeviceToDevice, st));
+    return LR_OK;
+}
+
+extern "C" int lr_workspace_rev_key_at(lr_workspace *ws, int pair, int n0, float *key, void *stream)
+{
+    LR_CHECK_DEVICE(ws, stream, "lr_workspace_rev_key_at");
+    LR_REQUIRE(key, LR_EINVAL, "lr_workspace_rev_key_at: null pointer");
+    LR_REQUIRE(pair >= 0 && pair < ws->last_npairs, LR_EINVAL, "lr_workspace_rev_key_at: the last registration call on this workspace had fewer pairs");
+    LR_REQUIRE(n0 > 0 && n0 <= ws->max_n0, LR_ESIZE, "lr_workspace_rev_key_at: n0 exceeds the workspace");
+    LR_HIP(hipMemcpyAsync(key, reinterpret_cast<const char *>(ws->rev_s1) + (size_t)pair * ws->stride, sizeof(float) * (size_t)n0,
+                          hipMemcpyDeviceToDevice, (hipStream_t)stream));
+    return LR_OK;
+}
+
+extern "C" int lr_workspace_form_launches(lr_workspace *ws, long long out[4])
+{
+    LR_REQUIRE(ws && out, LR_EINVAL, "lr_workspace_form_launches: null pointer");
+    for (int k = 0; k < 4; ++k) out[k] = ws->form_launches[k];
     return LR_OK;
 }
 
@@ -620,9 +640,9 @@
     LR_TRY(lr_nn16_prep(c, F0, n0, F1, n1, true));
     const bool fuse_seed = p->mode != LR_MODE_NO_FILTER;
     LR_TRY_HIP(lr_timer_mark(c, LR_EV_CALL_BEGIN));
-    const bool want2 = !(ws->nn_second_auto && p->mode != LR_MODE_GPF && p->ransac.sampler == 0);
+    const bool want2 = !(ws->nn_second_auto && p->mode != LR_MODE_GPF && p->ransac.sampler == 0 && p->refit != 3);
     int32_t *idx2 = want2 ? ws->nn_idx2 : nullptr;
-    LR_TRY(lr_nn16_run(c, F0, n0, F1, n1, ws->nn_idx1, idx2, ws->nn_s1, ws->nn_s2, fuse_seed));
+    LR_TRY(lr_nn16_run(c, F0, n0, F1, n1, ws->nn_idx1, idx2, ws->nn_s1, ws->nn_s2, fuse_seed, !want2));
     LR_TRY_HIP(lr_timer_mark(c, LR_EV_FWD_NN_DONE));
     if (p->mode == LR_MODE_NO_FILTER) {
         LR_TRY(lr_identity_corr(c, n0, ws->nn_idx1, idx2, ws->corr_idx0, ws->corr_idx1, idx2 ? ws->corr_idx2 : nullptr, m_dev));
diff --git a/lidarregistration_amd/csrc/lr_internal.h b/lidarregistration_amd/csrc/lr_internal.h
--- a/lidarregistration_amd/csrc/lr_internal.h
+++ b/lidarregistration_amd/csrc/lr_internal.h
@@ -113,8 +113,11 @@
     float *bmax0, *bmax1;
     float *bmin0, *bmin1;
     float *nn_range;
-    int form_prev[2];
+    int form_prev[4];
     int32_t *form_host, *form_dev;
+    int form_only[2];
+    unsigned *form_acc;
+    long long form_launches[4];
     uint32_t *rev_seed;
     unsigned long long *rev_seed64;
     int32_t *rev_rows;
@@ -224,7 +227,7 @@
 
 int lr_nn16_prep(const lr_call &c, const float *F0, int n0, const float *F1, int n1, bool zero_counters = false);
 int lr_nn16_run(const lr_call &c, const float *F0, int n0, const float *F1, int n1,
-                int32_t *idx1, int32_t *idx2, float *s1, float *s2, bool seed_reverse = false);
+                int32_t *idx1, int32_t *idx2, float *s1, float *s2, bool seed_reverse = false, bool bound_key = false);
 int lr_nn16_reverse(const lr_call &c, const float *F0, int n0, const float *F1, int n1, const int32_t *fwd_idx1, int32_t *rev, bool seeded = false);
 
 int lr_mutual_run(const lr_call &c, int n0, const int32_t *idx1, const int32_t *idx2, const int32_t *rev,
diff --git a/lidarregistration_amd/csrc/lr_nn16.hip b/lidarregistration_amd/csrc/lr_nn16.hip
--- a/lidarregistration_amd/csrc/lr_nn16.hip
+++ b/lidarregistration_amd/csrc/lr_nn16.hip
@@ -79,7 +79,7 @@
 
 __global__ void __launch_bounds__(256)
 nn16_range_kernel(int na, const float *__restrict__ bmaxa, const float *__restrict__ bmina, int nb, const float *__restrict__ bmaxb,
-                  const float *__restrict__ bminb, float *__restrict__ range, int32_t *__restrict__ form_out, lr_zargs z)
+                  const float *__restrict__ bminb, float *__restrict__ range, int32_t *__restrict__ form_out, unsigned *__restrict__ form_acc, lr_zargs z)
 {
     __shared__ float s_m[4], s_n[4];
     if (z.descs) { na = z.descs[blockIdx.z].n0; nb = z.descs[blockIdx.z].n1; }
@@ -97,7 +97,17 @@
         const float hi = fmaxf(fmaxf(s_m[0], s_m[1]), fmaxf(s_m[2], s_m[3])), lo = fminf(fminf(s_n[0], s_n[1]), fminf(s_n[2], s_n[3]));
         range[2 * second] = hi;
         range[2 * second + 1] = lo;
-        if (form_out) form_out[second] = (lo > 0.0f && hi < LR_INF && hi - lo <= 1e-4f * hi) ? 1 : 2;
+        const int form = (lo > 0.0f && hi < LR_INF && hi - lo <= 1e-4f * hi) ? 1 : 2;
+        if (form_out && !form_acc) form_out[second] = form;
+        if (form_out && form_acc) {
+            atomicOr(&form_acc[second], (unsigned)form);
+            __threadfence();
+            if (atomicAdd(&form_acc[2 + second], 1u) == gridDim.z - 1) {
+                __threadfence();
+                form_out[second] = (int32_t)atomicExch(&form_acc[second], 0u);
+                form_acc[2 + second] = 0u;
+            }
+        }
     }
 }
 
@@ -159,7 +169,7 @@
     const unsigned long long old = atomicMin(best, key);
     atomicMin(second, old > key ? old : key);
 }
-__device__ __forceinline__ void ex_write_row(const lr_ex_out &o, int rowd, unsigned long long kb, unsigned long long ks, int nb, int need, float &sv, float &key)
+__device__ __forceinline__ void ex_write_row(const lr_ex_out &o, int rowd, unsigned long long kb, unsigned long long ks, int nb, int need, float bound, float &sv, float &key)
 {
     const int i1 = kb == LR_EX_EMPTY ? -1 : (int)(unsigned)kb;
     const float b1 = kb == LR_EX_EMPTY ? LR_INF : __uint_as_float((unsigned)(kb >> 32));
@@ -175,7 +185,7 @@
             atomicMin(&o.seed64[i1], ((unsigned long long)__float_as_uint(sv) << 32) | (unsigned)rowd);
         }
         key = sv;
-        if (need >= 2) { key = ks == LR_EX_EMPTY ? 3.0e38f : __uint_as_float((unsigned)(ks >> 32)); if (!(key < 3.0e38f)) key = 3.0e38f; }
+        if (need >= 2) { key = ks == LR_EX_EMPTY ? 3.0e38f : __uint_as_float((unsigned)(ks >> 32)); key = fminf(key, bound); if (!(key < 3.0e38f)) key = 3.0e38f; }
         o.seed_s1[rowd] = key;
     }
 }
@@ -744,7 +754,7 @@
 __global__ void __launch_bounds__(256)
 nn16_exact_kernel(const float *__restrict__ Fq, const float *__restrict__ nQ, int na,
                   const float *__restrict__ Fc, const float *__restrict__ nC, int nb,
-                  const int32_t *__restrict__ cand_cnt, const int32_t *__restrict__ cand, int nstrips, int need,
+                  const int32_t *__restrict__ cand_cnt, const int32_t *__restrict__ cand, int nstrips, int need, int top1,
                   const float *__restrict__ yfin, int yfin_stride,
                   const int32_t *__restrict__ rowmap, const int32_t *__restrict__ na_dev, lr_ex_out out,
                   int32_t *__restrict__ counters, const float *__restrict__ range_c, int dir, int gx, int total, lr_zargs z)
@@ -757,6 +767,8 @@
     __shared__ unsigned long long s_best[LR_EX_ROWS], s_second[LR_EX_ROWS];
     __shared__ int s_cnt[LR_EX_ROWS], s_rowd[LR_EX_ROWS], s_badrow[LR_EX_ROWS];
     __shared__ int s_bad, s_skip, s_nredo, s_redo[LR_EX_ROWS];
+    __shared__ float s_yf[LR_EX_ROWS], s_g1[LR_EX_ROWS], s_thr1[LR_EX_ROWS], s_ek[LR_EX_ROWS];
+    __shared__ unsigned s_lb2[LR_EX_ROWS];
     if (z.descs) {
         const lr_pair_desc d = z.descs[pair];
         Fq = dir ? d.F1 : d.F0; na = dir ? d.n1 : d.n0; Fc = dir ? d.F0 : d.F1; nb = dir ? d.n0 : d.n1;
@@ -779,7 +791,10 @@
         float *dst = &s_a[rl * LR_EX_STRIDE + 8 * part];
         dst[0] = u.x; dst[1] = u.y; dst[2] = u.z; dst[3] = u.w; dst[4] = v.x; dst[5] = v.y; dst[6] = v.z; dst[7] = v.w;
         const bool bad = ex_bad8(u, v);
-        if (tid < LR_EX_ROWS) { s_best[tid] = LR_EX_EMPTY; s_second[tid] = LR_EX_EMPTY; s_cnt[tid] = 0; s_badrow[tid] = 0; }
+        if (tid < LR_EX_ROWS) {
+            s_best[tid] = LR_EX_EMPTY; s_second[tid] = LR_EX_EMPTY; s_cnt[tid] = 0; s_badrow[tid] = 0;
+            s_yf[tid] = LR_INF; s_g1[tid] = -LR_INF; s_thr1[tid] = -LR_INF; s_ek[tid] = 0.0f; s_lb2[tid] = 0x7f800000u;
+        }
         if (tid == 0) {
             s_bad = ((range_c != nullptr && range_c[1] < 0.0f) || miss) ? 1 : 0; s_skip = miss; s_nredo = 0;
         }
@@ -806,7 +821,6 @@
         const int32_t *cw = cand_cnt + bxi * (nstrips + 1);
         const int used = min(max(cw[nstrips], 1), nstrips);
         const int seg_cap = lr_seg_cap(used);
-        __shared__ float s_yf[LR_EX_ROWS];
         if (tid < LR_EX_ROWS) {
             float yv = LR_INF;
             if (yfin && row0 + tid < na) for (int sidx = 0; sidx < used; ++sidx) yv = fminf(yv, yfin[(size_t)sidx * yfin_stride + row0 + tid]);
@@ -814,6 +828,32 @@
         }
         __syncthreads();
         const uint2 *__restrict__ segs = reinterpret_cast<const uint2 *>(cand) + (size_t)bxi * LR_NN16_SEG;
+        if (top1) {
+            for (int sidx = 0; sidx < used; ++sidx) {
+                const int c = cw[sidx];
+                for (int e = tid; e < c; e += 256) {
+                    const uint2 v = segs[(size_t)sidx * seg_cap + e];
+                    if (!(v.x & LR_PB_HASG)) continue;
+                    const int rl = lr_pb_row(lr_pb_kb(v.x), __builtin_ctz((v.y & 0xffffu) | 0x8000u));
+                    const unsigned gb = v.y & 0xffff0000u;
+                    const float gv = __uint_as_float(gb), yr = s_yf[rl];
+                    if (gv + 1e-5f * (fabsf(gv) + fabsf(yr)) < -yr) continue;
+                    if (!(fabsf(gv) < LR_INF)) continue;
+                    const float glo = __uint_as_float((gb & 0x80000000u) ? (gb | 0xffffu) : (gb >= 0x10000u ? gb - 0x10000u : 0u));
+                    if (fabsf(glo) < LR_INF) atomicMax(&s_g1[rl], glo);
+                }
+            }
+            __syncthreads();
+            if (tid < LR_EX_ROWS) {
+                const float n0v = s_nq[tid], scale = n0v + (range_c ? range_c[0] : LR_INF);
+                const float ek = (1.05e-3f * scale + 4e-7f) + 12e-6f * scale;
+                const float ub = fmaxf((n0v - 2.0f * s_g1[tid]) + ek, 1e-20f);
+                const float thr = 0.5f * ((n0v - ek) - ub * (1.0f + 1e-6f)) - 4e-6f * scale;
+                s_ek[tid] = ek;
+                s_thr1[tid] = thr == thr ? thr : -LR_INF;
+            }
+            __syncthreads();
+        }
         for (int sidx = 0; sidx < used; ++sidx) {
             const int c = cw[sidx];
             if (c < 0) { if (tid == 0) s_bad = 1; continue; }
@@ -824,6 +864,11 @@
                     const int rl = lr_pb_row(ekb, __builtin_ctz((v.y & 0xffffu) | 0x8000u));
                     const float gv = __uint_as_float(v.y & 0xffff0000u), yr = s_yf[rl];
                     if (gv + 1e-5f * (fabsf(gv) + fabsf(yr)) < -yr) continue;
+                    if (gv < s_thr1[rl]) {
+                        atomicMin(&s_lb2[rl], __float_as_uint(fmaxf((s_nq[rl] - 2.0f * gv) - s_ek[rl], 0.0f)));
+                        atomicAdd(&s_cnt[rl], 1);
+                        continue;
+                    }
                 }
                 f32x4 t[8];
                 const f32x4 *pb = reinterpret_cast<const f32x4 *>(Fc + (size_t)j * 32);
@@ -847,7 +892,7 @@
     const int nredo = s_nredo;
     for (int r = 0; r < nredo; ++r) {
         const int rl = s_redo[r];
-        if (tid == 0) { s_best[rl] = LR_EX_EMPTY; s_second[rl] = LR_EX_EMPTY; atomicAdd(&counters[LR_CNT_FIX_TOTAL], 1); }
+        if (tid == 0) { s_best[rl] = LR_EX_EMPTY; s_second[rl] = LR_EX_EMPTY; s_lb2[rl] = 0x7f800000u; s_yf[rl] = LR_INF; atomicAdd(&counters[LR_CNT_FIX_TOTAL], 1); }
         __syncthreads();
         for (int j = tid; j < nb; j += 256) {
             f32x4 t[8];
@@ -860,17 +905,29 @@
     __syncthreads();
     float sv = 3.0e38f, key = 0.0f;
     const bool writer = tid < LR_EX_ROWS && row0 + tid < na;
-    if (writer) ex_write_row(out, s_rowd[tid], s_best[tid], s_second[tid], nb, need, sv, key);
+    float bound = LR_INF;
+    if (top1 && writer) {
+        float xo = (s_nq[tid] + 2.0f * s_yf[tid]) - 3.0f * s_ek[tid];
+        if (!(xo == xo)) xo = 0.0f;
+        const float b2 = fmaxf(fminf(__uint_as_float(s_lb2[tid]), xo), 0.0f);
+        const float r = __builtin_sqrtf(b2);
+        bound = (r > 0.0f && r < LR_INF) ? __uint_as_float(__float_as_uint(r) - 1u) : r;
+        if (!(bound == bound)) bound = 0.0f;
+    }
+    if (writer) ex_write_row(out, s_rowd[tid], s_best[tid], s_second[tid], nb, need, bound, sv, key);
     if (out.seed_out && tid < 64) ex_range(out, writer, sv, key, tid);
 }
 
+static int lr_nn16_form_hint(const lr_call &c, int col_cloud);
 int lr_nn16_prep(const lr_call &c, const float *F0, int n0, const float *F1, int n1, bool zero_counters)
 {
     lr_workspace *ws = c.ws;
+    ws->form_only[0] = lr_nn16_form_hint(c, 0); ws->form_only[1] = lr_nn16_form_hint(c, 1);
     hipLaunchKernelGGL(nn16_prep_kernel, dim3(lr_cdiv(n0, 32) + lr_cdiv(n1, 32), 1, c.pairs), dim3(256), 0, c.st, F0, n0, ws->H0, ws->nrm0, ws->bmax0, ws->bmin0,
                        F1, n1, ws->H1, ws->nrm1, ws->bmax1, ws->bmin1, ws->rev_seed, ws->rev_seed64, ws->counters, zero_counters ? 1 : 0, lr_cdiv(n0, 32), ws->yshare, c.z);
     hipLaunchKernelGGL(nn16_range_kernel, dim3(2, 1, c.pairs), dim3(256), 0, c.st, n0, (const float *)ws->bmax0, (const float *)ws->bmin0, n1, (const float *)ws->bmax1,
-                       (const float *)ws->bmin1, ws->nn_range, c.pairs == 1 ? ws->form_dev : (int32_t *)nullptr, c.z);
+                       (const float *)ws->bmin1, ws->nn_range, ws->form_dev ? ws->form_dev + (c.pairs == 1 ? 0 : 2) : (int32_t *)nullptr,
+                       c.pairs == 1 ? (unsigned *)nullptr : ws->form_acc, c.z);
     LR_LAUNCH_CHECK();
     return LR_OK;
 }
@@ -878,10 +935,11 @@
 static int lr_nn16_form_hint(const lr_call &c, int col_cloud)
 {
     lr_workspace *ws = c.ws;
-    if (c.pairs != 1 || !ws->form_host) return 0;
-    const int h = *reinterpret_cast<const volatile int32_t *>(&ws->form_host[col_cloud]);
-    const int prev = ws->form_prev[col_cloud];
-    ws->form_prev[col_cloud] = h;
+    if (!ws->form_host) return 0;
+    const int k = col_cloud + (c.pairs == 1 ? 0 : 2);
+    const int h = *reinterpret_cast<const volatile int32_t *>(&ws->form_host[k]);
+    const int prev = ws->form_prev[k];
+    ws->form_prev[k] = h;
     return ((h == 1 || h == 2) && h == prev) ? h : 0;
 }
 
@@ -900,7 +958,7 @@
     const int total = a.row_blocks * a.strips * c.pairs;
     const dim3 grid(8 * lr_cdiv(total, 8));
     LR_TRY_HIP(lr_timer_mark(c, a.dir ? LR_EV_REV_FILTER_BEGIN : LR_EV_FWD_FILTER_BEGIN));
-    const int only = lr_nn16_form_hint(c, a.dir ? 0 : 1);
+    const int only = ws->form_only[a.dir ? 0 : 1];
     int32_t *miss = ws->counters + (a.dir ? LR_CNT_FORM_MISS_R : LR_CNT_FORM_MISS_F);
     unsigned long long *clk = ws->clock_probe ? ws->clk_dev : (unsigned long long *)nullptr;
     const lr_pb_tail tl = { clk };
@@ -909,17 +967,18 @@
         hipLaunchKernelGGL(kernel, grid, dim3(256), 0, c.st, tl, clk, a.Hq, a.na, a.rowmap, a.na_dev, a.Hc, a.nC, a.nb, a.tps, a.tau, ws->cand_cnt, ws->cand,
                            a.colmap, a.tile_min, a.row_bound, a.rev_offs, a.rev_range, a.yfin, a.yfin_stride, a.yshare, miss, a.thr, pg, c.z);
     };
-    if (only != 2) launch(nn16_passb_kernel<true>);
-    if (only != 1) launch(nn16_passb_kernel<false>);
+    if (only != 2) { launch(nn16_passb_kernel<true>); ++ws->form_launches[a.dir ? 2 : 0]; }
+    if (only != 1) { launch(nn16_passb_kernel<false>); ++ws->form_launches[a.dir ? 3 : 1]; }
     return lr_timer_mark(c, a.dir ? LR_EV_REV_FILTER_END : LR_EV_FWD_FILTER_END);
 }
 
 int lr_nn16_run(const lr_call &c, const float *Fq, int na, const float *Fc, int nb,
-                int32_t *idx1, int32_t *idx2, float *s1, float *s2, bool seed_reverse)
+                int32_t *idx1, int32_t *idx2, float *s1, float *s2, bool seed_reverse, bool bound_key)
 {
     lr_workspace *ws = c.ws;
     const float *nQ = ws->nrm0, *nC = ws->nrm1, *range_c = ws->nn_range + 2;
-    const int need = idx2 ? 2 : 1;
+    const int top1 = (bound_key && !idx2) ? 1 : 0;
+    const int need = (idx2 || top1) ? 2 : 1;
     const int ntiles = lr_cdiv(nb, 32);
     const int row_blocks = lr_cdiv(na, LR_BLOCK_ROWS);
     int strips = c.pairs > 1 ? lr_cdiv(ws->nn_blocks_batch, row_blocks * c.pairs) : ws->nn_blocks_target / row_blocks;
@@ -942,7 +1001,7 @@
                            reinterpret_cast<uint32_t *>(ws->counters + LR_CNT_RLO), ws->rev_seed64 };
     const int ex_gx = lr_cdiv(na, LR_EX_ROWS), ex_total = ex_gx * c.pairs;
     hipLaunchKernelGGL(nn16_exact_kernel, dim3(8 * lr_cdiv(ex_total, 8)), dim3(256), 0, c.st, Fq, nQ, na, Fc, nC, nb, ws->cand_cnt, ws->cand,
-                       strips, need, (const float *)ws->yfin, ws->max_n, (const int32_t *)nullptr, (const int32_t *)nullptr, eo, ws->counters,
+                       strips, need, top1, (const float *)ws->yfin, ws->max_n, (const int32_t *)nullptr, (const int32_t *)nullptr, eo, ws->counters,
                        range_c, 0, ex_gx, ex_total, c.z);
     LR_LAUNCH_CHECK();
     return LR_OK;
@@ -1149,7 +1208,7 @@
     const lr_ex_out reo = { rev, nullptr, nullptr, nullptr, nullptr, nullptr, nullptr, seeded ? ws->rev_seed64 : (unsigned long long *)nullptr };
     const int ex_gx = lr_cdiv(na, LR_EX_ROWS), ex_total = ex_gx * c.pairs;
     hipLaunchKernelGGL(nn16_exact_kernel, dim3(8 * lr_cdiv(ex_total, 8)), dim3(256), 0, st, F1, nrm1, na, F0, nrm0, nb, ws->cand_cnt, ws->cand,
-                       strips, 1, (const float *)nullptr, 0, (const int32_t *)ws->rev_rows, (const int32_t *)n_rows, reo, ws->counters,
+                       strips, 1, 0, (const float *)nullptr, 0, (const int32_t *)ws->rev_rows, (const int32_t *)n_rows, reo, ws->counters,
                        (const float *)ws->nn_range, 1, ex_gx, ex_total, c.z);
     LR_LAUNCH_CHECK();
     return LR_OK;
```

Measured after the change: 12100 pairs/s. -4.1%, worse.
